# yifanlu0227/HEAL

Hardware: AMD Instinct MI355X
Metric: scenes/sec (5-agent OPV2V-H, PointPillars+PyramidFusion) (higher is better)
Workload: dtype f32

## Files before the change

### heal_amd/_capi.py

```python
import ctypes
import os
import re

HERE = os.path.dirname(os.path.abspath(__file__))
LIB_PATH = os.environ.get("HEAL_AMD_LIB") or os.path.join(HERE, "lib", "libheal_amd.so")
HEADER = os.path.join(os.path.dirname(HERE), "include", "heal_amd.h")
HEADER_EXPERIMENTAL = os.path.join(os.path.dirname(HERE), "include", "heal_amd_experimental.h")

_lib = None

c_void_p, c_int, c_float, c_size_t = ctypes.c_void_p, ctypes.c_int, ctypes.c_float, ctypes.c_size_t

_SIGNATURES = {
    "heal_abi_version": (c_int, []),
    "heal_last_error": (ctypes.c_char_p, []),
    "heal_fill_bytes": (c_int, [c_void_p, c_int, c_size_t, c_void_p]),
    "heal_next_launch_events": (c_int, [c_void_p, c_void_p]),
    "heal_voxelize_workspace": (c_size_t, [c_int, c_int, c_int, ctypes.c_longlong]),
    "heal_voxelize": (c_int, [c_void_p, c_int, c_void_p, c_void_p, c_int, c_int, c_int,
                              c_void_p, c_void_p, c_void_p, c_void_p, c_void_p, c_void_p, c_void_p, c_size_t, c_int, c_void_p]),
    "heal_voxelize_batch_workspace": (c_size_t, [c_int, c_int, c_int, c_int, ctypes.c_longlong]),
    "heal_voxelize_batch": (c_int, [c_void_p, c_void_p, c_int, c_void_p, c_void_p, c_int, c_int, c_void_p, c_void_p,
                                    c_void_p, c_void_p, c_void_p, c_size_t, c_int, c_void_p]),
    "heal_mask_points": (c_int, [c_void_p, c_int, c_void_p, c_int, c_void_p, c_void_p]),
    "heal_pfn_scatter_workspace": (c_size_t, [c_int] * 5),
    "heal_pfn_scatter": (c_int, [c_void_p, c_void_p, c_void_p, c_int, c_void_p, c_int,
                                 c_void_p, c_void_p, c_void_p, c_int,
                                 c_float, c_float, c_float, c_float, c_float, c_float,
                                 c_int, c_int, c_int, c_void_p, c_void_p, c_void_p, c_size_t, c_void_p]),
    "heal_pfn_pillars": (c_int, [c_void_p, c_void_p, c_void_p, c_int, c_void_p, c_int, c_void_p, c_void_p, c_void_p, c_int,
                                 c_float, c_float, c_float, c_float, c_float, c_float, c_int, c_int, c_int, c_void_p, c_void_p,
                                 c_void_p]),
    "heal_pillar_canvas": (c_int, [c_void_p, c_void_p, c_int, c_int, c_int, c_int, c_void_p, c_void_p]),
    "heal_pillar_stem_block": (c_int, [c_void_p, c_void_p, c_int, c_int, c_int, c_int] + [c_void_p] * 4 + [c_int] + [c_void_p] * 3),
    "heal_bev_pool_backward": (c_int, [c_void_p] * 5 + [c_int] * 6 + [c_void_p] * 6),
    "heal_warp_fuse": (c_int, [c_void_p, c_void_p, c_int, c_int, c_int, c_int, c_void_p, c_void_p, c_int, c_void_p,
                               c_void_p, c_void_p]),
    "heal_warp_fuse_levels": (c_int, [c_int, c_void_p, c_void_p, c_int, c_void_p, c_void_p, c_void_p, c_void_p, c_void_p, c_int,
                                      c_void_p, c_void_p, c_void_p]),
    "heal_warp_fuse_backward": (c_int, [c_void_p, c_void_p, c_int, c_int, c_int, c_int, c_void_p, c_void_p, c_int, c_void_p,
                                        c_void_p, c_void_p, c_void_p, c_void_p]),
    "heal_warp_agent": (c_int, [c_void_p, c_void_p, c_int, c_int, c_int, c_void_p, c_void_p, c_int, c_void_p,
                                c_void_p, c_void_p, c_void_p]),
    "heal_warp_agents_pm": (c_int, [c_void_p, c_int, c_int, c_int, c_int, c_void_p, c_void_p, c_int, c_void_p, c_void_p]),
    "heal_fuse_warped": (c_int, [c_void_p, c_void_p, c_int, c_int, c_int, c_int, c_void_p, c_void_p]),
    "heal_fuse_warped_rows": (c_int, [c_void_p, c_void_p, c_void_p, c_int, c_int, c_int, c_int, c_void_p, c_void_p]),
    "heal_decode_nms_workspace": (c_size_t, [c_int, c_int]),
    "heal_decode_nms": (c_int, [c_void_p, c_void_p, c_void_p, c_void_p, c_int, c_int, c_int, c_int,
                                c_float, c_float, c_float, c_int, c_void_p, c_void_p,
                                c_void_p, c_void_p, c_void_p, c_int, c_void_p, c_size_t, c_void_p]),
    "heal_quad_iou": (c_int, [c_void_p, c_int, c_void_p, c_int, c_void_p, c_void_p]),
    "heal_bev_pool_workspace": (c_size_t, [c_int] * 9),
    "heal_bev_pool": (c_int, [c_void_p, c_void_p, c_void_p, c_void_p, c_int, c_int, c_int, c_int, c_int, c_int,
                              c_void_p, c_void_p, c_void_p, c_void_p, c_void_p, c_size_t, c_void_p]),
    "heal_bev_pool_pm_workspace": (c_size_t, [c_int] * 5),
    "heal_bev_pool_pm": (c_int, [c_void_p, c_int, c_void_p, c_void_p] + [c_int] * 6 + [c_void_p] * 5 + [c_size_t, c_void_p]),
    "heal_bev_pool_scatter": (c_int, [c_void_p, c_int, c_void_p, c_void_p] + [c_int] * 6 + [c_void_p] * 4 + [c_size_t, c_void_p]),
    "heal_bev_pool_scatter_multi": (c_int, [c_int] + [c_void_p] * 16),
    "heal_bev_pool_emit": (c_int, [c_int, c_int, c_void_p, c_void_p, c_void_p, c_size_t, c_void_p]),
    "heal_bev_stem_block": (c_int, [c_int, c_int] + [c_void_p] * 8 + [c_size_t, c_void_p]),
    "heal_pfn_train_blocks": (c_int, [c_int]),
    "heal_pfn_features": (c_int, [c_void_p, c_void_p, c_void_p, c_int, c_int, c_void_p, c_void_p, c_void_p, c_float, c_float,
                                  c_float, c_float, c_float, c_float, c_void_p, c_void_p]),
    "heal_pfn_moments": (c_int, [c_void_p, c_void_p, c_void_p, c_int, c_int, c_float, c_float, c_float, c_float, c_float, c_float,
                                 c_void_p, c_void_p]),
    "heal_pfn_backward": (c_int, [c_void_p, c_void_p, c_void_p, c_int, c_int, c_void_p, c_void_p, c_void_p, c_void_p, c_void_p,
                                  c_float, c_float, c_float, c_float, c_float, c_float, c_void_p, c_void_p, c_void_p]),
    "heal_mean_vfe": (c_int, [c_void_p, c_void_p, c_int, c_int, c_int, c_void_p, c_void_p, c_void_p]),
    "heal_sp_sort_workspace": (c_size_t, [c_int]),
    "heal_sp_sort_sites": (c_int, [c_void_p, c_int, c_void_p, c_int, c_void_p, c_void_p, c_void_p, c_size_t, c_void_p,
                                   c_void_p]),
    "heal_sp_wgrad_chunks": (c_int, [c_int]),
    "heal_sp_wgrad": (c_int, [c_void_p, c_void_p, c_void_p, c_int, c_int, c_int, c_int, c_void_p, c_void_p, c_void_p]),
    "heal_sp_gather_rows": (c_int, [c_void_p, c_void_p, c_int, c_int, c_void_p, c_void_p, c_void_p]),
    "heal_sp_table_capacity": (c_size_t, [c_int]),
    "heal_sp_hash_build": (c_int, [c_void_p, c_int, c_void_p, c_int, c_void_p, c_void_p, c_size_t, c_void_p, c_void_p]),
    "heal_sp_neighbors": (c_int, [c_void_p, c_int, c_void_p, c_void_p, c_void_p, c_void_p, c_void_p, c_int,
                                  c_void_p, c_void_p, c_size_t, c_void_p, c_void_p, c_void_p]),
    "heal_sp_out_sites_workspace": (c_size_t, [c_int, c_int]),
    "heal_sp_out_sites": (c_int, [c_void_p, c_int, c_void_p, c_void_p, c_void_p, c_void_p, c_void_p, c_int,
                                  c_void_p, c_int, c_void_p, c_void_p, c_size_t, c_void_p, c_void_p]),
    "heal_conv_gemm": (c_int, [c_void_p, c_void_p, c_void_p, c_void_p] + [c_int] * 8 + [c_void_p, c_void_p]),
    "heal_ln_stats": (c_int, [c_void_p, c_int, c_int, c_float, c_void_p, c_void_p]),
    "heal_linear": (c_int, [c_void_p, c_int, c_int, ctypes.c_longlong, c_void_p, c_void_p, c_void_p, c_int, c_void_p, c_int,
                            c_int, c_void_p, c_int, c_void_p, c_int, c_int, c_int, c_int, c_int, c_int, c_int,
                            ctypes.c_longlong, c_int, c_void_p]),
    "heal_split_attn_workspace": (c_size_t, [c_int, c_int, c_int]),
    "heal_split_attn_weights": (c_int, [c_void_p, ctypes.c_longlong, c_int, c_int, c_int] + [c_void_p] * 5 + [c_float] +
                                [c_void_p] * 5),
    "heal_split_attn_colsum": (c_int, [c_void_p, ctypes.c_longlong, c_int, c_int, c_int, c_void_p, c_void_p]),
    "heal_split_attn_weights_from_colsum": (c_int, [c_void_p, c_int, c_int, c_int, c_int] + [c_void_p] * 5 + [c_float] +
                                            [c_void_p] * 4),
    "heal_sp_rank_bytes": (c_size_t, [c_void_p, c_int]),
    "heal_sp_out_sites_rank": (c_int, [c_void_p, c_int, c_void_p, c_void_p, c_void_p, c_void_p, c_void_p, c_int,
                                       c_void_p, c_int, c_void_p, c_void_p, c_size_t, c_void_p, c_void_p, c_void_p]),
    "heal_sp_neighbors_rank": (c_int, [c_void_p, c_int, c_void_p, c_void_p, c_void_p, c_void_p, c_void_p, c_int,
                                       c_void_p, c_size_t, c_int, c_void_p, c_void_p, c_void_p, c_void_p]),
    "heal_sp_neighbors_root": (c_int, [c_void_p, c_int, c_void_p, c_void_p, c_void_p, c_void_p, c_void_p, c_int,
                                       c_void_p, c_size_t, c_int, c_void_p, c_void_p, c_void_p, c_void_p]),
    "heal_sp_root_rank_bytes": (c_size_t, [c_void_p, c_int]),
    "heal_sp_pair_tiles_words": (c_size_t, [c_int, c_int]),
    "heal_sp_neighbor_tiles": (c_int, [c_void_p, c_int, c_void_p, c_void_p, c_void_p, c_void_p, c_void_p, c_int,
                                       c_void_p, c_size_t, c_int, c_int, c_void_p, c_int, c_void_p, c_void_p, c_void_p]),
    "heal_sp_tiles_to_neighbors": (c_int, [c_void_p, c_int, c_int, c_void_p, c_void_p, c_void_p]),
    "heal_sp_conv_tiles_supported": (c_int, [c_int, c_int]),
    "heal_sp_conv_tiles": (c_int, [c_void_p, c_void_p, c_int, c_int, c_int, c_int, c_void_p, c_void_p, c_void_p, c_int,
                                   c_void_p, c_void_p, c_void_p]),
    "heal_sp_root_rank": (c_int, [c_void_p, c_int, c_void_p, c_int, c_void_p, c_void_p, c_void_p, c_int, c_void_p, c_void_p,
                                  c_size_t, c_void_p, c_void_p]),
    "heal_gconv_conv3_supported": (c_int, [c_int] * 5),
    "heal_gconv_conv3": (c_int, [c_void_p] * 6 + [c_int] * 7 + [c_void_p, c_void_p]),
    "heal_sp_transpose_neighbors": (c_int, [c_void_p, c_int, c_int, c_int, c_void_p, c_void_p, c_void_p]),
    "heal_sp_weight_fragments": (c_int, [c_void_p, c_int, c_int, c_int, c_void_p, c_void_p]),
    "heal_sp_conv": (c_int, [c_void_p, c_void_p, c_int, c_int, c_int, c_int, c_void_p, c_void_p, c_void_p, c_void_p, c_int,
                             c_void_p, c_void_p, c_void_p]),
    "heal_sp_to_bev_workspace": (c_size_t, [c_int, c_int, c_int, c_int]),
    "heal_sp_to_bev": (c_int, [c_void_p, c_void_p, c_int, c_int, c_void_p, c_int, c_void_p, c_void_p, c_size_t,
                               c_void_p, c_void_p]),
    "heal_agent_attention": (c_int, [c_void_p, c_void_p, c_void_p, c_void_p, c_int, c_int, c_int, c_int, c_float,
                                     c_int, c_void_p, c_int, c_void_p]),
    "heal_agent_attention_backward": (c_int, [c_void_p] * 5 + [c_int, c_int, c_int, c_int, c_float, c_int] + [c_void_p] * 3 +
                                      [c_int, c_void_p]),
    "heal_grouped_conv3x3": (c_int, [c_void_p, c_void_p, c_void_p, c_int, c_int, c_int, c_int, c_int, c_int, c_int,
                                     c_void_p, c_void_p]),
    "heal_bias_act": (c_int, [c_void_p, c_void_p, c_void_p, c_int, c_int, c_int, c_int, c_void_p]),
    "heal_resnext_bottleneck": (c_int, [c_void_p] * 7 + [c_int, c_int, c_int, c_int, c_void_p, c_void_p]),
    "heal_upsample2x_bilinear": (c_int, [c_void_p, c_int, c_int, c_int, c_int, c_void_p, c_void_p]),
    "heal_depthwise_conv": (c_int, [c_void_p, c_void_p, c_void_p] + [c_int] * 11 + [c_void_p, c_void_p, c_void_p]),
    "heal_camera_matrices": (c_int, [c_void_p] * 5 + [c_int, c_void_p, c_void_p]),
    "heal_channel_dot": (c_int, [c_void_p] * 3 + [c_int] * 3 + [c_void_p, c_void_p]),
    "heal_layernorm_nchw": (c_int, [c_void_p] * 3 + [c_int] * 3 + [c_float, c_void_p, c_void_p]),
    "heal_se_gate": (c_int, [c_void_p] * 5 + [c_int] * 3 + [c_float, c_int, c_void_p, c_void_p]),
    "heal_conv1x1": (c_int, [c_void_p] * 5 + [c_int] * 8 + [c_void_p, c_void_p]),
    "heal_stem7x7": (c_int, [c_void_p, ctypes.c_longlong, c_int, c_int, c_int, c_int, c_void_p, c_void_p, c_int, c_void_p, c_void_p]),
    "heal_conv1x1_split_supported": (c_int, [c_int] * 4),
    "heal_conv1x1_split": (c_int, [c_void_p] * 4 + [c_int] * 7 + [c_void_p, c_void_p]),
    "heal_conv1x1_tiled_supported": (c_int, [c_int] * 5),
    "heal_conv1x1_tiled": (c_int, [c_void_p] * 4 + [c_int] * 9 + [c_void_p, c_void_p]),
    "heal_conv1x1_splitk_workspace": (c_size_t, [c_int] * 5),
    "heal_conv1x1_splitk": (c_int, [c_void_p] * 5 + [c_int] * 7 + [c_void_p, c_void_p, c_size_t, c_void_p]),
    "heal_conv1x1_d2s": (c_int, [c_void_p] * 3 + [c_int] * 9 + [c_void_p, c_void_p]),
    "heal_conv3x3": (c_int, [c_void_p] * 4 + [c_int] * 7 + [c_void_p, c_void_p]),
    "heal_conv3x3_same": (c_int, [c_void_p] * 3 + [c_int] * 11 + [c_void_p, c_void_p]),
    "heal_grouped16_conv3x3": (c_int, [c_void_p] * 3 + [c_int] * 5 + [c_void_p, c_void_p]),
    "heal_grouped_small_conv3x3": (c_int, [c_void_p] * 3 + [c_int] * 7 + [c_void_p, c_void_p]),
    "heal_conv3x3_winograd4": (c_int, [c_void_p] * 4 + [c_int] * 6 + [c_void_p, c_void_p]),
    "heal_conv3x3_winograd": (c_int, [c_void_p] * 4 + [c_int] * 7 + [c_void_p, c_void_p]),
    "heal_conv3x3_winograd_kc": (c_int, [c_void_p] * 4 + [c_int] * 8 + [c_void_p, c_void_p]),
    "heal_conv3x3_winograd_splitk_workspace": (c_size_t, [c_int] * 5),
    "heal_conv3x3_winograd_splitk": (c_int, [c_void_p] * 4 + [c_int] * 8 + [c_void_p, c_void_p, c_size_t, c_void_p]),
    "heal_nms_quads_workspace": (c_size_t, [c_int]),
    "heal_nms_quads": (c_int, [c_void_p, c_int, c_float, c_void_p, c_size_t, c_void_p, c_void_p, c_void_p]),
    "heal_window_attention": (c_int, [c_void_p, c_void_p, c_int, c_int, c_int, c_int, c_int, c_int, c_float, c_void_p,
                                      c_void_p]),
    "heal_window_attention_backward_workspace": (c_size_t, [c_int, c_int, c_int, c_int]),
    "heal_window_attention_backward": (c_int, [c_void_p] * 4 + [c_int] * 6 + [c_float, c_void_p, c_void_p, c_void_p, c_size_t,
                                                c_void_p]),
    "heal_agent_window_attention": (c_int, [c_void_p, c_void_p] + [c_int] * 8 + [c_float, c_void_p, c_void_p]),
    "heal_agent_mean": (c_int, [c_void_p, c_int, ctypes.c_longlong, c_void_p, c_void_p]),
    "heal_v2v_message_workspace": (c_size_t, [c_int] * 5),
    "heal_v2v_message": (c_int, [c_void_p, c_void_p, c_void_p, ctypes.c_longlong, c_void_p, c_void_p] + [c_int] * 9
                         + [c_void_p, c_void_p, c_size_t, c_void_p]),
    "heal_gru_zero_state": (c_int, [c_void_p, ctypes.c_longlong, c_void_p, ctypes.c_longlong] + [c_int] * 4 + [c_void_p, c_void_p]),
    "heal_label_assign_workspace": (c_size_t, [c_int]),
    "heal_label_assign": (c_int, [c_void_p, c_int, c_void_p, c_int, c_float, c_float, c_void_p, c_void_p, c_void_p,
                                  c_size_t, c_void_p]),
    "heal_boxes_bev_matrix": (c_int, [c_void_p, c_int, c_void_p, c_int, c_int, c_void_p, c_void_p]),
    "heal_nms_bev_workspace": (c_size_t, [c_int]),
    "heal_nms_bev": (c_int, [c_void_p, c_int, c_float, c_int, c_void_p, c_size_t, c_void_p, c_void_p, c_void_p]),
}


class HealAmdError(RuntimeError):
    pass


def declared_symbols(experimental=False):
    text = open(HEADER_EXPERIMENTAL if experimental else HEADER).read()
    text = re.sub(r"/\*.*?\*/", "", text, flags=re.S)
    return sorted(set(re.findall(r"\b(heal_[a-z0-9_]+)\s*\(", text)))


def abi_version_of_header():
    m = re.search(r"#define\s+HEAL_AMD_ABI_VERSION\s+(\d+)", open(HEADER).read())
    if not m:
        raise HealAmdError(f"{HEADER} does not define HEAL_AMD_ABI_VERSION")
    return int(m.group(1))


def lib():
    global _lib
    if _lib is None:
        if not os.path.exists(LIB_PATH):
            raise HealAmdError(
                f"{LIB_PATH} is missing: the HIP extension has not been built "
                "(run `python -m heal_amd.build`); heal_amd has no CPU fallback")
        import torch
        L = ctypes.CDLL(LIB_PATH)
        for name, (res, args) in _SIGNATURES.items():
            if not hasattr(L, name):
                continue
            f = getattr(L, name)
            f.restype = res
            f.argtypes = args
        want = abi_version_of_header()
        got = int(L.heal_abi_version()) if hasattr(L, "heal_abi_version") else -1
        if got != want:
            raise HealAmdError(f"{LIB_PATH} has C-ABI version {got}, include/heal_amd.h declares {want}: rebuild it "
                               "(python -m heal_amd.build --force)")
        _lib = L
    return _lib


_TRACE = int(os.environ.get("HEAL_TRACE_CALLS", "0") or 0)


def _trace_call(name, args):
    import sys
    import torch
    cap = torch.cuda.is_current_stream_capturing()
    extra = ""
    if _TRACE >= 2:
        extra = " " + " ".join(hex(a.value or 0) if isinstance(a, ctypes.c_void_p) else str(a) for a in args
                               if isinstance(a, (int, float, ctypes.c_void_p)))
    print(f"[heal pid {os.getpid()}] {'capture ' if cap else ''}{name}{extra}", file=sys.stderr, flush=True)


def _trace_done(name):
    import sys
    import torch
    if not torch.cuda.is_current_stream_capturing():
        torch.cuda.synchronize()
        print(f"[heal pid {os.getpid()}]   ok {name}", file=sys.stderr, flush=True)


_GUARD = os.environ.get("HEAL_GRAPH_GUARD", "0") == "1"
_guard_log = []


def _segments():
    import torch
    segs = []
    for seg in torch.cuda.memory_snapshot():
        blocks, addr = [], seg["address"]
        for b in seg["blocks"]:
            a = b.get("address", addr)
            blocks.append((a, a + b["size"], b["state"]))
            addr = a + b["size"]
        pool = tuple(seg.get("segment_pool_id", (0, 0)))
        segs.append((seg["address"], seg["address"] + seg["total_size"], pool != (0, 0), blocks))
    segs.sort()
    return segs


def _locate(segs, addr):
    import bisect
    i = bisect.bisect_right(segs, (addr, float("inf"), True, [])) - 1
    if i < 0 or not (segs[i][0] <= addr < segs[i][1]):
        return None
    for lo, hi, state in segs[i][3]:
        if lo <= addr < hi:
            return segs[i][2], state
    return segs[i][2], "unknown"


def guard_begin():
    global _guard_log
    _guard_log = []


def guard_take():
    global _guard_log
    log, _guard_log = _guard_log, []
    if not log:
        return []
    segs = _segments()
    seen, out = set(), []
    for name, addr in log:
        if addr not in seen and _locate(segs, addr) is not None:
            seen.add(addr)
            out.append((name, addr))
    return out


def guard_check(entries, what="captured graph"):
    if not entries:
        return
    segs = _segments()
    for name, addr in entries:
        where = _locate(segs, addr)
        if where is None:
            raise HealAmdError(f"{what}: {name} was captured with device address {addr:#x}, which is no longer mapped "
                               "(its tensor was freed and the memory returned to the driver)")
        private, state = where
        if not private and state != "active_allocated":
            raise HealAmdError(f"{what}: {name} was captured with device address {addr:#x}, whose block is now '{state}' "
                               "(its tensor was freed: a replay would read or overwrite somebody else's memory)")


def call(name, *args):
    L = lib()
    if not hasattr(L, name):
        raise HealAmdError(f"libheal_amd.so does not export {name}")
    if _TRACE:
        _trace_call(name, args)
    if _GUARD:
        import torch
        if torch.cuda.is_current_stream_capturing():
            _guard_log.extend((name, a.value) for a in args if isinstance(a, ctypes.c_void_p) and a.value)
    rc = getattr(L, name)(*args)
    if rc != 0:
        raise HealAmdError(f"{name} failed: {L.heal_last_error().decode(errors='replace')}")
    if _TRACE:
        _trace_done(name)


def query(name, *args):
    L = lib()
    if not hasattr(L, name):
        raise HealAmdError(f"libheal_amd.so does not export {name}")
    return int(getattr(L, name)(*args))
```

### heal_amd/csrc/common.h

```cpp
#pragma once
#include <hip/hip_runtime.h>
#include <hip/hip_ext.h>
#include <stdint.h>
#include <stddef.h>
#include <stdio.h>
#include <stdarg.h>

#define HEAL_WAVE 64

namespace heal {

char* err_buf();
int set_error(const char* fmt, ...);

inline size_t align_up(size_t x, size_t a = 256) { return (x + a - 1) / a * a; }
inline int ceil_div(int a, int b) { return (a + b - 1) / b; }
inline int64_t ceil_div64(int64_t a, int64_t b) { return (a + b - 1) / b; }

struct Arena {
    char* base; size_t cap; size_t off;
    Arena(void* p, size_t n) : base((char*)p), cap(n), off(0) {}
    template <typename T> T* take(size_t count) {
        size_t bytes = align_up(count * sizeof(T));
        T* r = (T*)(base + off);
        off += bytes;
        return r;
    }
    bool ok() const { return off <= cap && (base != nullptr || off == 0); }
};

#define HEAL_HIP(expr)                                                                      \
    do {                                                                                    \
        hipError_t e__ = (expr);                                                            \
        if (e__ != hipSuccess)                                                              \
            return heal::set_error("%s failed: %s (%s:%d)", #expr, hipGetErrorString(e__), \
                                   __FILE__, __LINE__);                                     \
    } while (0)

#define HEAL_REQUIRE(cond, ...)                       \
    do {                                              \
        if (!(cond)) return heal::set_error(__VA_ARGS__); \
    } while (0)

#define HEAL_LAUNCH_CHECK() HEAL_HIP(hipGetLastError())

int debug_env_once(const char* name);
#define HEAL_DEBUG_ENV(name) ([]() -> int { static const int v__ = heal::debug_env_once(name); return v__; }())

int fill_bytes(void* dst, int byte, size_t bytes, hipStream_t s);
int copy_word(int* dst, const int* src, hipStream_t s);
#define HEAL_FILL(dst, byte, bytes, s)                      \
    do {                                                    \
        if (heal::fill_bytes((dst), (byte), (bytes), (s))) return 1; \
    } while (0)

struct LaunchEvents { hipEvent_t start, stop; };
LaunchEvents take_launch_events();
#define HEAL_LAUNCH_EV(kernel, grid, block, lds, stream, ...)                                                        \
    do {                                                                                                             \
        const heal::LaunchEvents ev__ = heal::take_launch_events();                                                  \
        if (ev__.start && ev__.stop)                                                                                 \
            hipExtLaunchKernelGGL(kernel, grid, block, (std::uint32_t)(lds), stream, ev__.start, ev__.stop, 0, __VA_ARGS__); \
        else                                                                                                         \
            hipLaunchKernelGGL(kernel, grid, block, (std::uint32_t)(lds), stream, __VA_ARGS__);                      \
    } while (0)

#define HEAL_LAUNCH_EV2(kernel, grid, block, lds, stream, ev_start, ev_stop, ...)                                    \
    do {                                                                                                             \
        if ((ev_start) || (ev_stop))                                                                                 \
            hipExtLaunchKernelGGL(kernel, grid, block, (std::uint32_t)(lds), stream, ev_start, ev_stop, 0, __VA_ARGS__); \
        else                                                                                                         \
            hipLaunchKernelGGL(kernel, grid, block, (std::uint32_t)(lds), stream, __VA_ARGS__);                      \
    } while (0)

__device__ __forceinline__ int lane_id() { return threadIdx.x & 63; }

__device__ __forceinline__ unsigned long long lanemask_lt() {
    return (1ull << (threadIdx.x & 63)) - 1ull;
}

__device__ __forceinline__ float wave_sum(float v) {
#pragma unroll
    for (int o = 32; o > 0; o >>= 1) v += __shfl_xor(v, o, 64);
    return v;
}
__device__ __forceinline__ int wave_sum_i(int v) {
#pragma unroll
    for (int o = 32; o > 0; o >>= 1) v += __shfl_xor(v, o, 64);
    return v;
}
__device__ __forceinline__ int wave_incl_scan(int v) {
    const int l = threadIdx.x & 63;
#pragma unroll
    for (int o = 1; o < 64; o <<= 1) {
        int t = __shfl_up(v, o, 64);
        if (l >= o) v += t;
    }
    return v;
}


__device__ __forceinline__ void lds_barrier() { asm volatile("s_waitcnt lgkmcnt(0)\n\ts_barrier" ::: "memory"); }

struct Block3 { unsigned x, y, z; };
__device__ inline Block3 xcd_block() {
    const unsigned gx = gridDim.x, gy = gridDim.y, nb = gx * gy * gridDim.z;
    unsigned b = blockIdx.x + gx * (blockIdx.y + gy * blockIdx.z);
    const unsigned q = nb >> 3, r = nb & 7u, xcd = b & 7u;
    b = (xcd < r ? xcd * (q + 1) : r * (q + 1) + (xcd - r) * q) + (b >> 3);
    Block3 o;
    o.x = b % gx;
    b /= gx;
    o.y = b % gy;
    o.z = b / gy;
    return o;
}

}
```

### heal_amd/csrc/conv1x1.hip

```cpp
#include <stdlib.h>
#include "common.h"
#include "../../include/heal_amd.h"

namespace heal {

using f32x4 = __attribute__((ext_vector_type(4))) float;

template <int BM, int BN, int KC, int STRIDE>
__global__ __launch_bounds__(256) void k_conv1x1(const float* __restrict__ x, const float* __restrict__ wfrag,
                                                const float* __restrict__ bias, const float* __restrict__ res,
                                                const float* __restrict__ in_scale, int Cin, int Kpad, int Cout,
                                                int HW, int Wo, int in_W, int in_HW, int act, int out_pm,
                                                int d2s_k, int d2s_ctot, int d2s_coff, int n_img, int ksplit,
                                                float* __restrict__ y) {
    constexpr int MT = BM / 64;
    constexpr int NT = BN / 16;
    constexpr int LD = BN + 16;
    constexpr int KS = KC / 4;
    constexpr int TPR = BN / 4;
    constexpr int RPP = 256 / TPR;
    constexpr int NPASS = KC / RPP;
    static_assert(NPASS >= 1 && KC % RPP == 0, "bad staging shape");
    __shared__ __attribute__((aligned(16))) float sB[2][KC][LD];
    const Block3 bk = xcd_block();
    const int m0 = bk.x * BM, p0 = bk.y * BN, n = bk.z % n_img, kpart = bk.z / n_img;
    const int wave = threadIdx.x >> 6, l = threadIdx.x & 63;
    const int lk = l >> 4, ln = l & 15;
    const float* __restrict__ xin = x + (size_t)n * Cin * in_HW;
    const int ksteps = Kpad / 4;
    const int nchunks_all = Kpad / KC, cps = (nchunks_all + ksplit - 1) / ksplit;
    const int cbeg = kpart * cps, nchunks = min(cbeg + cps, nchunks_all);
    const float* __restrict__ scl = in_scale ? in_scale + (size_t)n * Cin : nullptr;
    const int sp = (threadIdx.x % TPR) * 4, sc = threadIdx.x / TPR;
    const bool pix_ok = p0 + sp < HW;

    f32x4 acc[MT][NT];
#pragma unroll
    for (int mt = 0; mt < MT; ++mt)
#pragma unroll
        for (int nt = 0; nt < NT; ++nt) acc[mt][nt] = f32x4{0.f, 0.f, 0.f, 0.f};

    float4 stage[NPASS];
    auto load_chunk = [&](int c) {
#pragma unroll
        for (int i = 0; i < NPASS; ++i) {
            const int ch = c * KC + sc + RPP * i;
            if (pix_ok && ch < Cin) {
                float4 v;
                if constexpr (STRIDE == 1) {
                    v = *reinterpret_cast<const float4*>(xin + (size_t)ch * HW + p0 + sp);
                } else {
                    const int p = p0 + sp, oy = p / Wo, ox = p - oy * Wo;
                    const float* src = xin + (size_t)ch * in_HW + (size_t)(oy * STRIDE) * in_W + ox * STRIDE;
                    v = make_float4(src[0], src[STRIDE], src[2 * STRIDE], src[3 * STRIDE]);
                }
                if (scl) { const float g = scl[ch]; v.x *= g; v.y *= g; v.z *= g; v.w *= g; }
                stage[i] = v;
            } else {
                stage[i] = make_float4(0.f, 0.f, 0.f, 0.f);
            }
        }
    };
    auto store_chunk = [&](int buf) {
#pragma unroll
        for (int i = 0; i < NPASS; ++i) *reinterpret_cast<float4*>(&sB[buf][sc + RPP * i][sp]) = stage[i];
    };

    float a_cur[MT][KS], a_nxt[MT][KS];
    auto load_a = [&](int c, float (&a)[MT][KS]) {
#pragma unroll
        for (int mt = 0; mt < MT; ++mt) {
            const int mtg = (m0 >> 4) + wave * MT + mt;
#pragma unroll
            for (int q = 0; q < KS / 4; ++q) {
                const float4 v = *reinterpret_cast<const float4*>(wfrag + (((size_t)mtg * (ksteps / 4) + (c * KS) / 4 + q) * 64 + l) * 4);
                a[mt][4 * q] = v.x; a[mt][4 * q + 1] = v.y; a[mt][4 * q + 2] = v.z; a[mt][4 * q + 3] = v.w;
            }
        }
    };

    load_a(cbeg, a_cur);
    load_chunk(cbeg);
    store_chunk(0);
    __syncthreads();
    for (int c = cbeg; c < nchunks; ++c) {
        const int buf = (c - cbeg) & 1;
        if (c + 1 < nchunks) {
            load_a(c + 1, a_nxt);
            load_chunk(c + 1);
        }
        float bfr[2][NT];
        auto read_b = [&](int ks, float (&dst)[NT]) {
#pragma unroll
            for (int gq = 0; gq < NT / 4; ++gq) {
                const float4 v = *reinterpret_cast<const float4*>(&sB[buf][ks * 4 + lk][gq * 64 + 4 * ln]);
                dst[4 * gq] = v.x; dst[4 * gq + 1] = v.y; dst[4 * gq + 2] = v.z; dst[4 * gq + 3] = v.w;
            }
        };
        read_b(0, bfr[0]);
#pragma unroll
        for (int ks = 0; ks < KS; ++ks) {
            if (ks + 1 < KS) read_b(ks + 1, bfr[(ks + 1) & 1]);
            __builtin_amdgcn_sched_barrier(0);
#pragma unroll
            for (int nt = 0; nt < NT; ++nt)
#pragma unroll
                for (int mt = 0; mt < MT; ++mt)
                    acc[mt][nt] = __builtin_amdgcn_mfma_f32_16x16x4f32(a_cur[mt][ks], bfr[ks & 1][nt], acc[mt][nt], 0, 0, 0);
        }
        if (c + 1 < nchunks) store_chunk(buf ^ 1);
        __syncthreads();
#pragma unroll
        for (int mt = 0; mt < MT; ++mt)
#pragma unroll
            for (int ks = 0; ks < KS; ++ks) a_cur[mt][ks] = a_nxt[mt][ks];
    }

    if (out_pm == 1) {
        float* __restrict__ yout = y + (size_t)n * HW * Cout;
#pragma unroll
        for (int mt = 0; mt < MT; ++mt) {
            const int co = m0 + (wave * MT + mt) * 16 + lk * 4;
            if (co >= Cout) continue;
            float4 bv = make_float4(0.f, 0.f, 0.f, 0.f);
            if (bias) bv = *reinterpret_cast<const float4*>(bias + co);
#pragma unroll
            for (int nt = 0; nt < NT; ++nt) {
                const int p = p0 + (nt / 4) * 64 + 4 * ln + (nt & 3);
                if (p >= HW) continue;
                float4 v = make_float4(acc[mt][nt][0] + bv.x, acc[mt][nt][1] + bv.y, acc[mt][nt][2] + bv.z,
                                       acc[mt][nt][3] + bv.w);
                if (act == 1) {
                    v.x = fmaxf(v.x, 0.f); v.y = fmaxf(v.y, 0.f); v.z = fmaxf(v.z, 0.f); v.w = fmaxf(v.w, 0.f);
                } else if (act == 2) {
                    v.x = v.x / (1.f + expf(-v.x)); v.y = v.y / (1.f + expf(-v.y));
                    v.z = v.z / (1.f + expf(-v.z)); v.w = v.w / (1.f + expf(-v.w));
                }
                *reinterpret_cast<float4*>(yout + (size_t)p * Cout + co) = v;
            }
        }
        return;
    }
    float* __restrict__ yout = y + ((size_t)kpart * n_img + n) * Cout * HW;
    const float* __restrict__ rin = res ? res + (size_t)n * Cout * HW : nullptr;
    constexpr int NG = NT / 4;
#pragma unroll
    for (int mt = 0; mt < MT; ++mt) {
        float4 rq[4][NG];
        if (rin) {
#pragma unroll
            for (int r = 0; r < 4; ++r)
#pragma unroll
                for (int gq = 0; gq < NG; ++gq) {
                    const int co = min(m0 + (wave * MT + mt) * 16 + lk * 4 + r, Cout - 1), p = min(p0 + gq * 64 + 4 * ln, HW - 4);
                    rq[r][gq] = *reinterpret_cast<const float4*>(rin + (size_t)co * HW + p);
                }
        }
#pragma unroll
        for (int r = 0; r < 4; ++r) {
            const int co = m0 + (wave * MT + mt) * 16 + lk * 4 + r;
            if (co >= Cout) continue;
            const float bv = bias ? bias[co] : 0.f;
#pragma unroll
            for (int gq = 0; gq < NG; ++gq) {
                const int p = p0 + gq * 64 + 4 * ln;
                if (p >= HW) continue;
                float4 v = make_float4(acc[mt][4 * gq][r] + bv, acc[mt][4 * gq + 1][r] + bv, acc[mt][4 * gq + 2][r] + bv,
                                       acc[mt][4 * gq + 3][r] + bv);
                const size_t o = (size_t)co * HW + p;
                if (rin) { const float4 q = rq[r][gq]; v.x += q.x; v.y += q.y; v.z += q.z; v.w += q.w; }
                if (act == 1) {
                    v.x = fmaxf(v.x, 0.f); v.y = fmaxf(v.y, 0.f); v.z = fmaxf(v.z, 0.f); v.w = fmaxf(v.w, 0.f);
                } else if (act == 2) {
                    v.x = v.x / (1.f + expf(-v.x)); v.y = v.y / (1.f + expf(-v.y));
                    v.z = v.z / (1.f + expf(-v.z)); v.w = v.w / (1.f + expf(-v.w));
                } else if (act == 3) {
                    v.x = 0.5f * v.x * (1.f + erff(v.x * 0.70710678118654752f));
                    v.y = 0.5f * v.y * (1.f + erff(v.y * 0.70710678118654752f));
                    v.z = 0.5f * v.z * (1.f + erff(v.z * 0.70710678118654752f));
                    v.w = 0.5f * v.w * (1.f + erff(v.w * 0.70710678118654752f));
                }
                if (out_pm != 2) {
                    *reinterpret_cast<float4*>(yout + o) = v;
                } else {
                    const int kk = d2s_k * d2s_k, Ho = HW / Wo;
                    const int c = co / kk, rr = co - c * kk, dy = rr / d2s_k, dx = rr - dy * d2s_k;
                    const int hh = p / Wo, ww = p - hh * Wo;
                    float* dst = y + (((size_t)n * d2s_ctot + d2s_coff + c) * ((size_t)Ho * d2s_k) + (size_t)hh * d2s_k + dy) *
                                         ((size_t)Wo * d2s_k) + (size_t)ww * d2s_k + dx;
                    if (d2s_k == 1) {
                        *reinterpret_cast<float4*>(dst) = v;
                    } else {
                        dst[0] = v.x; dst[d2s_k] = v.y; dst[2 * d2s_k] = v.z; dst[3 * d2s_k] = v.w;
                    }
                }
            }
        }
    }
}


__global__ __launch_bounds__(256) void k_conv1x1_splitk_reduce(const float4* __restrict__ part, const float* __restrict__ bias,
                                                              const float4* __restrict__ res, int ksplit, int Cout, int HW4,
                                                              size_t total4, int act, float4* __restrict__ y) {
    const size_t i = (size_t)blockIdx.x * 256 + threadIdx.x;
    if (i >= total4) return;
    float4 v = part[i];
    for (int k = 1; k < ksplit; ++k) {
        const float4 q = part[(size_t)k * total4 + i];
        v.x += q.x; v.y += q.y; v.z += q.z; v.w += q.w;
    }
    const float bv = bias ? bias[(i / HW4) % Cout] : 0.f;
    v.x += bv; v.y += bv; v.z += bv; v.w += bv;
    if (res) { const float4 q = res[i]; v.x += q.x; v.y += q.y; v.z += q.z; v.w += q.w; }
    if (act == 1) {
        v.x = fmaxf(v.x, 0.f); v.y = fmaxf(v.y, 0.f); v.z = fmaxf(v.z, 0.f); v.w = fmaxf(v.w, 0.f);
    } else if (act == 2) {
        v.x = v.x / (1.f + expf(-v.x)); v.y = v.y / (1.f + expf(-v.y)); v.z = v.z / (1.f + expf(-v.z)); v.w = v.w / (1.f + expf(-v.w));
    } else if (act == 3) {
        v.x = 0.5f * v.x * (1.f + erff(v.x * 0.70710678118654752f)); v.y = 0.5f * v.y * (1.f + erff(v.y * 0.70710678118654752f));
        v.z = 0.5f * v.z * (1.f + erff(v.z * 0.70710678118654752f)); v.w = 0.5f * v.w * (1.f + erff(v.w * 0.70710678118654752f));
    }
    y[i] = v;
}

}

using namespace heal;

namespace heal {
int splitk_reduce_launch(const float* partials, const float* bias, const float* residual, int ksplit, int n, int cout, int HW,
                         int act, float* y, hipStream_t s, hipEvent_t ev_stop) {
    const size_t total4 = (size_t)n * cout * HW / 4;
    HEAL_LAUNCH_EV2(k_conv1x1_splitk_reduce, dim3((unsigned)((total4 + 255) / 256)), dim3(256), 0, s, (hipEvent_t) nullptr, ev_stop,
                    reinterpret_cast<const float4*>(partials), bias, reinterpret_cast<const float4*>(residual), ksplit, cout,
                    HW / 4, total4, act, reinterpret_cast<float4*>(y));
    HEAL_LAUNCH_CHECK();
    return 0;
}
}

static int conv1x1_launch(const float* x, const float* weight_frag, const float* bias, const float* residual,
                          const float* in_scale, int n, int cin, int cout, int H, int W, int stride, int act,
                          int out_pixel_major, int d2s_k, int d2s_ctot, int d2s_coff, float* y, void* stream,
                          int ksplit = 1, float* partials = nullptr) {
    HEAL_REQUIRE(n >= 1 && H >= 1 && W >= 1 && cin >= 1 && cout >= 1, "conv1x1: bad shape");
    HEAL_REQUIRE(stride == 1 || stride == 2, "conv1x1: stride must be 1 or 2 (got %d)", stride);
    const int kpad = (cin + 31) / 32 * 32, mpad = (cout + 63) / 64 * 64;
    const int Ho = (H - 1) / stride + 1, Wo = (W - 1) / stride + 1, HW = Ho * Wo;
    if (stride == 1) HEAL_REQUIRE(HW % 4 == 0, "conv1x1: H*W must be a multiple of 4 (got %d)", HW);
    else HEAL_REQUIRE(Wo % 4 == 0, "conv1x1: output width must be a multiple of 4 for stride 2 (got %d)", Wo);
    HEAL_REQUIRE(act >= 0 && act <= 3, "conv1x1: act must be 0 (none), 1 (ReLU), 2 (SiLU) or 3 (GELU)");
    HEAL_REQUIRE(x && weight_frag && y, "conv1x1: null pointer");
    if (out_pixel_major == 1) {
        HEAL_REQUIRE(residual == nullptr && act != 3, "conv1x1: pixel-major output takes no residual / GELU");
        HEAL_REQUIRE(cout % 4 == 0 && ((uintptr_t)bias & 15) == 0, "conv1x1: pixel-major output needs Cout %% 4 == 0 and a 16-B aligned bias");
    }
    hipStream_t s = (hipStream_t)stream;
    int bm = 64, bn = 64, kc = 32;
    if (const char* e = getenv("HEAL_C1_CFG")) {
        int a_ = 0, b_ = 0, c_ = 0;
        if (stride == 1 && sscanf(e, "%d,%d,%d", &a_, &b_, &c_) == 3) { bm = a_; bn = b_; kc = c_; }
    }
    HEAL_REQUIRE(mpad % bm == 0, "conv1x1: padded Cout %d not a multiple of the tile height %d", mpad, bm);
#define HEAL_C1(BM_, BN_, KC_, ST_)                                                                              \
    if (bm == BM_ && bn == BN_ && kc == KC_ && stride == ST_) {                                                  \
        if (ksplit > 1)                                                                                          \
            HEAL_LAUNCH_EV2((k_conv1x1<BM_, BN_, KC_, ST_>), dim3(mpad / BM_, ceil_div(HW, BN_), n * ksplit), dim3(256), 0, s, \
                            ev.start, (hipEvent_t) nullptr,                                                      \
                            x, weight_frag, (const float*)nullptr, (const float*)nullptr, in_scale, cin, kpad, cout, HW, Wo, W, \
                            H * W, 0, 0, 1, 0, 0, n, ksplit, partials);                                          \
        else                                                                                                     \
            HEAL_LAUNCH_EV2((k_conv1x1<BM_, BN_, KC_, ST_>), dim3(mpad / BM_, ceil_div(HW, BN_), n), dim3(256), 0, s, \
                            ev.start, ev.stop,                                                                   \
                            x, weight_frag, bias, residual, in_scale, cin, kpad, cout, HW, Wo, W, H * W, act, out_pixel_major, \
                            d2s_k, d2s_ctot, d2s_coff, n, 1, y);                                                 \
        launched = true;                                                                                         \
    }
    bool launched = false;
    const LaunchEvents ev = take_launch_events();
    HEAL_C1(64, 64, 32, 1) HEAL_C1(64, 64, 32, 2)
    HEAL_C1(128, 128, 32, 1) HEAL_C1(64, 128, 32, 1) HEAL_C1(128, 64, 32, 1)
#undef HEAL_C1
    HEAL_REQUIRE(launched, "conv1x1: no kernel for tile (%d,%d,%d) stride %d", bm, bn, kc, stride);
    if (ksplit > 1) {
        const size_t total4 = (size_t)n * cout * HW / 4;
        HEAL_LAUNCH_EV2(k_conv1x1_splitk_reduce, dim3((unsigned)((total4 + 255) / 256)), dim3(256), 0, s, (hipEvent_t) nullptr, ev.stop,
                        reinterpret_cast<const float4*>(partials), bias, reinterpret_cast<const float4*>(residual), ksplit, cout,
                        HW / 4, total4, act, reinterpret_cast<float4*>(y));
    }
    HEAL_LAUNCH_CHECK();
    return 0;
}

extern "C" int heal_conv1x1(const float* x, const float* weight_frag, const float* bias, const float* residual,
                            const float* in_scale, int n, int cin, int cout, int H, int W, int stride, int act,
                            int out_pixel_major, float* y, void* stream) {
    HEAL_REQUIRE(out_pixel_major == 0 || out_pixel_major == 1, "conv1x1: out_pixel_major must be 0 or 1");
    return conv1x1_launch(x, weight_frag, bias, residual, in_scale, n, cin, cout, H, W, stride, act, out_pixel_major, 1, 0, 0,
                          y, stream);
}

extern "C" int heal_conv1x1_d2s(const float* x, const float* weight_frag, const float* bias, int n, int cin, int cout, int H,
                                int W, int act, int k, int dst_channels, int dst_channel_offset, float* y, void* stream) {
    HEAL_REQUIRE(k >= 1 && k <= 8 && cout % (k * k) == 0, "conv1x1_d2s: Cout must be a multiple of k^2 (k = %d)", k);
    HEAL_REQUIRE(W % 4 == 0, "conv1x1_d2s: W must be a multiple of 4 (got %d)", W);
    HEAL_REQUIRE(dst_channel_offset >= 0 && dst_channel_offset + cout / (k * k) <= dst_channels,
                 "conv1x1_d2s: channel slice [%d, %d) outside the %d destination channels", dst_channel_offset,
                 dst_channel_offset + cout / (k * k), dst_channels);
    HEAL_REQUIRE(((uintptr_t)y & 15) == 0, "conv1x1_d2s: destination must be 16-B aligned");
    return conv1x1_launch(x, weight_frag, bias, nullptr, nullptr, n, cin, cout, H, W, 1, act, 2, k, dst_channels,
                          dst_channel_offset, y, stream);
}

extern "C" size_t heal_conv1x1_splitk_workspace(int n, int cout, int H, int W, int ksplit) {
    return ksplit > 1 ? (size_t)ksplit * n * cout * H * W * sizeof(float) : 0;
}

extern "C" int heal_conv1x1_splitk(const float* x, const float* weight_frag, const float* bias, const float* residual,
                                   const float* in_scale, int n, int cin, int cout, int H, int W, int act, int ksplit, float* y,
                                   void* ws, size_t ws_bytes, void* stream) {
    const int nchunks = (cin + 31) / 32;
    HEAL_REQUIRE(ksplit >= 2 && ksplit <= nchunks, "conv1x1_splitk: ksplit must be in [2, %d] (got %d)", nchunks, ksplit);
    HEAL_REQUIRE((ksplit - 1) * ceil_div(nchunks, ksplit) < nchunks,
                 "conv1x1_splitk: %d splits of %d chunks leave an empty split (use ceil(chunks / ceil(chunks / ksplit)))", ksplit,
                 nchunks);
    HEAL_REQUIRE((H * W) % 4 == 0, "conv1x1_splitk: H*W must be a multiple of 4");
    HEAL_REQUIRE((long long)n * ksplit <= 65535, "conv1x1_splitk: n * ksplit exceeds the grid limit");
    HEAL_REQUIRE(ws && ws_bytes >= heal_conv1x1_splitk_workspace(n, cout, H, W, ksplit) && ((uintptr_t)ws & 15) == 0,
                 "conv1x1_splitk: workspace too small or misaligned");
    HEAL_REQUIRE(act >= 0 && act <= 3, "conv1x1_splitk: act must be 0..3");
    return conv1x1_launch(x, weight_frag, bias, residual, in_scale, n, cin, cout, H, W, 1, act, 0, 1, 0, 0, y, stream, ksplit,
                          (float*)ws);
}
```

### heal_amd/csrc/gconv_small.hip

```cpp
#include <stdlib.h>
#include "common.h"
#include "../../include/heal_amd.h"

namespace heal {

using f32x4 = __attribute__((ext_vector_type(4))) float;

template <int CG, int TH, int STRIDE>
__global__ __launch_bounds__(256) __attribute__((amdgpu_waves_per_eu(3, 4))) void k_gconv_small(
    const float* __restrict__ x, const float* __restrict__ wq, const float* __restrict__ bias, int C, int H, int W, int Ho,
    int Wo, int tiles_x, int relu, float* __restrict__ y) {
    static_assert(CG == 4 || CG == 8 || CG == 16, "4, 8 or 16 channels per group");
    static_assert(TH == 8 || TH == 16, "tile height");
    static_assert(STRIDE == 1 || STRIDE == 2, "stride");
    constexpr int TW = STRIDE == 1 ? 32 : 16, NSEG = TW / 16, RW = TH / 4;
    constexpr int PR = STRIDE * TH + 3 - STRIDE, PC = STRIDE * TW + 3 - STRIDE;
    constexpr int NSIDE = 3 - STRIDE;
    constexpr int NSTEP = 9 * CG;
    constexpr int KH = CG == 16 ? 2 : 1;
    constexpr int CGH = CG / KH;
    constexpr int NB = CG / 4, NBH = CGH / 4;
    __shared__ float4 sP[PR * PC * 4];
    __shared__ float4 sW[NSTEP * 16 / 4];
    const Block3 bk = xcd_block();
    const int sg = bk.y, n = bk.z;
    const int ty = bk.x / tiles_x, tx = bk.x - ty * tiles_x;
    const int oy0 = ty * TH, ox0 = tx * TW;
    const int gy0 = oy0 * STRIDE - 1, gx0 = ox0 * STRIDE;
    const int t = threadIdx.x, wave = t >> 6, l = t & 63;
    const size_t HW = (size_t)H * W, HWo = (size_t)Ho * Wo;
    const float* __restrict__ xin = x + ((size_t)n * C + (size_t)sg * 16) * HW;

    constexpr int N_IN = PR * 8 * 4, IT_IN = (N_IN + 255) / 256;
    constexpr int N_HA = PR * NSIDE * 4;
    static_assert(N_HA <= 256 && STRIDE * TW == 32, "staging shape");
    float4 vin[IT_IN][4];
    unsigned ok_bits = 0;
#pragma unroll
    for (int it = 0; it < IT_IN; ++it) {
        const int u = min(t + 256 * it, N_IN - 1);
        const int gq = u & 3, quad = (u >> 2) & 7, row = u >> 5;
        const int gy = gy0 + row, gx = gx0 + quad * 4;
        const bool ok = gy >= 0 && gy < H && gx < W;
        ok_bits |= ok ? (1u << it) : 0u;
        const float* src = xin + (size_t)(gq * 4) * HW + (ok ? (size_t)gy * W + gx : 0);
        vin[it][0] = *reinterpret_cast<const float4*>(src);
        vin[it][1] = *reinterpret_cast<const float4*>(src + HW);
        vin[it][2] = *reinterpret_cast<const float4*>(src + 2 * HW);
        vin[it][3] = *reinterpret_cast<const float4*>(src + 3 * HW);
    }
    float4 vha;
    {
        const int u = min(t, N_HA - 1);
        const int gq = u & 3, side = NSIDE == 2 ? (u >> 2) & 1 : 0, row = u / (4 * NSIDE);
        const int gy = gy0 + row, gx = side ? gx0 + 32 : gx0 - 1;
        const bool ok = gy >= 0 && gy < H && gx >= 0 && gx < W;
        ok_bits |= ok ? 256u : 0u;
        const float* src = xin + (size_t)(gq * 4) * HW + (ok ? (size_t)gy * W + gx : 0);
        vha = make_float4(src[0], src[HW], src[2 * HW], src[3 * HW]);
    }
    constexpr int N_W4 = NSTEP * 16 / 4, IT_W = (N_W4 + 255) / 256;
#pragma unroll
    for (int it = 0; it < IT_W; ++it) {
        const int i = min(t + 256 * it, N_W4 - 1);
        sW[i] = reinterpret_cast<const float4*>(wq + (size_t)sg * NSTEP * 16)[i];
    }
#pragma unroll
    for (int it = 0; it < IT_IN; ++it) {
        const int u = min(t + 256 * it, N_IN - 1);
        const int gq = u & 3, quad = (u >> 2) & 7, row = u >> 5;
        const bool ok = (ok_bits >> it) & 1u;
        float4* d = sP + (row * PC + 1 + quad * 4) * 4 + gq;
        const float4 a = vin[it][0], b = vin[it][1], c = vin[it][2], e = vin[it][3];
        d[0] = make_float4(ok ? a.x : 0.f, ok ? b.x : 0.f, ok ? c.x : 0.f, ok ? e.x : 0.f);
        d[4] = make_float4(ok ? a.y : 0.f, ok ? b.y : 0.f, ok ? c.y : 0.f, ok ? e.y : 0.f);
        d[8] = make_float4(ok ? a.z : 0.f, ok ? b.z : 0.f, ok ? c.z : 0.f, ok ? e.z : 0.f);
        d[12] = make_float4(ok ? a.w : 0.f, ok ? b.w : 0.f, ok ? c.w : 0.f, ok ? e.w : 0.f);
    }
    {
        const int u = min(t, N_HA - 1);
        const int gq = u & 3, side = NSIDE == 2 ? (u >> 2) & 1 : 0, row = u / (4 * NSIDE);
        const bool okh = ok_bits & 256u;
        sP[(row * PC + (side ? PC - 1 : 0)) * 4 + gq] =
            make_float4(okh ? vha.x : 0.f, okh ? vha.y : 0.f, okh ? vha.z : 0.f, okh ? vha.w : 0.f);
    }
    __syncthreads();
    const float bv0 = bias ? bias[sg * 16 + (l & 15)] : 0.f;
    const int p = (l >> 4) * 4 + (l & 3);
    const int unit0 = (((l >> 2) & 3) * 4 / CG) * NB;
    const float4* __restrict__ abase = sP + ((wave * RW * STRIDE) * PC + p * STRIDE) * 4 + unit0;

    f32x4 acc[RW][NSEG];
#pragma unroll
    for (int o = 0; o < RW; ++o)
#pragma unroll
        for (int s = 0; s < NSEG; ++s) acc[o][s] = f32x4{0.f, 0.f, 0.f, 0.f};
#pragma unroll
    for (int half = 0; half < KH; ++half) {
        float wreg[9 * CGH];
#pragma unroll
        for (int tap = 0; tap < 9; ++tap)
#pragma unroll
            for (int ci = 0; ci < CGH; ++ci)
                wreg[tap * CGH + ci] = reinterpret_cast<const float*>(sW)[(tap * CG + half * CGH + ci) * 16 + (l & 15)];
#pragma unroll
        for (int ry = 0; ry < STRIDE * (RW - 1) + 3; ++ry) {
#pragma unroll
            for (int dx = 0; dx < 3; ++dx) {
                float4 av[NSEG][NBH];
#pragma unroll
                for (int s = 0; s < NSEG; ++s)
#pragma unroll
                    for (int h = 0; h < NBH; ++h) av[s][h] = abase[(ry * PC + s * 16 * STRIDE + dx) * 4 + half * NBH + h];
#pragma unroll
                for (int ci = 0; ci < CGH; ++ci) {
#pragma unroll
                    for (int o = 0; o < RW; ++o) {
                        const int dy = ry - STRIDE * o;
                        if (dy < 0 || dy > 2) continue;
#pragma unroll
                        for (int s = 0; s < NSEG; ++s) {
                            const float4 q = av[s][ci >> 2];
                            const float a = (ci & 3) == 0 ? q.x : (ci & 3) == 1 ? q.y : (ci & 3) == 2 ? q.z : q.w;
                            acc[o][s] = __builtin_amdgcn_mfma_f32_4x4x1f32(a, wreg[(dy * 3 + dx) * CGH + ci], acc[o][s], 0, 0, 0);
                        }
                    }
                }
            }
        }
    }
    float* __restrict__ yout = y + ((size_t)n * C + (size_t)sg * 16 + (l & 15)) * HWo;
#pragma unroll
    for (int o = 0; o < RW; ++o) {
        const int oy = oy0 + wave * RW + o;
#pragma unroll
        for (int s = 0; s < NSEG; ++s) {
            const int ox = ox0 + s * 16 + (l >> 4) * 4;
            if (oy >= Ho || ox >= Wo) continue;
            float4 v = make_float4(acc[o][s][0] + bv0, acc[o][s][1] + bv0, acc[o][s][2] + bv0, acc[o][s][3] + bv0);
            if (relu) { v.x = fmaxf(v.x, 0.f); v.y = fmaxf(v.y, 0.f); v.z = fmaxf(v.z, 0.f); v.w = fmaxf(v.w, 0.f); }
            *reinterpret_cast<float4*>(yout + (size_t)oy * Wo + ox) = v;
        }
    }
}

}

using namespace heal;

extern "C" int heal_grouped_small_conv3x3(const float* x, const float* weight_q, const float* bias, int n, int channels,
                                          int group_channels, int H, int W, int stride, int relu, float* y, void* stream) {
    HEAL_REQUIRE(group_channels == 4 || group_channels == 8 || group_channels == 16,
                 "grouped_small_conv3x3: 4, 8 or 16 channels per group (got %d)", group_channels);
    HEAL_REQUIRE(stride == 1 || stride == 2, "grouped_small_conv3x3: stride must be 1 or 2 (got %d)", stride);
    const int Ho = (H - 1) / stride + 1, Wo = (W - 1) / stride + 1;
    HEAL_REQUIRE(n >= 1 && channels >= 16 && channels % 16 == 0 && H >= 1 && W >= 4 && W % 4 == 0 && Wo % 4 == 0,
                 "grouped_small_conv3x3: needs channels %% 16 == 0, W %% 4 == 0 and an output width %% 4 == 0 (got C=%d W=%d)",
                 channels, W);
    HEAL_REQUIRE(x && weight_q && y && ((uintptr_t)x & 15) == 0 && ((uintptr_t)y & 15) == 0,
                 "grouped_small_conv3x3: bad pointer (x, y must be 16-B aligned)");
    int th = (group_channels == 4 && stride == 1) ? 16 : 8;
    if (const char* e = getenv("HEAL_GS_TH")) th = atoi(e) == 8 ? 8 : atoi(e) == 16 ? 16 : th;
    if (stride == 2 || group_channels == 16) th = 8;
    const int tw = stride == 1 ? 32 : 16;
    const int tiles_x = ceil_div(Wo, tw), tiles_y = ceil_div(Ho, th);
    HEAL_REQUIRE(channels / 16 <= 65535 && n <= 65535, "grouped_small_conv3x3: grid limit");
    const dim3 grid(tiles_x * tiles_y, channels / 16, n);
    hipStream_t s_ = (hipStream_t)stream;
#define HEAL_GS(CG_, TH_, ST_)                                                                                        \
    if (group_channels == CG_ && th == TH_ && stride == ST_)                                                          \
        HEAL_LAUNCH_EV((k_gconv_small<CG_, TH_, ST_>), grid, dim3(256), 0, s_, x, weight_q, bias, channels, H, W, Ho, Wo, tiles_x, relu, y);
    HEAL_GS(4, 16, 1) HEAL_GS(4, 8, 1) HEAL_GS(8, 16, 1) HEAL_GS(8, 8, 1)
    HEAL_GS(4, 8, 2) HEAL_GS(8, 8, 2) HEAL_GS(16, 8, 1) HEAL_GS(16, 8, 2)
#undef HEAL_GS
    HEAL_LAUNCH_CHECK();
    return 0;
}
```

### heal_amd/opencood/models/fuse_modules/pyramid_fuse.py

```python
import torch
import torch.nn as nn

from heal_amd import derived, ops
from heal_amd.opencood.models.sub_modules.bev_blocks import (Bottleneck, ResNetBEVBackbone, ResNetModified)


def crop_window(H, W, ratio_h, ratio_w):
    crop_H = H / ratio_h - 4
    crop_W = W / ratio_w - 4
    return (int(H // 2 - crop_H // 2), int(H // 2 + crop_H // 2),
            int(W // 2 - crop_W // 2), int(W // 2 + crop_W // 2))


def weighted_fuse_autograd(x, occ, record_len, affine_matrix, crops=None):
    import torch.nn.functional as F
    score = torch.sigmoid(occ) + 1e-4
    if crops is not None:
        keep = torch.ones_like(score)
        for a, c in enumerate(crops):
            if c is not None:
                keep[a] = 0
                keep[a, :, c[0]:c[1], c[2]:c[3]] = 1
        score = score * keep
    out, start = [], 0
    for b, n in enumerate(record_len):
        M = torch.as_tensor(affine_matrix[b][0, :n], dtype=x.dtype, device=x.device)
        xs, ss = x[start:start + n], score[start:start + n]
        grid = F.affine_grid(M, list(xs.shape), align_corners=False)
        feat = F.grid_sample(xs, grid, align_corners=False)
        sc = F.grid_sample(ss, F.affine_grid(M, list(ss.shape), align_corners=False), align_corners=False)
        sc = sc.masked_fill(sc == 0, float("-inf")).softmax(dim=0)
        sc = torch.where(torch.isnan(sc), torch.zeros_like(sc), sc)
        out.append((feat * sc).sum(0))
        start += n
    return torch.stack(out)


class _WarpFuse(torch.autograd.Function):

    @staticmethod
    def forward(ctx, x, occ, rows, grid_f64, crop):
        x, occ = x.contiguous(), occ.contiguous()
        ctx.save_for_backward(x, occ)
        ctx.args = (rows, grid_f64, crop)
        return ops.warp_fuse(x, occ, rows, grid_f64, crop)

    @staticmethod
    def backward(ctx, grad_out):
        x, occ = ctx.saved_tensors
        rows, grid_f64, crop = ctx.args
        g_x, g_occ = ops.warp_fuse_backward(x, occ, rows, grad_out.contiguous(), grid_f64, crop)
        return g_x, g_occ, None, None, None


def weighted_fuse(x, occ, record_len, affine_matrix, grid_f64=True, crops=None):
    import os
    grad = torch.is_grad_enabled() and (x.requires_grad or occ.requires_grad)
    if grad and not (x.is_cuda and os.environ.get("HEAL_K5_BACKWARD", "1") == "1"):
        return weighted_fuse_autograd(x, occ, record_len, affine_matrix, crops)
    out = []
    start = 0
    for b, n in enumerate(record_len):
        rows = affine_matrix[b][0, :n]
        crop = None
        if crops is not None:
            crop = [crops[start + a] if crops[start + a] is not None else (0, 0, 0, 0) for a in range(n)]
        if grad:
            out.append(_WarpFuse.apply(x[start:start + n], occ[start:start + n], rows, grid_f64, crop))
        else:
            out.append(ops.warp_fuse(x[start:start + n], occ[start:start + n], rows, grid_f64, crop))
        start += n
    return out[0].unsqueeze(0) if len(out) == 1 else torch.stack(out)


def _stage_influence(lo, hi, layer, size_in):
    size = size_in
    for blk in layer:
        s_ = blk.stride
        size = (size - 1) // s_ + 1
        lo = max(0, -((1 - lo) // s_))
        hi = min(size, hi // s_ + 1)
    return lo, hi, size


def _stage_needs(olo, ohi, layer, size_in):
    for blk in reversed(list(layer)):
        s_ = blk.stride
        olo, ohi = s_ * olo - 1, s_ * (ohi - 1) + 2
    return max(0, olo), min(size_in, ohi)


class PyramidFusion(ResNetBEVBackbone):
    def __init__(self, model_cfg, input_channels=64):
        super().__init__(model_cfg, input_channels)
        if model_cfg["resnext"]:
            self.resnet = ResNetModified(Bottleneck, model_cfg["layer_nums"], model_cfg["layer_strides"],
                                         model_cfg["num_filters"], inplanes=model_cfg.get("inplanes", 64),
                                         groups=32, width_per_group=4, expansion=1)
        self.align_corners = model_cfg.get("align_corners", False)
        if self.align_corners:
            raise NotImplementedError("align_corners=True fusion is not used by any HEAL config")
        for i in range(self.num_levels):
            setattr(self, f"single_head_{i}", nn.Conv2d(model_cfg["num_filters"][i], 1, kernel_size=1))

    def occupancy_head(self, i, feature):
        head = getattr(self, f"single_head_{i}")
        if not torch.is_grad_enabled() and ops.channel_dot_supported(feature):
            return ops.channel_dot(feature, head.weight, head.bias)
        return head(feature)

    def forward_single(self, spatial_features):
        feature_list = self.get_multiscale_feature(spatial_features)
        occ_map_list = [self.occupancy_head(i, feature_list[i]) for i in range(self.num_levels)]
        return self.decode_multiscale_feature(feature_list), occ_map_list

    def _zero_response_slot(self, like):
        return "pyramid_zero_response", [*self.resnet.parameters(), *self.resnet.buffers()], (tuple(like.shape[1:]), str(like.device))

    def _zero_response(self, like):
        def build():
            z = torch.zeros((1,) + tuple(like.shape[1:]), dtype=like.dtype, device=like.device)
            return [f.clone() for f in self.resnet(z)]
        tag, sources, extra = self._zero_response_slot(like)
        return derived.derived(tag, sources, build, extra)

    def _camcrop_plan(self, x, cam_slice, box):
        H, W = int(x.shape[2]), int(x.shape[3])
        ly, hy, lx, hx = box
        plan = []
        for i in range(self.layernum_):
            layer = getattr(self.resnet, f"layer{i}")
            s_tot = 1
            for blk in layer:
                s_tot *= blk.stride
            oly, ohy, Ho = _stage_influence(ly, hy, layer, H)
            olx, ohx, Wo = _stage_influence(lx, hx, layer, W)
            iy0, iy1 = _stage_needs(oly, ohy, layer, H)
            ix0, ix1 = _stage_needs(olx, ohx, layer, W)
            a = 8 * s_tot
            cy0, cy1, cx0, cx1 = iy0 // a * a, min(H, -(-iy1 // a) * a), ix0 // a * a, min(W, -(-ix1 // a) * a)
            if (cy1 - cy0) * (cx1 - cx0) > 0.7 * H * W:
                plan.append(None)
            else:
                plan.append(((cy0, cy1, cx0, cx1), (oly, ohy, olx, ohx),
                             (oly - cy0 // s_tot, ohy - cy0 // s_tot, olx - cx0 // s_tot, ohx - cx0 // s_tot)))
            ly, hy, lx, hx, H, W = oly, ohy, olx, ohx, Ho, Wo
        return plan

    def get_multiscale_feature_camcrop(self, x, cam_slice, box):
        n = int(x.shape[0])
        c0, c1 = cam_slice
        other = (0, c0) if c0 > 0 else (c1, n)
        bg = self._zero_response(x)
        plan = self._camcrop_plan(x, cam_slice, box)
        feats = []
        for i in range(self.layernum_):
            layer = getattr(self.resnet, f"layer{i}")
            if plan[i] is None:
                x = self.resnet.run_stage(layer, x)
                feats.append(x)
                continue
            (cy0, cy1, cx0, cx1), (gy0, gy1, gx0, gx1), (py0, py1, px0, px1) = plan[i]
            full = torch.empty((n,) + tuple(bg[i].shape[1:]), dtype=x.dtype, device=x.device)
            if other[1] > other[0]:
                xa = x[other[0]:other[1]]
                for j, blk in enumerate(layer):
                    xa = blk(xa, out=full[other[0]:other[1]]) if j == len(layer) - 1 else blk(xa)
            yc = layer(x[c0:c1, :, cy0:cy1, cx0:cx1].contiguous())
            full[c0:c1] = bg[i]
            full[c0:c1, :, gy0:gy1, gx0:gx1] = yc[:, :, py0:py1, px0:px1]
            x = full
            feats.append(x)
        return feats

    @property
    def layernum_(self):
        return self.resnet.layernum

    def _camcrop_args(self, spatial_features, agent_modality_list, cam_boxes):
        import os
        if (not cam_boxes or agent_modality_list is None or torch.is_grad_enabled() or not spatial_features.is_cuda
                or os.environ.get("HEAL_PYRAMID_CAMCROP", "1") != "1"):
            return None
        cams = [k for k, m in enumerate(agent_modality_list) if m in cam_boxes]
        n = len(agent_modality_list)
        if not cams or cams != list(range(cams[0], cams[-1] + 1)) or (cams[0] != 0 and cams[-1] != n - 1):
            return None
        from heal_amd.opencood.models.sub_modules.bev_blocks import Bottleneck
        if not all(isinstance(b, Bottleneck) and b.conv2.kernel_size == (3, 3) and b.conv2.padding == (1, 1)
                   for i in range(self.layernum_) for b in getattr(self.resnet, f"layer{i}")):
            return None
        boxes = [cam_boxes[agent_modality_list[k]] for k in cams]
        box = (min(b[0] for b in boxes), max(b[1] for b in boxes), min(b[2] for b in boxes), max(b[3] for b in boxes))
        H, W = int(spatial_features.shape[2]), int(spatial_features.shape[3])
        if H % 32 or W % 32 or not (0 <= box[0] < box[1] <= H and 0 <= box[2] < box[3] <= W):
            return None
        if derived.capturing() and not derived.ready(*self._zero_response_slot(spatial_features)):
            return None
        return (cams[0], cams[-1] + 1), box

    def multiscale(self, spatial_features, agent_modality_list=None, cam_boxes=None):
        cc = self._camcrop_args(spatial_features, agent_modality_list, cam_boxes)
        if cc is not None:
            return self.get_multiscale_feature_camcrop(spatial_features, *cc)
        return self.get_multiscale_feature(spatial_features)

    def forward_collab(self, spatial_features, record_len, affine_matrix, agent_modality_list=None,
                       cam_crop_info=None, grid_f64=True, cam_boxes=None):
        feature_list = self.multiscale(spatial_features, agent_modality_list, cam_boxes if len(record_len) == 1 else None)
        use_crop = bool(cam_crop_info) and not self.training
        fused_feature_list, occ_map_list = [], []
        import os
        if (len(record_len) == 1 and not torch.is_grad_enabled() and feature_list[0].is_cuda and 1 <= self.num_levels <= 4
                and int(record_len[0]) <= 8 and os.environ.get("HEAL_K5_LEVELS", "1") == "1"):
            n = int(record_len[0])
            crops_all = []
            for i in range(self.num_levels):
                occ_map_list.append(self.occupancy_head(i, feature_list[i]))
                crops = None
                if use_crop:
                    _, _, H, W = occ_map_list[i].shape
                    crops = [crop_window(H, W, cam_crop_info[mod][f"crop_ratio_H_{mod}"], cam_crop_info[mod][f"crop_ratio_W_{mod}"])
                             if mod in cam_crop_info else None for mod in agent_modality_list]
                crops_all.append(crops)
            fused = ops.warp_fuse_levels([f[:n] for f in feature_list], [o[:n] for o in occ_map_list], affine_matrix[0][0, :n],
                                         grid_f64, crops_all if use_crop else None)
            return self.decode_multiscale_feature([f.unsqueeze(0) for f in fused]), occ_map_list
        for i in range(self.num_levels):
            occ_map = self.occupancy_head(i, feature_list[i])
            occ_map_list.append(occ_map)
            crops = None
            if use_crop:
                _, _, H, W = occ_map.shape
                crops = []
                for mod in agent_modality_list:
                    if mod in cam_crop_info:
                        crops.append(crop_window(H, W, cam_crop_info[mod][f"crop_ratio_H_{mod}"],
                                                 cam_crop_info[mod][f"crop_ratio_W_{mod}"]))
                    else:
                        crops.append(None)
            fused_feature_list.append(weighted_fuse(feature_list[i], occ_map, record_len, affine_matrix,
                                                    grid_f64, crops))
        return self.decode_multiscale_feature(fused_feature_list), occ_map_list
```

### heal_amd/opencood/models/sub_modules/bev_blocks.py

```python
import numpy as np
import torch
import torch.nn as nn
import torch.nn.functional as F

from heal_amd.derived import derived


def fold_bn(conv, bn, transposed=False):
    def build():
        scale = bn.weight / torch.sqrt(bn.running_var + bn.eps)
        shift = bn.bias - bn.running_mean * scale
        if transposed:
            w = conv.weight * scale.view(1, -1, 1, 1)
        else:
            w = conv.weight * scale.view(-1, 1, 1, 1)
        b = shift if conv.bias is None else shift + conv.bias * scale
        return w.contiguous(), b.contiguous()
    return derived("fold_bn", (conv.weight, conv.bias, bn.weight, bn.bias, bn.running_mean, bn.running_var), build, (transposed,))


import os
_CONV1X1 = os.environ.get("HEAL_CONV1X1", "1") == "1"
_CONV3X3 = os.environ.get("HEAL_CONV3X3", "1") == "1"


def conv_bias_act(x, w, b, stride, padding, dilation=1, groups=1, relu=True, residual=None, out=None):
    from heal_amd import ops
    if torch.is_grad_enabled() and (x.requires_grad or w.requires_grad or (b is not None and b.requires_grad)):
        y = F.conv2d(x, w, b, stride, padding, dilation, groups)
        if residual is not None:
            y = y + residual
        return F.relu(y) if relu else y
    st = stride if isinstance(stride, int) else stride[0]
    pd = padding if isinstance(padding, int) else padding[0]
    dl = dilation if isinstance(dilation, int) else dilation[0]
    if (groups > 1 and w.shape[2:] == (3, 3) and pd == 1 and dl == 1 and st in (1, 2) and residual is None
            and w.shape[1] in (4, 8, 16) and w.shape[0] == x.shape[1]):
        return ops.grouped_conv3x3(x, w, b, groups, st, relu)
    if _CONV1X1 and groups == 1 and w.shape[2:] == (1, 1) and st in (1, 2) and pd == 0:
        Ho, Wo = (int(x.shape[2]) - 1) // st + 1, (int(x.shape[3]) - 1) // st + 1
        if ops.conv1x1_supported(int(w.shape[1]), int(w.shape[0]), Ho * Wo, st, Wo):
            return ops.conv1x1(x, w, b, residual, 1 if relu else 0, stride=st, out=out)
    if (_CONV3X3 and x.is_cuda and groups == 1 and tuple(w.shape[2:]) == (3, 3) and pd == 1 and dl == 1 and st in (1, 2)
            and (padding if isinstance(padding, int) else padding[1]) == 1
            and (stride if isinstance(stride, int) else stride[1]) == st):
        return ops.conv3x3(x, w, b, residual, relu, st)
    if (x.is_cuda and groups == 1 and tuple(w.shape[2:]) == (7, 7) and st == 2 and pd == 3 and dl == 1 and residual is None
            and ops.conv7x7_s2_supported(int(w.shape[1]), int(w.shape[0]), int(x.shape[3]))):
        return ops.conv7x7_s2(x, w, b, relu)
    _library_fallthrough(x, w, stride, padding, dilation, groups)
    y = F.conv2d(x, w, None, stride, padding, dilation, groups)
    if b is None and residual is None and not relu:
        return y
    return ops.bias_act_(y, b, residual, relu)


LIBRARY_CONV_SHAPES = {}


def _library_fallthrough(x, w, stride, padding, dilation, groups):
    key = (int(w.shape[1]) * groups, int(w.shape[0]), tuple(int(v) for v in w.shape[2:]), stride, padding, dilation, groups,
           int(x.shape[2]), int(x.shape[3]))
    n = LIBRARY_CONV_SHAPES.get(key, 0)
    LIBRARY_CONV_SHAPES[key] = n + 1
    if n == 0 and x.is_cuda:
        import warnings
        warnings.warn(f"heal_amd: convolution Cin={key[0]} Cout={key[1]} k={key[2]} stride={stride} pad={padding} dil={dilation} "
                      f"groups={groups} on a {key[7]}x{key[8]} map is not covered by a hand-written kernel: library (MIOpen) path",
                      RuntimeWarning, stacklevel=3)


def grad_path(x, *modules):
    if not torch.is_grad_enabled():
        return False
    if torch.is_tensor(x) and x.requires_grad:
        return True
    for m in modules:
        if m is not None and (m.training or any(p.requires_grad for p in m.parameters())):
            return True
    return False


def _require_eval(module):
    if module.training and torch.is_grad_enabled():
        raise NotImplementedError(
            f"{type(module).__name__}: no gradient path (the sparse-convolution encoder is inference-only in this build). "
            "Call model.eval() and run under torch.no_grad(), or freeze this module (eval mode, input without gradient).")


class ConvBN(nn.Module):

    @staticmethod
    def run(x, conv, bn, relu, residual=None, out=None):
        if out is not None and not grad_path(x, bn, conv):
            w, b = fold_bn(conv, bn)
            y = conv_bias_act(x, w, b, conv.stride, conv.padding, conv.dilation, conv.groups, relu, residual, out=out)
            if y.data_ptr() != out.data_ptr():
                out.copy_(y)
            return out
        if out is not None:
            return out.copy_(ConvBN.run(x, conv, bn, relu, residual))
        if grad_path(x, bn, conv):
            y = bn(conv(x))
            if residual is not None:
                y = y + residual
            return F.relu(y) if relu else y
        w, b = fold_bn(conv, bn)
        return conv_bias_act(x, w, b, conv.stride, conv.padding, conv.dilation, conv.groups, relu, residual)


def conv3x3(in_planes, out_planes, stride=1, groups=1, dilation=1):
    return nn.Conv2d(in_planes, out_planes, kernel_size=3, stride=stride, padding=dilation, groups=groups,
                     bias=False, dilation=dilation)


def conv1x1(in_planes, out_planes, stride=1):
    return nn.Conv2d(in_planes, out_planes, kernel_size=1, stride=stride, bias=False)


class BasicBlock(nn.Module):
    expansion = 1

    def __init__(self, inplanes, planes, stride=1, downsample=None, groups=1, base_width=64, dilation=1,
                 norm_layer=None):
        super().__init__()
        norm_layer = norm_layer or nn.BatchNorm2d
        if groups != 1 or base_width != 64:
            raise ValueError("BasicBlock only supports groups=1 and base_width=64")
        self.conv1 = conv3x3(inplanes, planes, stride)
        self.bn1 = norm_layer(planes)
        self.relu = nn.ReLU(inplace=True)
        self.conv2 = conv3x3(planes, planes)
        self.bn2 = norm_layer(planes)
        self.downsample = downsample
        self.stride = stride

    def takes_pooled(self):
        d = self.downsample
        return (d is not None and isinstance(d[0], nn.Conv2d) and d[0].kernel_size == (1, 1) and d[0].stride == (2, 2)
                and d[0].padding == (0, 0) and d[0].out_channels == 64 and d[0].bias is None
                and self.conv1.stride == (2, 2) and self.conv1.out_channels == 64 and self.conv1.in_channels % 32 == 0
                and isinstance(self.bn1, nn.BatchNorm2d) and isinstance(d[1], nn.BatchNorm2d))

    def _stem_params(self, x):
        from heal_amd import ops
        w1, b1 = fold_bn(self.conv1, self.bn1)
        wd, bd = fold_bn(self.downsample[0], self.downsample[1])
        frag = getattr(x, "fragments", ops.stem_fragments)
        return derived("stem_block", (w1, b1, wd, bd), lambda: frag(w1, wd) + (b1, bd), (getattr(x, "weight_layout", "tiles"),))

    def forward(self, x):
        from heal_amd import ops
        if isinstance(x, (ops.PooledBEV, ops.PillarBEV)):
            if (not grad_path(None, self) and self.takes_pooled() and x.channels == self.conv1.in_channels
                    and x.stem_supported(self.conv1.out_channels, self.downsample[0].out_channels)):
                wm, wd, b1, bd = self._stem_params(x)
                out, identity = x.stem_block(wm, b1, wd, bd)
                return ConvBN.run(out, self.conv2, self.bn2, relu=True, residual=identity)
            x = x.dense()
        identity = x
        if self.downsample is not None:
            identity = ConvBN.run(x, self.downsample[0], self.downsample[1], relu=False)
        out = ConvBN.run(x, self.conv1, self.bn1, relu=True)
        return ConvBN.run(out, self.conv2, self.bn2, relu=True, residual=identity)


class Bottleneck(nn.Module):
    expansion = 4

    def __init__(self, inplanes, planes, stride=1, downsample=None, groups=1, base_width=64, dilation=1,
                 norm_layer=None, expansion=None):
        super().__init__()
        norm_layer = norm_layer or nn.BatchNorm2d
        exp = self.expansion if expansion is None else expansion
        width = int(planes * (base_width / 64.0)) * groups
        self.conv1 = conv1x1(inplanes, width)
        self.bn1 = norm_layer(width)
        self.conv2 = conv3x3(width, width, stride, groups, dilation)
        self.bn2 = norm_layer(width)
        self.conv3 = conv1x1(width, planes * exp)
        self.bn3 = norm_layer(planes * exp)
        self.relu = nn.ReLU(inplace=True)
        self.downsample = downsample
        self.stride = stride

    def _fused_params(self):
        from heal_amd import ops
        w1, b1 = fold_bn(self.conv1, self.bn1)
        w2, b2 = fold_bn(self.conv2, self.bn2)
        w3, b3 = fold_bn(self.conv3, self.bn3)
        return derived("resnext_bottleneck", (w1, b1, w2, b2, w3, b3), lambda: (
            ops.mfma_a_fragments(w1.reshape(w1.shape[0], w1.shape[1])), b1, w2, b2,
            ops.mfma_a_fragments(w3.reshape(w3.shape[0], w3.shape[1])), b3))

    def _fusable(self, x):
        import os
        if os.environ.get("HEAL_FUSED_BOTTLENECK", "0") != "1":
            return False
        from heal_amd import ops
        if not ops.experimental_build():
            return False
        c = self.conv1.in_channels
        return (x.is_cuda and self.downsample is None and self.stride == 1 and self.conv2.groups == 32
                and self.conv3.out_channels == c and self.conv1.out_channels == 2 * c and c in (64, 128, 256)
                and self.conv2.dilation == (1, 1))

    def out_shape(self, x):
        s = self.stride
        return (int(x.shape[0]), self.conv3.out_channels, (int(x.shape[2]) - 1) // s + 1, (int(x.shape[3]) - 1) // s + 1)

    def forward(self, x, out=None):
        if not grad_path(x, self) and self._fusable(x):
            from heal_amd import ops
            y = ops.resnext_bottleneck(x.contiguous(), *self._fused_params())
            return y if out is None else out.copy_(y)
        identity = x
        if self.downsample is not None:
            identity = ConvBN.run(x, self.downsample[0], self.downsample[1], relu=False)
        y = ConvBN.run(x, self.conv1, self.bn1, relu=True)
        y = ConvBN.run(y, self.conv2, self.bn2, relu=True)
        return ConvBN.run(y, self.conv3, self.bn3, relu=True, residual=identity, out=out)


class ResNetModified(nn.Module):

    def __init__(self, block, layers, layer_strides, num_filters, groups=1, width_per_group=64, inplanes=64,
                 expansion=None):
        super().__init__()
        self.inplanes = inplanes
        self.groups = groups
        self.base_width = width_per_group
        self.layernum = len(num_filters)
        self._exp = block.expansion if expansion is None else expansion
        for i in range(self.layernum):
            setattr(self, f"layer{i}", self._make_layer(block, num_filters[i], layers[i], layer_strides[i]))
        for m in self.modules():
            if isinstance(m, nn.Conv2d):
                nn.init.kaiming_normal_(m.weight, mode="fan_out", nonlinearity="relu")

    def _make_layer(self, block, planes, blocks, stride):
        exp = self._exp
        kw = {"expansion": exp} if block is Bottleneck else {}
        downsample = None
        if stride != 1 or self.inplanes != planes * exp:
            downsample = nn.Sequential(conv1x1(self.inplanes, planes * exp, stride), nn.BatchNorm2d(planes * exp))
        layers = [block(self.inplanes, planes, stride, downsample, self.groups, self.base_width, 1, None, **kw)]
        self.inplanes = planes * exp
        for _ in range(1, blocks):
            layers.append(block(self.inplanes, planes, groups=self.groups, base_width=self.base_width, **kw))
        return nn.Sequential(*layers)

    @staticmethod
    def stage_chunk(layer, x):
        mb = float(os.environ.get("HEAL_STAGE_CHUNK_MB", "0"))
        if mb <= 0 or not x.is_cuda or torch.is_grad_enabled() or not all(isinstance(b, Bottleneck) for b in layer):
            return 0
        n = int(x.shape[0])
        blk = layer[-1]
        co, s0 = blk.conv3.out_channels, layer[0].stride
        ho, wo = (int(x.shape[2]) - 1) // s0 + 1, (int(x.shape[3]) - 1) // s0 + 1
        per_agent = 4.0 * ho * wo * (2 * co + 2 * blk.conv1.out_channels) / 2 ** 20
        chunk = max(1, int(mb // per_agent))
        return chunk if chunk < n else 0

    def run_stage(self, layer, x):
        chunk = self.stage_chunk(layer, x)
        if not chunk:
            return layer(x)
        n = int(x.shape[0])
        shape = list(x.shape)
        for blk in layer:
            shape = list(blk.out_shape(torch.empty(shape, device="meta")))
        y = torch.empty(shape, dtype=x.dtype, device=x.device)
        for a in range(0, n, chunk):
            xa = x[a:a + chunk]
            for j, blk in enumerate(layer):
                xa = blk(xa, out=y[a:a + chunk]) if j == len(layer) - 1 else blk(xa)
        return y

    def forward(self, x):
        feats = []
        for i in range(self.layernum):
            x = self.run_stage(getattr(self, f"layer{i}"), x)
            feats.append(x)
        return feats


class _Deblock(nn.Sequential):

    def __init__(self, conv, bn):
        super().__init__(conv, bn, nn.ReLU())

    def out_shape(self, x):
        conv = self[0]
        if isinstance(conv, nn.ConvTranspose2d):
            return conv.out_channels, int(x.shape[2]) * conv.stride[0], int(x.shape[3]) * conv.stride[1]
        s0, s1 = conv.stride
        return conv.out_channels, (int(x.shape[2]) - conv.kernel_size[0]) // s0 + 1, (int(x.shape[3]) - conv.kernel_size[1]) // s1 + 1

    def forward(self, x, into=None):
        y = self._forward(x, into)
        if into is not None and y.data_ptr() != into[0][:, into[1]:].data_ptr():
            dst = into[0][:, into[1]:into[1] + y.shape[1]]
            dst.copy_(y)
            return dst
        return y

    def _forward(self, x, into=None):
        if grad_path(x, self):
            return super().forward(x)
        conv, bn = self[0], self[1]
        from heal_amd import ops
        if isinstance(conv, nn.ConvTranspose2d):
            w, b = fold_bn(conv, bn, transposed=True)
            k = conv.kernel_size[0]
            if (_CONV1X1 and x.is_cuda and conv.kernel_size == conv.stride and conv.kernel_size[0] == conv.kernel_size[1]
                    and conv.padding == (0, 0) and conv.output_padding == (0, 0) and conv.groups == 1
                    and ops.conv1x1_supported(int(w.shape[0]), int(w.shape[1]) * k * k, int(x.shape[2] * x.shape[3]))):
                cin, cout = int(w.shape[0]), int(w.shape[1])
                wp, bp = derived("deblock_pointwise", (w, b), lambda: (
                    w.permute(1, 2, 3, 0).reshape(cout * k * k, cin, 1, 1).contiguous(), b.repeat_interleave(k * k).contiguous()))
                if into is not None and int(x.shape[3]) % 4 == 0 and into[0].is_contiguous():
                    return ops.conv1x1_d2s(x, wp, bp, 1, k, into[0], into[1])
                y = ops.conv1x1(x, wp, bp, None, 1)
                return y if k == 1 else F.pixel_shuffle(y, k)
            y = F.conv_transpose2d(x, w, None, conv.stride, conv.padding, conv.output_padding, conv.groups)
            return ops.bias_act_(y, b, None, True)
        w, b = fold_bn(conv, bn)
        return conv_bias_act(x, w, b, conv.stride, conv.padding, 1, 1, True)


class ResNetBEVBackbone(nn.Module):

    def __init__(self, model_cfg, input_channels=64):
        super().__init__()
        self.model_cfg = model_cfg
        if "layer_nums" in model_cfg:
            layer_nums = model_cfg["layer_nums"]
            layer_strides = model_cfg["layer_strides"]
            num_filters = model_cfg["num_filters"]
            assert len(layer_nums) == len(layer_strides) == len(num_filters)
        else:
            layer_nums = layer_strides = num_filters = []
        if "upsample_strides" in model_cfg:
            assert len(model_cfg["upsample_strides"]) == len(model_cfg["num_upsample_filter"])
            num_upsample_filters = model_cfg["num_upsample_filter"]
            upsample_strides = model_cfg["upsample_strides"]
        else:
            upsample_strides = num_upsample_filters = []
        self.resnet = ResNetModified(BasicBlock, layer_nums, layer_strides, num_filters,
                                     inplanes=model_cfg.get("inplanes", 64))
        self.num_levels = len(layer_nums)
        self.deblocks = nn.ModuleList()
        for idx in range(self.num_levels):
            if len(upsample_strides) > 0:
                stride = upsample_strides[idx]
                if stride >= 1:
                    conv = nn.ConvTranspose2d(num_filters[idx], num_upsample_filters[idx], stride, stride=stride,
                                              bias=False)
                else:
                    stride = int(np.round(1 / stride))
                    conv = nn.Conv2d(num_filters[idx], num_upsample_filters[idx], stride, stride=stride, bias=False)
                self.deblocks.append(_Deblock(conv, nn.BatchNorm2d(num_upsample_filters[idx], eps=1e-3, momentum=0.01)))
        c_in = sum(num_upsample_filters)
        if len(upsample_strides) > self.num_levels:
            self.deblocks.append(_Deblock(
                nn.ConvTranspose2d(c_in, c_in, upsample_strides[-1], stride=upsample_strides[-1], bias=False),
                nn.BatchNorm2d(c_in, eps=1e-3, momentum=0.01)))
        self.num_bev_features = c_in

    def takes_pooled(self):
        first = getattr(self.resnet, "layer0", None)
        return first is not None and len(first) > 0 and isinstance(first[0], BasicBlock) and first[0].takes_pooled()

    def get_multiscale_feature(self, spatial_features):
        return self.resnet(spatial_features)

    def decode_multiscale_feature(self, x):
        ups = []
        if (len(self.deblocks) >= self.num_levels > 1 and x[0].is_cuda and not grad_path(x[0], self)
                and len({self.deblocks[i].out_shape(x[i])[1:] for i in range(self.num_levels)}) == 1):
            shapes = [self.deblocks[i].out_shape(x[i]) for i in range(self.num_levels)]
            cat = torch.empty((int(x[0].shape[0]), sum(s[0] for s in shapes), shapes[0][1], shapes[0][2]),
                              dtype=x[0].dtype, device=x[0].device)
            off = 0
            for i in range(self.num_levels):
                self.deblocks[i](x[i], into=(cat, off))
                off += shapes[i][0]
            ups = [cat]
        else:
            for i in range(self.num_levels):
                ups.append(self.deblocks[i](x[i]) if len(self.deblocks) > 0 else x[i])
        x = torch.cat(ups, dim=1) if len(ups) > 1 else ups[0]
        if len(self.deblocks) > self.num_levels:
            x = self.deblocks[-1](x)
        return x

    def get_layer_i_feature(self, spatial_features, layer_i):
        return getattr(self.resnet, f"layer{layer_i}")(spatial_features)

    def forward(self, data_dict):
        x = self.resnet(data_dict["spatial_features"])
        data_dict["spatial_features_2d"] = self.decode_multiscale_feature(x)
        return data_dict


class DoubleConv(nn.Module):

    def __init__(self, in_channels, out_channels, kernel_size, stride, padding):
        super().__init__()
        self.double_conv = nn.Sequential(
            nn.Conv2d(in_channels, out_channels, kernel_size=kernel_size, stride=stride, padding=padding),
            nn.ReLU(inplace=True),
            nn.Conv2d(out_channels, out_channels, kernel_size=3, padding=1),
            nn.ReLU(inplace=True))

    def forward(self, x):
        if grad_path(x, self):
            return self.double_conv(x)
        c0, c1 = self.double_conv[0], self.double_conv[2]
        x = conv_bias_act(x, c0.weight, c0.bias, c0.stride, c0.padding, 1, 1, True)
        return conv_bias_act(x, c1.weight, c1.bias, c1.stride, c1.padding, 1, 1, True)


class DownsampleConv(nn.Module):

    def __init__(self, config):
        super().__init__()
        self.layers = nn.ModuleList([])
        input_dim = config["input_dim"]
        for ksize, dim, stride, padding in zip(config["kernal_size"], config["dim"], config["stride"],
                                               config["padding"]):
            self.layers.append(DoubleConv(input_dim, dim, kernel_size=ksize, stride=stride, padding=padding))
            input_dim = dim

    def forward(self, x):
        for layer in self.layers:
            x = layer(x)
        return x


class LayerNorm(nn.Module):

    def __init__(self, normalized_shape, eps=1e-6, data_format="channels_last"):
        super().__init__()
        self.weight = nn.Parameter(torch.ones(normalized_shape))
        self.bias = nn.Parameter(torch.zeros(normalized_shape))
        self.eps = eps
        self.data_format = data_format
        if data_format not in ("channels_last", "channels_first"):
            raise NotImplementedError
        self.normalized_shape = (normalized_shape,)

    def forward(self, x):
        if self.data_format == "channels_last":
            return F.layer_norm(x, self.normalized_shape, self.weight, self.bias, self.eps)
        u = x.mean(1, keepdim=True)
        s = (x - u).pow(2).mean(1, keepdim=True)
        x = (x - u) / torch.sqrt(s + self.eps)
        return self.weight[:, None, None] * x + self.bias[:, None, None]


class ConvNeXtBlock(nn.Module):

    def __init__(self, dim, layer_scale_init_value=1e-6, kernel_size=7):
        super().__init__()
        self.dwconv = nn.Conv2d(dim, dim, kernel_size=kernel_size, padding=kernel_size // 2, groups=dim)
        self.norm = LayerNorm(dim, eps=1e-6)
        self.pwconv1 = nn.Linear(dim, 4 * dim)
        self.act = nn.GELU()
        self.pwconv2 = nn.Linear(4 * dim, dim)
        self.gamma = nn.Parameter(layer_scale_init_value * torch.ones((dim)), requires_grad=True) \
            if layer_scale_init_value > 0 else None

    def _folded_pw2(self):
        def build():
            w, b = self.pwconv2.weight, self.pwconv2.bias
            if self.gamma is not None:
                w, b = w * self.gamma[:, None], b * self.gamma
            return w.contiguous()[:, :, None, None], b.contiguous()
        return derived("convnext_pw2", (self.pwconv2.weight, self.pwconv2.bias, self.gamma), build)

    def forward(self, x):
        from heal_amd import ops
        inp = x
        k = self.dwconv.kernel_size[0]
        fused = x.is_cuda and not grad_path(x, self)
        if fused and k == 7 and int(x.shape[0] * x.shape[1]) <= 65535:
            x = ops.depthwise_conv(x, self.dwconv.weight, self.dwconv.bias, 1, (3, 3, 3, 3), "none")
        else:
            x = self.dwconv(x)
        if fused and ops.conv1x1_supported(x.shape[1], 4 * x.shape[1], int(x.shape[2] * x.shape[3])):
            xn = ops.layernorm_nchw(x, self.norm.weight, self.norm.bias, self.norm.eps)
            h = ops.conv1x1(xn, self.pwconv1.weight[:, :, None, None], self.pwconv1.bias, None, 3)
            w2, b2 = self._folded_pw2()
            return ops.conv1x1(h, w2, b2, inp, 0)
        x = x.permute(0, 2, 3, 1)
        x = self.pwconv2(self.act(self.pwconv1(self.norm(x))))
        if self.gamma is not None:
            x = self.gamma * x
        return inp + x.permute(0, 3, 1, 2)


class ConvNeXt(nn.Module):

    def __init__(self, args):
        super().__init__()
        if args.get("deform", False):
            raise NotImplementedError("deformable ConvNeXt aligner is out of scope (needs mmcv)")
        self.model = nn.Sequential(*[ConvNeXtBlock(args["dim"], kernel_size=args.get("kernel_size", 7))
                                     for _ in range(args["num_of_blocks"])])

    def forward(self, x):
        return self.model(x)


class AlignNet(nn.Module):

    def __init__(self, args):
        super().__init__()
        name = args["core_method"]
        if name == "identity":
            self.channel_align = nn.Identity()
        elif name == "convnext":
# ... 32 lines not shown
```

### heal_amd/ops.py

```python
import ctypes
import os

import numpy as np
import torch

from . import _capi, derived
from .derived import derived as _derived

_WS = {}

TIMING = None
SP_TRACE = None
LAST_CALLS = None


def _remember(name, fn):
    if LAST_CALLS is not None:
        LAST_CALLS[name] = fn


def graph_period_ms(fn, reps=20, iters=10):
    global TIMING, LAST_CALLS
    saved = (TIMING, LAST_CALLS)
    TIMING, LAST_CALLS = None, None
# ... 1222 lines not shown
                and self.n < (1 << 24) and bool(_capi.query("heal_sp_conv_tiles_supported", int(cin), int(cout))))

    def out_sites(self, ksize, stride, padding):
        return self.out_sites_ex(ksize, stride, padding)[:3]

    def out_sites_ex(self, ksize, stride, padding):
        out_shape = [(self.spatial_shape[d] + 2 * padding[d] - ksize[d]) // stride[d] + 1 for d in range(3)]
        K = int(ksize[0] * ksize[1] * ksize[2])
        dev = self.indices.device
        cells = self.batch_size * out_shape[0] * out_shape[1] * out_shape[2]
        worst = max(1, min(self.n * min(K, 8), cells))
        out_cap = worst if self.n_dev is None else max(1, min(worst, 2 * self._root_cap))
        out_idx = torch.empty((out_cap, 4), dtype=torch.int32, device=dev)
        n_out = torch.zeros((1,), dtype=torch.int32, device=dev)
        rank = None
        if os.environ.get("HEAL_SP_RULEBOOK", "rank") != "hash":
            nbytes = _capi.query("heal_sp_rank_bytes", _i3(out_shape), self.batch_size)
            rank = torch.empty((nbytes,), dtype=torch.uint8, device=dev)
            with _Timed("sp_rulebook"):
                _capi.call("heal_sp_out_sites_rank", _ptr(self.indices), self.n, _i3(ksize), _i3(stride), _i3(padding),
                           _i3(self.spatial_shape), _i3(out_shape), self.batch_size, _ptr(out_idx), out_cap, _ptr(n_out),
                           _ptr(rank), nbytes, _optr(self.n_dev), _ptr(sparse_overflow_flag(dev)), _stream())
        else:
            ws = _workspace("sp_out_sites", _capi.query("heal_sp_out_sites_workspace", self.n, K), dev)
            with _Timed("sp_rulebook"):
                _capi.call("heal_sp_out_sites", _ptr(self.indices), self.n, _i3(ksize), _i3(stride), _i3(padding),
                           _i3(self.spatial_shape), _i3(out_shape), self.batch_size, _ptr(out_idx), out_cap, _ptr(n_out),
                           _ptr(ws), ws.numel(), _optr(self.n_dev), _stream())
        if self.n_dev is None:
            return out_idx[:int(n_out.item())], out_shape, None, rank
        self._checks.append((n_out, out_cap))
        _SPARSE_CHECKS.append((n_out, out_cap))
        if len(_SPARSE_CHECKS) > 4096:
            del _SPARSE_CHECKS[:2048]
        return out_idx, out_shape, n_out, rank

    def conv(self, nbr, weight, bn_scale, bn_shift, relu=True, n_out_dev=None):
        weight = _need(weight, torch.float32, "weight")
        K, cin, cout = (int(v) for v in weight.shape)
        features = _need_rows(self.features, cin, "features", "SparseTensor.conv")
        if not isinstance(nbr, PairTiles):
            nbr = _need_nbr(nbr, K, "SparseTensor.conv")
        bn_scale = _need_channels(bn_scale, cout, "bn_scale", "SparseTensor.conv")
        bn_shift = _need_channels(bn_shift, cout, "bn_shift", "SparseTensor.conv")
        frag = sp_weight_fragments(weight)
        n_out = int(nbr.shape[0])
        out = torch.empty((n_out, cout), dtype=torch.float32, device=nbr.device)
        with _Timed(f"sp_conv_{cin}_{cout}") as tm:
            if isinstance(nbr, PairTiles):
                if K != 27 or not _capi.query("heal_sp_conv_tiles_supported", cin, cout):
                    raise ValueError(f"SparseTensor.conv: pair tiles do not serve a {K}-tap {cin} -> {cout} layer "
                                     "(SparseTensor.rulebook decides per layer)")
                _capi.call("heal_sp_conv_tiles", _ptr(features), _ptr(nbr.buf), n_out, nbr.slot_sites, cin, cout, _ptr(frag),
                           _ptr(bn_scale), _ptr(bn_shift), int(bool(relu)), _ptr(out), _optr(n_out_dev), _stream())
            else:
                _capi.call("heal_sp_conv", _ptr(features), _ptr(nbr), n_out, K, cin, cout, _ptr(weight), _optr(frag),
                           _ptr(bn_scale), _ptr(bn_shift), int(bool(relu)), _ptr(out), _optr(n_out_dev), _stream())
        if SP_TRACE is not None and TIMING is not None:
            SP_TRACE.append({"cin": cin, "cout": cout, "K": K, "n_in": self.n_dev if self.n_dev is not None else self.n,
                             "n_out": n_out_dev if n_out_dev is not None else n_out, "nbr": nbr, "events": (tm.e0, tm.e1)})
        return out

    def dense(self):
        C = int(self.features.shape[1])
        D, H, W = self.spatial_shape
        dev = self.indices.device
        out = torch.empty((self.batch_size, C * D, H, W), dtype=torch.float32, device=dev)
        ws = _workspace("sp_to_bev", _capi.query("heal_sp_to_bev_workspace", self.batch_size, D, H, W), dev)
        with _Timed("sp_to_bev"):
            _capi.call("heal_sp_to_bev", _ptr(self.features), _ptr(self.indices), self.n, C, _i3(self.spatial_shape),
                       self.batch_size, _ptr(out), _ptr(ws), ws.numel(), _optr(self.n_dev), _stream())
        return out


_SP_IDENT = {}


def sp_conv_raw(features, nbr, weight):
    features = _need(features, torch.float32, "features")
    weight = _need(weight, torch.float32, "weight")
    K, cin, cout = (int(v) for v in weight.shape)
    features = _need_rows(features, cin, "features", "sp_conv_raw")
    nbr = _need_nbr(nbr, K, "sp_conv_raw")
    key = (cout, str(features.device))
    ident = _SP_IDENT.get(key)
    if ident is None:
        ident = _SP_IDENT[key] = (torch.ones(cout, device=features.device), torch.zeros(cout, device=features.device))
    n_out = int(nbr.shape[0])
    out = torch.empty((n_out, cout), dtype=torch.float32, device=features.device)
    if n_out:
        _capi.call("heal_sp_conv", _ptr(features), _ptr(nbr), n_out, K, cin, cout, _ptr(weight), _optr(sp_weight_fragments(weight)),
                   _ptr(ident[0]), _ptr(ident[1]), 0, _ptr(out), None, _stream())
    return out


def sp_wgrad_supported(cin, cout):
    return 1 <= cin <= 64 and cout in (16, 32, 48, 64)


def sp_wgrad(features, grad_out, nbr):
    features = _need(features, torch.float32, "features")
    grad_out = _need(grad_out, torch.float32, "grad_out")
    nbr = _need(nbr, torch.int32, "nbr")
    if nbr.dim() != 2 or features.dim() != 2 or grad_out.dim() != 2:
        raise _capi.HealAmdError(f"sp_wgrad: features {tuple(features.shape)}, grad_out {tuple(grad_out.shape)} and nbr "
                                 f"{tuple(nbr.shape)} must be matrices")
    n_out, K = (int(v) for v in nbr.shape)
    cin, cout = int(features.shape[1]), int(grad_out.shape[1])
    if int(grad_out.shape[0]) != n_out:
        raise _capi.HealAmdError(f"sp_wgrad: grad_out has {int(grad_out.shape[0])} rows for the {n_out} output rows of nbr")
    if n_out == 0:
        return torch.zeros((K, cin, cout), dtype=torch.float32, device=features.device)
    chunks = _capi.query("heal_sp_wgrad_chunks", n_out)
    part = torch.empty((chunks, K, cin, cout), dtype=torch.float32, device=features.device)
    _capi.call("heal_sp_wgrad", _ptr(features), _ptr(grad_out), _ptr(nbr), n_out, K, cin, cout, None, _ptr(part), _stream())
    return part.sum(0)


def sp_transpose_neighbors(nbr, n_in):
    nbr = _need(nbr, torch.int32, "nbr")
    n_out, K = (int(v) for v in nbr.shape)
    nbr_t = torch.empty((int(n_in), K), dtype=torch.int32, device=nbr.device)
    _capi.call("heal_sp_transpose_neighbors", _ptr(nbr), n_out, K, int(n_in), _ptr(nbr_t), None, _stream())
    return nbr_t


def agent_attention(q, k, v, heads, scale, key_mask=None, out_rows=None, agent_major=False):
    q = _need(q, torch.float32, "q"); k = _need(k, torch.float32, "k"); v = _need(v, torch.float32, "v")
    if agent_major:
        L, n_pix, C = (int(x) for x in q.shape)
    else:
        n_pix, L, C = (int(x) for x in q.shape)
    rows = L if out_rows is None else int(out_rows)
    out = torch.empty((rows, n_pix, C) if agent_major else (n_pix, rows, C), dtype=torch.float32, device=q.device)
    if key_mask is not None:
        key_mask = _need(key_mask, torch.int32, "key_mask")
    with _Timed(f"agent_attention_h{heads}"):
        _capi.call("heal_agent_attention", _ptr(q), _ptr(k), _ptr(v), _optr(key_mask), n_pix, L, C, int(heads),
                   float(scale), rows, _ptr(out), int(bool(agent_major)), _stream())
    return out


def agent_attention_backward(q, k, v, grad_out, heads, scale, key_mask=None, agent_major=False):
    q = _need(q, torch.float32, "q"); k = _need(k, torch.float32, "k"); v = _need(v, torch.float32, "v")
    grad_out = _need(grad_out, torch.float32, "grad_out")
    if agent_major:
        L, n_pix, C = (int(x) for x in q.shape)
        rows = int(grad_out.shape[0])
    else:
        n_pix, L, C = (int(x) for x in q.shape)
        rows = int(grad_out.shape[1])
    if key_mask is not None:
        key_mask = _need(key_mask, torch.int32, "key_mask")
    gq, gk, gv = torch.empty_like(q), torch.empty_like(q), torch.empty_like(q)
    with _Timed(f"agent_attention_bwd_h{heads}"):
        _capi.call("heal_agent_attention_backward", _ptr(q), _ptr(k), _ptr(v), _optr(key_mask), _ptr(grad_out), n_pix, L, C,
                   int(heads), float(scale), rows, _ptr(gq), _ptr(gk), _ptr(gv), int(bool(agent_major)), _stream())
    return gq, gk, gv


class AgentAttention(torch.autograd.Function):

    @staticmethod
    def forward(ctx, q, k, v, heads, scale, out_rows, agent_major):
        q, k, v = q.contiguous(), k.contiguous(), v.contiguous()
        ctx.save_for_backward(q, k, v)
        ctx.cfg = (int(heads), float(scale), bool(agent_major))
        return agent_attention(q, k, v, heads, scale, out_rows=out_rows, agent_major=agent_major)

    @staticmethod
    def backward(ctx, grad_out):
        q, k, v = ctx.saved_tensors
        heads, scale, am = ctx.cfg
        gq, gk, gv = agent_attention_backward(q, k, v, grad_out.contiguous(), heads, scale, agent_major=am)
        return gq, gk, gv, None, None, None, None


def agent_attention_train_supported(q, heads):
    return bool(q.is_cuda and q.dtype == torch.float32 and q.shape[-1] == 256 and heads in (1, 4, 8, 16))


def ln_stats(x, eps):
    x = _need(x, torch.float32, "x")
    C = int(x.shape[-1])
    T = x.numel() // C
    stats = torch.empty((T, 2), dtype=torch.float32, device=x.device)
    _capi.call("heal_ln_stats", _ptr(x), T, C, float(eps), _ptr(stats), _stream())
    return stats


def linear_supported(n_tokens, n_in, n_out):
    return n_out % 128 == 0 and n_in % 32 == 0 and n_in >= 32 and n_tokens > 0


_ACT = {None: 0, "none": 0, "gelu": 1, "relu": 2}


def linear(x, weight, bias=None, stats=None, act=None, residual=None, out=None, row_map=None, parts=1, colscale=None,
           colscale_part=0, group_rows=0, bias_per_group=False, x_parts=1):
    x = _need(x, torch.float32, "x")
    weight = _need(weight, torch.float32, "weight")
    xk = int(x.shape[-1])
    K = xk * int(x_parts)
    T = x.numel() // K
    N = int(weight.shape[0])
    if int(weight.shape[1]) != K or not linear_supported(T, K, N) or N % parts or (N // parts) % 4:
        raise _capi.HealAmdError(f"linear: unsupported shape T={T} K={K} N={N} parts={parts}")
    pc = N // parts
    if out is None:
        out = torch.empty((parts, T, pc) if parts > 1 else (T, N), dtype=torch.float32, device=x.device)
    inner, outer = (int(row_map[0]), int(row_map[1])) if row_map is not None else (0, 0)
    if residual is not None:
        residual = _need(residual, torch.float32, "residual")
    with _Timed(f"linear_{K}_{N}", flops=2.0 * T * K * N, kernel_events=True):
        _capi.call("heal_linear", _ptr(x), xk, xk if x_parts > 1 else 0, T * xk, _optr(stats), _ptr(weight), _optr(bias),
                   int(bool(bias_per_group)),
                   _optr(colscale), int(colscale_part), int(group_rows), _optr(residual), N if residual is not None else 0,
                   _ptr(out), pc, T, N, K, inner, outer, pc, T * pc, _ACT[act], _stream())
    return out


def split_attn_weights(branches, groups, rows_per_group, w_out, b_out, fc1, ln_g, ln_b, eps, fc2):
    branches = _need(branches, torch.float32, "branches")
    C = int(branches.shape[-1])
    dev = branches.device
    ws = _workspace("split_attn", _capi.query("heal_split_attn_workspace", groups, rows_per_group, C), dev)
    scale = torch.empty((groups, 3, C), dtype=torch.float32, device=dev)
    bias = torch.empty((groups, C), dtype=torch.float32, device=dev)
    _capi.call("heal_split_attn_weights", _ptr(branches), int(branches.stride(0)), groups, rows_per_group, C, _ptr(w_out),
               _ptr(b_out), _ptr(fc1), _ptr(ln_g), _ptr(ln_b), float(eps), _ptr(fc2), _ptr(ws), _ptr(scale), _ptr(bias),
               _stream())
    return scale, bias


def split_attn_colsum(branches, groups, rows_per_group):
    branches = _need(branches, torch.float32, "branches")
    C = int(branches.shape[-1])
    out = torch.empty((groups, 3, (rows_per_group + 511) // 512, C), dtype=torch.float32, device=branches.device)
    _capi.call("heal_split_attn_colsum", _ptr(branches), int(branches.stride(0)), groups, rows_per_group, C, _ptr(out), _stream())
    return out


def split_attn_weights_from_colsum(colsum, rows_per_part, w_out, b_out, fc1, ln_g, ln_b, eps, fc2):
    colsum = _need(colsum, torch.float32, "colsum")
    n_parts, groups, _three, chunks, C = (int(v) for v in colsum.shape)
    if chunks != (rows_per_part + 511) // 512:
        raise ValueError(f"split_attn_weights_from_colsum: {chunks} chunks do not match {rows_per_part} rows per part")
    dev = colsum.device
    scale = torch.empty((groups, 3, C), dtype=torch.float32, device=dev)
    bias = torch.empty((groups, C), dtype=torch.float32, device=dev)
    _capi.call("heal_split_attn_weights_from_colsum", _ptr(colsum), n_parts, groups, int(rows_per_part), C, _ptr(w_out),
               _ptr(b_out), _ptr(fc1), _ptr(ln_g), _ptr(ln_b), float(eps), _ptr(fc2), _ptr(scale), _ptr(bias), _stream())
    return scale, bias


def grouped16_fragments(weight, cg):
    def build():
        C = int(weight.shape[0])
        w = weight.detach().reshape(C // 16, 16, cg, 9)
        if cg == 16:
            full = w
        else:
            full = torch.zeros((C // 16, 16, 16, 9), dtype=w.dtype, device=w.device)
            full[:, :8, :8] = w[:, :8]
            full[:, 8:, 8:] = w[:, 8:]
        return full.reshape(C // 16, 16, 4, 4, 9).permute(0, 4, 2, 3, 1).contiguous()
    return _derived("grouped16_fragments", (weight,), build)


def grouped_small_fragments(weight, cg):
    C = int(weight.shape[0])
    return _derived("grouped_small_fragments", (weight,),
                    lambda: weight.detach().reshape(C // 16, 16, cg, 9).permute(0, 3, 2, 1).contiguous())


def grouped_conv3x3(x, weight, bias, groups, stride=1, relu=True):
    import os
    x = _need(x, torch.float32, "x")
    weight = _need(weight, torch.float32, "weight")
    n, C, H, W = (int(v) for v in x.shape)
    bias = _need_bias(bias, C, "grouped_conv3x3")
    Ho, Wo = (H + 2 - 3) // stride + 1, (W + 2 - 3) // stride + 1
    y = torch.empty((n, C, Ho, Wo), dtype=torch.float32, device=x.device)
    cg = C // groups
    mode = os.environ.get("HEAL_GCONV_MFMA", "1")
    if C % 16 == 0 and W % 4 == 0 and Wo % 4 == 0 and mode in ("1", "s") and cg in (4, 8, 16):
        frag = grouped_small_fragments(weight, cg)
        with _Timed(f"grouped_conv3x3_c{C}" + ("_s2" if stride == 2 else ""), 2.0 * 9 * n * C * cg * Ho * Wo,
                    4.0 * n * C * (H * W + Ho * Wo), kernel_events=True):
            _capi.call("heal_grouped_small_conv3x3", _ptr(x), _ptr(frag), _ptr(bias), n, C, cg, H, W, int(stride),
                       int(bool(relu)), _ptr(y), _stream())
        return y
    if stride == 1 and C % 16 == 0 and W % 4 == 0 and ((cg == 16 and mode != "0") or (cg == 8 and mode == "8")):
        frag = grouped16_fragments(weight, cg)
        with _Timed(f"grouped_conv3x3_c{C}", 2.0 * 9 * n * C * cg * Ho * Wo, 4.0 * n * C * (H * W + Ho * Wo)):
            _capi.call("heal_grouped16_conv3x3", _ptr(x), _ptr(frag), _ptr(bias), n, C, H, W, int(bool(relu)), _ptr(y),
                       _stream())
        return y
    with _Timed(f"grouped_conv3x3_c{C}" + ("_s2" if stride == 2 else ""), 2.0 * 9 * n * C * (C // groups) * Ho * Wo,
                4.0 * n * C * (H * W + Ho * Wo)):
        _capi.call("heal_grouped_conv3x3", _ptr(x), _ptr(weight), _ptr(bias), n, C, int(groups), H, W, int(stride),
                   int(bool(relu)), _ptr(y), _stream())
    return y


def gconv_conv3_supported(width, cg, cout, H, W):
    return bool(_capi.query("heal_gconv_conv3_supported", int(width), int(cg), int(cout), int(H), int(W)))


def gconv_conv3(x, w2, b2, groups, w3, b3, residual=None, relu=True):
    x = _need(x, torch.float32, "x")
    n, width, H, W = (int(v) for v in x.shape)
    cg = width // groups
    cout = int(w3.shape[0])
    frag2 = grouped_small_fragments(_need(w2, torch.float32, "w2"), cg)
    frag3 = _derived("gconv_conv3_fragments", (w3,), lambda: mfma_a_fragments(w3.detach().reshape(cout, width)))
    y = torch.empty((n, cout, H, W), dtype=torch.float32, device=x.device)
    flops = 2.0 * n * H * W * (9 * width * cg + width * cout)
    nbytes = 4.0 * n * H * W * (width + cout * (2 if residual is not None else 1))
    with _Timed(f"gconv_conv3_{width}_{cout}", flops, nbytes, kernel_events=True):
        _capi.call("heal_gconv_conv3", _ptr(x), _ptr(frag2), _ptr(_need(b2, torch.float32, "b2")), _ptr(frag3),
                   _ptr(_need(b3, torch.float32, "b3")), _optr(residual), n, width, cg, cout, H, W, int(bool(relu)), _ptr(y), _stream())
    return y


def bias_act_(x, bias=None, residual=None, relu=True):
    x = _need(x, torch.float32, "x")
    n, C = int(x.shape[0]), int(x.shape[1])
    HW = int(x.shape[2] * x.shape[3])
    if residual is not None:
        residual = _need(residual, torch.float32, "residual")
    _capi.call("heal_bias_act", _ptr(x), _ptr(bias), _ptr(residual), n, C, HW, int(bool(relu)), _stream())
    return x


def mfma_a_fragments(wm):
    M, K = wm.shape
    return wm.reshape(M // 16, 16, K // 4, 4).permute(0, 2, 3, 1).reshape(M // 16, K // 4, 64).contiguous()


def conv1x1_fragments(w):
    def build():
        cout, cin = int(w.shape[0]), int(w.shape[1])
        mpad, kpad = (cout + 63) // 64 * 64, (cin + 31) // 32 * 32
        wm = w.detach().reshape(cout, cin)
        if (mpad, kpad) != (cout, cin):
            wm = torch.nn.functional.pad(wm, (0, kpad - cin, 0, mpad - cout))
        fr = mfma_a_fragments(wm)
        return fr.reshape(mpad // 16, kpad // 16, 4, 64).permute(0, 1, 3, 2).contiguous()
    return _derived("conv1x1_fragments", (w,), build)


def conv1x1_supported(cin, cout, hw, stride=1, out_w=None):
    if stride == 1:
        return hw % 4 == 0 and hw >= 64
    return stride == 2 and out_w is not None and out_w % 4 == 0 and hw >= 64


def conv1x1_ksplit(n, cin, cout, hw):
    chunks = (cin + 31) // 32
    blocks = -(-cout // 64) * -(-hw // 64) * n
    env = os.environ.get("HEAL_C1_KSPLIT")
    want = int(env) if env is not None else (min(chunks // 2, max(2, 256 // blocks)) if blocks < 128 and chunks >= 8 else 1)
    if want < 2 or chunks < 2 or hw % 4:
        return 1
    want = min(want, chunks, 65535 // n)
    return -(-chunks // -(-chunks // want))


def stem7x7_fragments(w):
    cout, cin = int(w.shape[0]), int(w.shape[1])
    if cout != 64 or tuple(w.shape[2:]) != (7, 7) or not 1 <= cin <= 4:
        raise _capi.HealAmdError(f"stem7x7: weight must be [64, 1..4, 7, 7], got {tuple(w.shape)}")

    def build():
        K = cin * 49
        ks = (K + 3) // 4
        wk = torch.nn.functional.pad(w.detach().to(torch.float32).reshape(64, K), (0, 4 * ks - K))
        return wk.reshape(4, 16, ks, 4).permute(0, 2, 3, 1).contiguous()
    return _derived("stem7x7_fragments", (w,), build)


def stem7x7(x, w, bias, pool=True):
    x = _need(x, torch.float32, "x")
    n, cx, H, W = (int(v) for v in x.shape)
    cin = int(w.shape[1])
    if cx < cin:
        raise _capi.HealAmdError(f"stem7x7: input has {cx} channels, the weight wants {cin}")
    frag = stem7x7_fragments(w)
    Hc, Wc = (H - 1) // 2 + 1, (W - 1) // 2 + 1
    Ho, Wo = ((Hc - 1) // 2 + 1, (Wc - 1) // 2 + 1) if pool else (Hc, Wc)
    y = torch.empty((n, 64, Ho, Wo), dtype=torch.float32, device=x.device)
    with _Timed(f"stem7x7_{cin}" + ("_pool" if pool else ""), 2.0 * n * 64 * cin * 49 * Hc * Wc, kernel_events=True):
        _capi.call("heal_stem7x7", _ptr(x), cx * H * W, n, cin, H, W, _ptr(frag),
                   _ptr(_need_bias(bias, 64, "stem7x7")), int(bool(pool)), _ptr(y), _stream())
    return y


def conv1x1_tiled_ok(n, cin, cout, hw):
    mode = os.environ.get("HEAL_C1_TILED", "0")
    if mode == "0" or not experimental_build() or cin % 32 or cout % 64 or hw % 4 or hw < 128:
        return False
    bm = 128 if cout % 128 == 0 else 64
    blocks = (cout // bm) * -(-hw // 128) * n
    if mode == "force":
        return True
    return blocks >= 256 and cin >= 128


def arith_products():
    a = os.environ.get("HEAL_ARITH", "")
    return {"bf16x6": 6, "bf16x9": 9}.get(a, 0)


def conv1x1_split_fragments(w):
    def build():
        cout, cin = int(w.shape[0]), int(w.shape[1])
        wm = w.detach().reshape(cout, cin).to(torch.float32)
        h = wm.to(torch.bfloat16)
        r1 = wm - h.float()
        m = r1.to(torch.bfloat16)
        lo = (r1 - m.float()).to(torch.bfloat16)
        planes = torch.stack([h, m, lo], 0)
        f = planes.reshape(3, cout // 128, 4, 32, cin // 32, 2, 2, 8)
        return f.permute(1, 4, 5, 2, 0, 6, 3, 7).contiguous()
    return _derived("conv1x1_split_fragments", (w,), build)


def _w_rowmajor(w):
    w2 = w.detach().reshape(int(w.shape[0]), int(w.shape[1]))
    return w2 if w2.is_contiguous() else w2.contiguous()


def _out_or_empty(out, shape, device, who):
    if out is None:
        return torch.empty(shape, dtype=torch.float32, device=device)
    if (tuple(out.shape) != tuple(shape) or out.dtype != torch.float32 or not out.is_cuda or not out.is_contiguous()):
        raise _capi.HealAmdError(f"{who}: `out` must be a contiguous f32 cuda tensor of shape {tuple(shape)}")
    return out


def conv1x1(x, w, bias=None, residual=None, act=0, in_scale=None, stride=1, pixel_major=False, out=None):
    x = _need(x, torch.float32, "x")
    n, cin, H, W = (int(v) for v in x.shape)
    cout = int(w.shape[0])
    bias = _need_bias(bias, cout, "conv1x1")
    Ho, Wo = (H - 1) // stride + 1, (W - 1) // stride + 1
    hard_ok = stride in (1, 2) and ((Ho * Wo) % 4 == 0 if stride == 1 else Wo % 4 == 0)
    if int(w.shape[1]) != cin or not hard_ok:
        raise _capi.HealAmdError(f"conv1x1: unsupported shape Cin={cin} Cout={cout} HxW={H}x{W} stride={stride}")
    if out is not None and pixel_major:
        raise _capi.HealAmdError("conv1x1: `out` is for the NCHW result")
    nprod = arith_products()
    if (nprod and stride == 1 and not pixel_major and in_scale is None and w.dtype == torch.float32
            and _capi.query("heal_conv1x1_split_supported", cin, cout, H, W)):
        y = _out_or_empty(out, (n, cout, H, W), x.device, "conv1x1")
        if residual is not None:
            residual = _need(residual, torch.float32, "residual")
            if tuple(residual.shape) != tuple(y.shape):
                raise _capi.HealAmdError("conv1x1: residual shape mismatch")
        frag = conv1x1_split_fragments(w)
        with _Timed(f"conv1x1_{cin}_{cout}", 2.0 * n * cin * cout * H * W,
                    4.0 * n * (cin * H * W + cout * H * W * (2 if residual is not None else 1)), kernel_events=True):
            _capi.call("heal_conv1x1_split", _ptr(x), _ptr(frag), _ptr(bias) if bias is not None else None,
                       _ptr(residual) if residual is not None else None, n, cin, cout, H, W, int(act), nprod, _ptr(y), _stream())
        return y
    if (stride == 1 and not pixel_major and in_scale is None and conv1x1_tiled_ok(n, cin, cout, H * W)
            and w.dtype == torch.float32):
        y = _out_or_empty(out, (n, cout, H, W), x.device, "conv1x1")
        if residual is not None:
            residual = _need(residual, torch.float32, "residual")
            if tuple(residual.shape) != tuple(y.shape):
                raise _capi.HealAmdError("conv1x1: residual shape mismatch")
        wr = _w_rowmajor(w)
        with _Timed(f"conv1x1_{cin}_{cout}", 2.0 * n * cin * cout * H * W,
                    4.0 * n * (cin * H * W + cout * H * W * (2 if residual is not None else 1))):
            _capi.call("heal_conv1x1_tiled", _ptr(x), _ptr(wr), _ptr(bias) if bias is not None else None,
                       _ptr(residual) if residual is not None else None, n, cin, cout, H, W, int(act), 0, 0, 0, _ptr(y), _stream())
        return y
    frag = conv1x1_fragments(w)
    if pixel_major:
        if residual is not None or cout % 4 != 0:
            raise _capi.HealAmdError("conv1x1: pixel-major output needs Cout % 4 == 0 and takes no residual")
        y = torch.empty((n, Ho * Wo, cout), dtype=torch.float32, device=x.device)
    else:
        y = _out_or_empty(out, (n, cout, Ho, Wo), x.device, "conv1x1")
    if residual is not None:
        residual = _need(residual, torch.float32, "residual")
        if tuple(residual.shape) != tuple(y.shape):
            raise _capi.HealAmdError("conv1x1: residual shape mismatch")
    if in_scale is not None:
        in_scale = _need(in_scale.reshape(n, cin), torch.float32, "in_scale")
    ksplit = conv1x1_ksplit(n, cin, cout, H * W) if (stride == 1 and not pixel_major) else 1
    if ksplit > 1:
        nbytes = _capi.query("heal_conv1x1_splitk_workspace", n, cout, H, W, ksplit)
        ws = _workspace("conv1x1_splitk", nbytes, x.device)
        with _Timed(f"conv1x1_{cin}_{cout}", 2.0 * n * cin * cout * H * W,
                    4.0 * n * (cin * H * W + cout * H * W * (2 if residual is not None else 1)), kernel_events=True):
            _capi.call("heal_conv1x1_splitk", _ptr(x), _ptr(frag), _ptr(bias) if bias is not None else None,
                       _ptr(residual) if residual is not None else None, _ptr(in_scale) if in_scale is not None else None,
                       n, cin, cout, H, W, int(act), ksplit, _ptr(y), _ptr(ws), ws.numel(), _stream())
        return y
    with _Timed(f"conv1x1_{cin}_{cout}" + ("_s2" if stride == 2 else ""), 2.0 * n * cin * cout * Ho * Wo,
                4.0 * n * (cin * Ho * Wo + cout * Ho * Wo * (2 if residual is not None else 1)), kernel_events=True):
        _capi.call("heal_conv1x1", _ptr(x), _ptr(frag), _ptr(bias) if bias is not None else None,
                   _ptr(residual) if residual is not None else None, _ptr(in_scale) if in_scale is not None else None,
                   n, cin, cout, H, W, int(stride), int(act), int(bool(pixel_major)), _ptr(y), _stream())
    return y


def conv1x1_d2s(x, w, bias, act, k, dst, channel_offset):
    x = _need(x, torch.float32, "x")
    dst = _need(dst, torch.float32, "dst")
    n, cin, H, W = (int(v) for v in x.shape)
    cout = int(w.shape[0])
    if (not dst.is_contiguous() or int(dst.shape[0]) != n or int(dst.shape[2]) != H * k or int(dst.shape[3]) != W * k
            or cout % (k * k) or W % 4):
        raise _capi.HealAmdError(f"conv1x1_d2s: destination {tuple(dst.shape)} does not fit x {tuple(x.shape)} at k={k}")
    bias = _need_bias(bias, cout, "conv1x1_d2s")
    if conv1x1_tiled_ok(n, cin, cout, H * W) and w.dtype == torch.float32:
        wr = _w_rowmajor(w)
        with _Timed(f"conv1x1_{cin}_{cout}", 2.0 * n * cin * cout * H * W, 4.0 * n * H * W * (cin + cout)):
            _capi.call("heal_conv1x1_tiled", _ptr(x), _ptr(wr), _ptr(bias) if bias is not None else None, None, n, cin, cout, H, W,
                       int(act), int(k), int(dst.shape[1]), int(channel_offset), _ptr(dst), _stream())
        return dst[:, channel_offset:channel_offset + cout // (k * k)]
    frag = conv1x1_fragments(w)
    with _Timed(f"conv1x1_{cin}_{cout}", 2.0 * n * cin * cout * H * W, 4.0 * n * H * W * (cin + cout), kernel_events=True):
        _capi.call("heal_conv1x1_d2s", _ptr(x), _ptr(frag), _ptr(bias) if bias is not None else None, n, cin, cout, H, W,
                   int(act), int(k), int(dst.shape[1]), int(channel_offset), _ptr(dst), _stream())
    return dst[:, channel_offset:channel_offset + cout // (k * k)]


def conv3x3_fragments(w):
    def build():
        cout, cin = int(w.shape[0]), int(w.shape[1])
        mpad, kpad = (cout + 63) // 64 * 64, (cin + 7) // 8 * 8
        wm = w.detach().reshape(cout, cin, 9)
        if (mpad, kpad) != (cout, cin):
            wm = torch.nn.functional.pad(wm, (0, 0, 0, kpad - cin, 0, mpad - cout))
        return wm.reshape(mpad // 64, 4, 16, kpad // 8, 2, 4, 9).permute(0, 3, 6, 4, 1, 5, 2).contiguous()
    return _derived("conv3x3_fragments", (w,), build)


def conv3x3_same(x, w, bias, stride, pad, act="none"):
    x = _need(x, torch.float32, "x")
    n, cin, H, W = (int(v) for v in x.shape)
    cout = int(w.shape[0])
    pl, pr, pt, pb = (int(v) for v in pad)
    Ho, Wo = (H + pt + pb - 3) // stride + 1, (W + pl + pr - 3) // stride + 1
    if pl not in (0, 1) or pt not in (0, 1) or pr > 1 or pb > 1 or tuple(w.shape[1:]) != (cin, 3, 3):
        raise _capi.HealAmdError(f"conv3x3_same: unsupported padding {pad} / weight {tuple(w.shape)}")
    frag = conv3x3_fragments(w)
    y = torch.empty((n, cout, Ho, Wo), dtype=torch.float32, device=x.device)
    with _Timed(f"conv3x3_{cin}_{cout}_s{stride}same", 2.0 * 9 * n * cin * cout * Ho * Wo, 4.0 * n * (cin * H * W + cout * Ho * Wo),
                kernel_events=True):
        _capi.call("heal_conv3x3_same", _ptr(x), _ptr(frag), _ptr(_need_bias(bias, cout, "conv3x3_same")),
                   n, cin, cout, H, W, int(stride), pt, pl, Ho, Wo, {"none": 0, "relu": 1, "silu": 2}[act], _ptr(y), _stream())
    return y


def conv3x3_winograd_waves(n=1, cout=64, H=256, W=256):
    import os
    e = os.environ.get("HEAL_WG_WAVES", "")
    if e in ("4", "8"):
        return int(e)
    blocks8 = n * ((cout + 63) // 64) * ((H + 15) // 16) * ((W + 15) // 16)
    return 8 if blocks8 >= 512 else 4


def conv3x3_winograd_kc(cin, waves, H=1, W=1):
    import os
    want = os.environ.get("HEAL_WG_KC", _WG_KC_DEFAULT)
    ok16 = (want == "16" and waves == 8 and cin % 16 == 0 and 16 * H * W * 4 < 2 ** 31 and experimental_build())
    return 16 if ok16 else 8


def experimental_build():
    return hasattr(_capi.lib(), "heal_gconv_conv3")


_WG_KC_DEFAULT = "8"


def conv3x3_winograd_fragments(w, waves=8, kc=8):
    def build():
        cout, cin = int(w.shape[0]), int(w.shape[1])
        mpad, kpad = (cout + 63) // 64 * 64, (cin + kc - 1) // kc * kc
        G = torch.tensor([[1.0, 0.0, 0.0], [0.5, 0.5, 0.5], [0.5, -0.5, 0.5], [0.0, 0.0, 1.0]], dtype=torch.float64,
                         device=w.device)
        U = (G @ w.detach().double() @ G.t()).float().reshape(cout, cin, 16)
        if (mpad, kpad) != (cout, cin):
            U = torch.nn.functional.pad(U, (0, 0, 0, kpad - cin, 0, mpad - cout))
        return U.reshape(mpad // 64, 4, 16, kpad // kc, kc // 4, 4, waves, 16 // waves).permute(0, 3, 6, 5, 2, 7, 4, 1).contiguous()
    return _derived("conv3x3_winograd_fragments", (w,), build, (waves, kc))


def conv3x3_winograd4_fragments(w):
    def build():
        cout, cin = int(w.shape[0]), int(w.shape[1])
        mpad, kpad = (cout + 31) // 32 * 32, (cin + 15) // 16 * 16
        G = torch.tensor([[1 / 4, 0, 0], [-1 / 6, -1 / 6, -1 / 6], [-1 / 6, 1 / 6, -1 / 6], [1 / 24, 1 / 12, 1 / 6],
                          [1 / 24, -1 / 12, 1 / 6], [0, 0, 1]], dtype=torch.float64, device=w.device)
        U = (G @ w.detach().double() @ G.t()).float().reshape(cout, cin, 36)
        if (mpad, kpad) != (cout, cin):
            U = torch.nn.functional.pad(U, (0, 0, 0, kpad - cin, 0, mpad - cout))
        return U.reshape(mpad // 32, 2, 16, kpad // 16, 4, 4, 4, 9).permute(0, 3, 1, 6, 5, 2, 7, 4).contiguous()
# ... 204 lines not shown
```

### include/heal_amd.h

```cpp
#ifndef HEAL_AMD_H
#define HEAL_AMD_H

#include <stddef.h>
#include <stdint.h>

#ifdef __cplusplus
extern "C" {
#endif

#define HEAL_AMD_ABI_VERSION 9

int heal_abi_version(void);
const char* heal_last_error(void);

int heal_fill_bytes(void* dst, int byte, size_t bytes, void* stream);
int heal_next_launch_events(void* start_event, void* stop_event);

size_t heal_voxelize_workspace(int n_points, int max_points, int max_voxels, long long agents_x_cells);
int heal_voxelize(const float* points, int n_points,
                  const float* range_host, const float* voxel_size_host,
                  int max_points, int max_voxels, int batch_idx,
                  float* voxels, int32_t* coords, int32_t* num_points, int32_t* n_voxels,
                  const int32_t* row_offset, int32_t* row_offset_next,
                  void* ws, size_t ws_bytes, int tables_clean, void* stream);

size_t heal_voxelize_batch_workspace(int n_points_total, int n_agents, int max_points, int max_voxels, long long agents_x_cells);
int heal_voxelize_batch(const float* points, const int32_t* point_offsets_host, int n_agents,
                        const float* range_host, const float* voxel_size_host, int max_points, int max_voxels,
                        float* voxels, int32_t* coords, int32_t* num_points, int32_t* row_offsets,
                        void* ws, size_t ws_bytes, int tables_clean, void* stream);

int heal_mask_points(const float* points, int n_points, const float* range_host, int mask_ego, float* out,
                     void* stream);

size_t heal_pfn_scatter_workspace(int n_voxels, int n_agents, int ny, int nx, int channels);
int heal_pfn_scatter(const float* voxels, const int32_t* coords, const int32_t* num_points,
                     int n_voxels, const int32_t* n_voxels_dev, int max_points,
                     const float* weight, const float* bn_scale, const float* bn_shift, int channels,
                     float vx, float vy, float vz, float x_offset, float y_offset, float z_offset,
                     int n_agents, int ny, int nx,
                     float* canvas, float* pillar_feat,
                     void* ws, size_t ws_bytes, void* stream);

int heal_pfn_pillars(const float* voxels, const int32_t* coords, const int32_t* num_points, int n_voxels,
                     const int32_t* n_voxels_dev, int max_points, const float* weight, const float* bn_scale,
                     const float* bn_shift, int channels, float vx, float vy, float vz, float x_offset, float y_offset,
                     float z_offset, int n_agents, int ny, int nx, float* pillar_feat, int32_t* cell_map, void* stream);
int heal_pillar_canvas(const int32_t* cell_map, const float* pillar_feat, int n_agents, int channels, int ny, int nx,
                       float* canvas, void* stream);
int heal_pillar_stem_block(const float* pillar_feat, const int32_t* cell_map, int n_agents, int channels, int ny, int nx,
                           const float* w_main, const float* b_main, const float* w_down, const float* b_down,
                           int weight_layout, float* out_main, float* out_identity, void* stream);

int heal_warp_fuse(const float* feats, const float* occ, int n_agents, int channels, int H, int W,
                   const double* affine_host, const double* affine_dev, int grid_f64,
                   const int32_t* crop_host, float* out, void* stream);

int heal_warp_fuse_levels(int n_levels, const float* const* feats_host, const float* const* occ_host, int n_agents,
                          const int32_t* channels_host, const int32_t* h_host, const int32_t* w_host,
                          const double* affine_host, const double* affine_dev, int grid_f64, const int32_t* crop_host,
                          float* const* out_host, void* stream);

int heal_warp_fuse_backward(const float* feats, const float* occ, int n_agents, int channels, int H, int W,
                            const double* affine_host, const double* affine_dev, int grid_f64, const int32_t* crop_host,
                            const float* grad_out, float* grad_feats, float* grad_occ, void* stream);

int heal_warp_agent(const float* feat, const float* occ, int channels, int H, int W,
                    const double* affine_host, const double* affine_dev, int grid_f64,
                    const int32_t* crop_host, float* feat_ego, float* score_ego, void* stream);
int heal_warp_agents_pm(const float* feats, int n_agents, int channels, int H, int W, const double* affine_host,
                        const double* affine_dev, int grid_f64, float* out, void* stream);
int heal_fuse_warped(const float* feats_ego, const float* scores_ego, int n_agents, int channels,
                     int H, int W, float* out, void* stream);
int heal_fuse_warped_rows(const float* base, const int64_t* feat_offsets_host, const int64_t* score_offsets_host,
                          int n_agents, int channels, int H, int W, float* out, void* stream);

size_t heal_decode_nms_workspace(int anchors_total, int nms_top);
int heal_decode_nms(const float* cls, const float* reg, const float* dir, const float* anchors,
                    int H, int W, int anchor_num, int num_bins,
                    float score_thr, float dir_offset, float nms_thr, int nms_top,
                    const float* tfm_host, const float* gt_range_host,
                    float* out_corners, float* out_scores, int32_t* out_count, int max_out,
                    void* ws, size_t ws_bytes, void* stream);

int heal_quad_iou(const float* a, int n, const float* b, int m, float* iou, void* stream);

int heal_camera_matrices(const float* rots, const float* trans, const float* intrins, const float* post_rots,
                         const float* post_trans, int n_cameras, float* cam_mats, void* stream);
size_t heal_bev_pool_workspace(int n_agents, int n_cams, int D, int fH, int fW, int channels,
                               int nx, int ny, int nz);
int heal_bev_pool(const float* depth_logit, const float* feat, const float* frustum,
                  const float* cam_mats, int n_agents, int n_cams, int D, int fH, int fW, int channels,
                  const float* dx_host, const float* bx_host, const int32_t* nx_host,
                  float* out, void* ws, size_t ws_bytes, void* stream);
size_t heal_bev_pool_pm_workspace(int n_agents, int channels, int nx, int ny, int nz);
int heal_bev_pool_scatter(const float* head, int head_stride, const float* frustum, const float* cam_mats, int n_agents,
                          int n_cams, int D, int fH, int fW, int channels, const float* dx_host, const float* bx_host,
                          const int32_t* nx_host, void* ws, size_t ws_bytes, void* stream);

int heal_bev_pool_emit(int n_agents, int channels, const int32_t* nx_host, float* out, void* ws, size_t ws_bytes,
                       void* stream);
int heal_bev_stem_block(int n_agents, int channels, const int32_t* nx_host, const float* w_main, const float* b_main,
                        const float* w_down, const float* b_down, float* out_main, float* out_identity, void* ws,
                        size_t ws_bytes, void* stream);
int heal_bev_pool_pm(const float* head, int head_stride, const float* frustum, const float* cam_mats, int n_agents,
                     int n_cams, int D, int fH, int fW, int channels, const float* dx_host, const float* bx_host,
                     const int32_t* nx_host, float* out, void* ws, size_t ws_bytes, void* stream);

int heal_pfn_train_blocks(int n_voxels);
int heal_pfn_features(const float* voxels, const int32_t* coords, const int32_t* num_points, int n_voxels, int max_points,
                      const float* weight, const float* bn_scale, const float* bn_shift, float vx, float vy, float vz,
                      float x_offset, float y_offset, float z_offset, float* pillar_feat, void* stream);
int heal_pfn_moments(const float* voxels, const int32_t* coords, const int32_t* num_points, int n_voxels, int max_points,
                     float vx, float vy, float vz, float x_offset, float y_offset, float z_offset, float* partials, void* stream);
int heal_pfn_backward(const float* voxels, const int32_t* coords, const int32_t* num_points, int n_voxels, int max_points,
                      const float* weight, const float* bn_scale, const float* bn_shift, const float* mean, const float* rstd,
                      float vx, float vy, float vz, float x_offset, float y_offset, float z_offset, const float* grad_pillar,
                      float* partials, void* stream);

int heal_mean_vfe(const float* voxels, const int32_t* num_points, int n_voxels, int max_points, int n_feat,
                  float* out, const int32_t* n_dev, void* stream);
size_t heal_sp_sort_workspace(int n);
int heal_sp_sort_sites(const int32_t* indices, int n, const int32_t* shape_host, int batch,
                       int32_t* sorted_indices, int32_t* perm, void* ws, size_t ws_bytes, const int32_t* n_dev,
                       void* stream);
int heal_sp_gather_rows(const float* features, const int32_t* perm, int n, int channels, const int32_t* n_dev, float* out,
                        void* stream);
size_t heal_sp_table_capacity(int n);
int heal_sp_hash_build(const int32_t* indices, int n, const int32_t* shape_host, int batch,
                       uint32_t* table_keys, int32_t* table_vals, size_t table_cap, const int32_t* n_dev,
                       void* stream);
int heal_sp_neighbors(const int32_t* out_indices, int n_out, const int32_t* ksize_host,
                      const int32_t* stride_host, const int32_t* padding_host, const int32_t* in_shape_host,
                      const int32_t* out_shape_host, int batch, const uint32_t* table_keys,
                      const int32_t* table_vals, size_t table_cap, int32_t* nbr, const int32_t* n_out_dev,
                      void* stream);
size_t heal_sp_out_sites_workspace(int n_in, int kernel_volume);
int heal_sp_out_sites(const int32_t* in_indices, int n_in, const int32_t* ksize_host,
                      const int32_t* stride_host, const int32_t* padding_host, const int32_t* in_shape_host,
                      const int32_t* out_shape_host, int batch, int32_t* out_indices, int out_cap,
                      int32_t* n_out, void* ws, size_t ws_bytes, const int32_t* n_in_dev, void* stream);
size_t heal_sp_rank_bytes(const int32_t* shape_host, int batch);
int heal_sp_out_sites_rank(const int32_t* in_indices, int n_in, const int32_t* ksize_host,
                           const int32_t* stride_host, const int32_t* padding_host, const int32_t* in_shape_host,
                           const int32_t* out_shape_host, int batch, int32_t* out_indices, int out_cap,
                           int32_t* n_out, void* rank, size_t rank_bytes, const int32_t* n_in_dev,
                           int32_t* overflow , void* stream);
int heal_sp_neighbors_rank(const int32_t* out_indices, int n_out, const int32_t* ksize_host,
                           const int32_t* stride_host, const int32_t* padding_host, const int32_t* in_shape_host,
                           const int32_t* out_shape_host, int batch, const void* rank, size_t rank_bytes,
                           int n_in, const int32_t* n_in_dev, int32_t* nbr, const int32_t* n_out_dev, void* stream);
size_t heal_sp_root_rank_bytes(const int32_t* shape_host, int batch);
int heal_sp_root_rank(const int32_t* indices, int n, const int32_t* shape_host, int batch, int32_t* sorted_indices,
                      int32_t* perm, const float* features , int channels,
                      float* sorted_features , void* rank,
                      size_t rank_bytes, const int32_t* n_dev, void* stream);
int heal_sp_neighbors_root(const int32_t* out_indices, int n_out, const int32_t* ksize_host,
                           const int32_t* stride_host, const int32_t* padding_host, const int32_t* in_shape_host,
                           const int32_t* out_shape_host, int batch, const void* rank, size_t rank_bytes,
                           int n_in, const int32_t* n_in_dev, int32_t* nbr, const int32_t* n_out_dev, void* stream);
size_t heal_sp_pair_tiles_words(int n_out, int slot_sites);
int heal_sp_neighbor_tiles(const int32_t* out_indices, int n_out, const int32_t* ksize_host, const int32_t* stride_host,
                           const int32_t* padding_host, const int32_t* in_shape_host, const int32_t* out_shape_host,
                           int batch, const void* rank, size_t rank_bytes, int root, int n_in, const int32_t* n_in_dev,
                           int slot_sites, uint32_t* tiles, const int32_t* n_out_dev, void* stream);
int heal_sp_tiles_to_neighbors(const uint32_t* tiles, int n_out, int slot_sites, const int32_t* n_out_dev, int32_t* nbr,
                               void* stream);
int heal_sp_conv_tiles_supported(int c_in, int c_out);
int heal_sp_conv_tiles(const float* feat_in, const uint32_t* tiles, int n_out, int slot_sites, int c_in, int c_out,
                       const float* weight_frag, const float* bn_scale, const float* bn_shift, int relu, float* feat_out,
                       const int32_t* n_out_dev, void* stream);
int heal_sp_transpose_neighbors(const int32_t* nbr, int n_out, int kernel_volume, int n_in, int32_t* nbr_t,
                                const int32_t* n_out_dev, void* stream);
int heal_sp_wgrad_chunks(int n_out);
int heal_sp_wgrad(const float* feat_in, const float* grad_out, const int32_t* nbr, int n_out, int kernel_volume, int c_in,
                  int c_out, const int32_t* n_out_dev, float* partials, void* stream);
int heal_sp_weight_fragments(const float* weight, int kernel_volume, int c_in, int c_out, float* out, void* stream);
int heal_sp_conv(const float* feat_in, const int32_t* nbr, int n_out, int kernel_volume, int c_in, int c_out,
                 const float* weight, const float* weight_frag, const float* bn_scale, const float* bn_shift,
                 int relu, float* feat_out, const int32_t* n_out_dev, void* stream);
size_t heal_sp_to_bev_workspace(int batch, int D, int H, int W);
int heal_sp_to_bev(const float* features, const int32_t* indices, int n, int channels,
                   const int32_t* shape_host, int batch, float* out, void* ws, size_t ws_bytes,
                   const int32_t* n_dev, void* stream);

int heal_bev_pool_backward(const float* grad_cells, const float* depth_logit, const float* feat, const float* frustum,
                           const float* cam_mats, int n_agents, int n_cams, int D, int fH, int fW, int channels,
                           const float* dx_host, const float* bx_host, const int32_t* nx_host, float* grad_logit,
                           float* grad_feat, void* stream);

int heal_agent_attention(const float* q, const float* k, const float* v, const int32_t* key_mask, int n_pix,
                         int n_agents, int channels, int heads, float scale, int out_rows, float* out,
                         int agent_major ,
                         void* stream);
int heal_agent_attention_backward(const float* q, const float* k, const float* v, const int32_t* key_mask,
                                  const float* grad_out, int n_pix, int n_agents, int channels, int heads, float scale,
                                  int out_rows, float* grad_q, float* grad_k, float* grad_v, int agent_major, void* stream);

int heal_grouped_conv3x3(const float* x, const float* weight, const float* bias, int n, int channels, int groups,
                         int H, int W, int stride, int relu, float* y, void* stream);
int heal_bias_act(float* x, const float* bias, const float* residual, int n, int channels, int HW, int relu,
                  void* stream);

int heal_upsample2x_bilinear(const float* x, int n, int channels, int H, int W, float* y, void* stream);

int heal_depthwise_conv(const float* x, const float* weight, const float* bias, int n, int channels, int H, int W,
                        int ksize, int stride, int pad_t, int pad_l, int Ho, int Wo, int act, float* y,
                        float* channel_sums, void* stream);

int heal_layernorm_nchw(const float* x, const float* gamma, const float* beta, int n, int channels, int HW, float eps,
                        float* y, void* stream);

int heal_channel_dot(const float* x, const float* weight, const float* bias, int n, int channels, int HW, float* y,
                     void* stream);

int heal_se_gate(const float* mean, const float* w_reduce, const float* b_reduce, const float* w_expand_t,
                 const float* b_expand, int n, int channels, int squeezed, float scale, int tiles, float* gate,
                 void* stream);

int heal_conv1x1(const float* x, const float* weight_frag, const float* bias, const float* residual,
                 const float* in_scale, int n, int cin, int cout, int H, int W, int stride, int act,
                 int out_pixel_major, float* y, void* stream);

int heal_conv3x3_same(const float* x, const float* weight_frag, const float* bias, int n, int cin, int cout, int H, int W,
                      int stride, int pad_t, int pad_l, int Ho, int Wo, int act, float* y, void* stream);

int heal_stem7x7(const float* x, long long image_stride, int n, int cin, int H, int W, const float* weight_frag,
                 const float* bias, int pool, float* y, void* stream);
int heal_conv1x1_split_supported(int cin, int cout, int H, int W);
int heal_conv1x1_split(const float* x, const void* weight_frag, const float* bias, const float* residual, int n, int cin, int cout,
                       int H, int W, int act, int n_products, float* y, void* stream);
size_t heal_conv1x1_splitk_workspace(int n, int cout, int H, int W, int ksplit);
int heal_conv1x1_splitk(const float* x, const float* weight_frag, const float* bias, const float* residual,
                        const float* in_scale, int n, int cin, int cout, int H, int W, int act, int ksplit, float* y, void* ws,
                        size_t ws_bytes, void* stream);

int heal_conv1x1_d2s(const float* x, const float* weight_frag, const float* bias, int n, int cin, int cout, int H, int W,
                     int act, int k, int dst_channels, int dst_channel_offset, float* y, void* stream);

int heal_conv3x3(const float* x, const float* weight_frag, const float* bias, const float* residual, int n, int cin,
                 int cout, int H, int W, int stride, int relu, float* y, void* stream);

int heal_conv_gemm(const float* x, const float* weight_tap_major, const float* bias, const float* residual, int n, int cin,
                   int cout, int H, int W, int ksize, int stride, int relu, float* y, void* stream);

int heal_grouped16_conv3x3(const float* x, const float* weight_frag, const float* bias, int n, int channels, int H, int W,
                           int relu, float* y, void* stream);

int heal_grouped_small_conv3x3(const float* x, const float* weight_q, const float* bias, int n, int channels,
                               int group_channels, int H, int W, int stride, int relu, float* y, void* stream);

int heal_conv3x3_winograd(const float* x, const float* u_frag, const float* bias, const float* residual, int n, int cin,
                          int cout, int H, int W, int relu, int waves, float* y, void* stream);
int heal_conv3x3_winograd_kc(const float* x, const float* u_frag, const float* bias, const float* residual, int n, int cin,
                             int cout, int H, int W, int relu, int waves, int kc, float* y, void* stream);
size_t heal_conv3x3_winograd_splitk_workspace(int n, int cout, int H, int W, int ksplit);
int heal_conv3x3_winograd_splitk(const float* x, const float* u_frag, const float* bias, const float* residual, int n, int cin,
                                 int cout, int H, int W, int relu, int waves, int ksplit, float* y, void* ws, size_t ws_bytes,
                                 void* stream);

int heal_boxes_bev_matrix(const float* boxes_a, int n, const float* boxes_b, int m, int mode, float* out,
                          void* stream);
size_t heal_nms_bev_workspace(int n);
int heal_nms_bev(const float* boxes_sorted, int n, float thresh, int rotated, void* workspace,
                 size_t workspace_bytes, long long* keep, int* num_keep, void* stream);

size_t heal_nms_quads_workspace(int n);
int heal_nms_quads(const float* quads_sorted, int n, float thresh, void* workspace, size_t workspace_bytes,
                   long long* keep, int* num_keep, void* stream);

int heal_window_attention(const float* qkv, const float* pos_bias, int n_agents, int H, int W, int heads,
                          int dim_head, int window, float scale, float* out, void* stream);
size_t heal_window_attention_backward_workspace(int n_agents, int H, int W, int heads);
int heal_window_attention_backward(const float* qkv, const float* pos_bias, const float* out, const float* grad_out, int n_agents,
                                   int H, int W, int heads, int dim_head, int window, float scale, float* grad_qkv,
                                   float* grad_bias, void* ws, size_t ws_bytes, void* stream);

int heal_agent_window_attention(const float* qkv, const float* bias, int n_agents, int n_valid, int H, int W, int heads,
                                int dim_head, int window, int mode, float scale, float* out, void* stream);
int heal_agent_mean(const float* x, int n_agents, long long n_elems, float* out, void* stream);

size_t heal_v2v_message_workspace(int n_ego, int cout, int H, int W, int nsplit);
int heal_v2v_message(const float* xs, const float* mask, const float* e, long long e_stride, const float* w_frag,
                     const float* residual, int n_ego, int n_agents, int cin, int cout, int H, int W, int mode, int nsplit,
                     int tile_h, float* out, void* ws, size_t ws_bytes, void* stream);
int heal_gru_zero_state(const float* gates, long long gates_stride, const float* add, long long add_stride, int n, int channels,
                        int H, int W, float* h, void* stream);

int heal_ln_stats(const float* x, int n_tokens, int channels, float eps, float* stats, void* stream);
int heal_linear(const float* x, int lda, int x_part_cols, long long x_part_stride, const float* ln_stats,
                const float* weight, const float* bias,
                int bias_per_group, const float* colscale, int colscale_part, int group_rows, const float* residual,
                int ldr, float* out, int ldo, int n_tokens, int n_out, int n_in, int map_inner, int map_outer,
                int part_cols, long long part_stride, int act, void* stream);
size_t heal_split_attn_workspace(int groups, int rows_per_group, int channels);
int heal_split_attn_weights(const float* branches, long long part_stride, int groups, int rows_per_group, int channels,
                            const float* w_out, const float* b_out, const float* fc1, const float* ln_gamma,
                            const float* ln_beta, float eps, const float* fc2, float* colsum_ws, float* scale,
                            float* bias, void* stream);
int heal_split_attn_colsum(const float* branches, long long part_stride, int groups, int rows_per_group, int channels,
                           float* colsum, void* stream);
int heal_split_attn_weights_from_colsum(const float* colsum, int n_parts, int groups, int rows_per_part, int channels,
                                        const float* w_out, const float* b_out, const float* fc1, const float* ln_gamma,
                                        const float* ln_beta, float eps, const float* fc2, float* scale, float* bias,
                                        void* stream);

size_t heal_label_assign_workspace(int n_gt);
int heal_label_assign(const float* anchor_boxes, int n_anchors, const float* gt_boxes, int n_gt,
                      float pos_threshold, float neg_threshold, int32_t* assigned, uint8_t* neg, void* ws,
                      size_t ws_bytes, void* stream);

#ifdef __cplusplus
}
#endif
#endif
```

Baseline: 162.6.

## Add multi-image batched conv1x1 and grouped conv3x3 kernels over strided regions

Adds 'images' variants of the conv1x1 and small-group grouped conv3x3 kernels. One launch walks a table of up to eight image regions, each with its own offsets, pitches and store window, and a tile-to-image lookup. The ResNeXt bottleneck now runs its convolutions through these variants, so differently sized or cropped feature maps are processed in one launch without compaction copies, and the final conv can write straight into a window of the destination. The cost is extra per-thread index arithmetic, non-contiguous loads, and partial-window scalar stores.

```diff
diff --git a/heal_amd/_capi.py b/heal_amd/_capi.py
--- a/heal_amd/_capi.py
+++ b/heal_amd/_capi.py
@@ -132,6 +132,10 @@
     "heal_layernorm_nchw": (c_int, [c_void_p] * 3 + [c_int] * 3 + [c_float, c_void_p, c_void_p]),
     "heal_se_gate": (c_int, [c_void_p] * 5 + [c_int] * 3 + [c_float, c_int, c_void_p, c_void_p]),
     "heal_conv1x1": (c_int, [c_void_p] * 5 + [c_int] * 8 + [c_void_p, c_void_p]),
+    "heal_conv1x1_images": (c_int, [c_void_p] * 5 + [c_int] * 5 + [c_void_p, c_void_p]),
+    "heal_grouped_small_conv3x3_images": (c_int, [c_void_p] * 4 + [c_int] * 5 + [c_void_p, c_void_p]),
+    "heal_images_plan": (c_int, [c_void_p] + [c_int] * 4 + [c_void_p]),
+    "heal_images_locate": (c_int, [c_void_p, c_int, c_int]),
     "heal_stem7x7": (c_int, [c_void_p, ctypes.c_longlong, c_int, c_int, c_int, c_int, c_void_p, c_void_p, c_int, c_void_p, c_void_p]),
     "heal_conv1x1_split_supported": (c_int, [c_int] * 4),
     "heal_conv1x1_split": (c_int, [c_void_p] * 4 + [c_int] * 7 + [c_void_p, c_void_p]),
@@ -175,6 +179,14 @@
     pass
 
 
+IMAGES_MAX = 8
+
+
+class ImageDesc(ctypes.Structure):
+    _fields_ = ([(k, ctypes.c_longlong) for k in ("x_off", "y_off", "r_off")]
+                + [(k, c_int) for k in ("x_row", "x_chan", "y_row", "y_chan", "r_row", "r_chan", "H", "W", "wy0", "wy1", "wx0", "wx1")])
+
+
 def declared_symbols(experimental=False):
     text = open(HEADER_EXPERIMENTAL if experimental else HEADER).read()
     text = re.sub(r"/\*.*?\*/", "", text, flags=re.S)
diff --git a/heal_amd/csrc/common.h b/heal_amd/csrc/common.h
--- a/heal_amd/csrc/common.h
+++ b/heal_amd/csrc/common.h
@@ -116,4 +116,14 @@
     return o;
 }
 
+#define HEAL_MAX_IMAGES 8
+template <typename D>
+__host__ __device__ inline int images_locate(const D* d, int n, int tile) {
+    int img = 0;
+#pragma unroll
+    for (int i = 1; i < HEAL_MAX_IMAGES; ++i)
+        if (i < n && tile >= d[i].tile0) img = i;
+    return img;
 }
+
+}
diff --git a/heal_amd/csrc/conv1x1.hip b/heal_amd/csrc/conv1x1.hip
--- a/heal_amd/csrc/conv1x1.hip
+++ b/heal_amd/csrc/conv1x1.hip
@@ -6,13 +6,22 @@
 
 using f32x4 = __attribute__((ext_vector_type(4))) float;
 
-template <int BM, int BN, int KC, int STRIDE>
-__global__ __launch_bounds__(256) void k_conv1x1(const float* __restrict__ x, const float* __restrict__ wfrag,
-                                                const float* __restrict__ bias, const float* __restrict__ res,
-                                                const float* __restrict__ in_scale, int Cin, int Kpad, int Cout,
-                                                int HW, int Wo, int in_W, int in_HW, int act, int out_pm,
-                                                int d2s_k, int d2s_ctot, int d2s_coff, int n_img, int ksplit,
-                                                float* __restrict__ y) {
+struct C1Image {
+    long long x_off, y_off, r_off;
+    int x_row, x_chan, y_row, y_chan, r_row, r_chan;
+    int Ho, Wo;
+    int wy0, wy1, wx0, wx1;
+    int tile0;
+};
+struct C1Images { C1Image d[HEAL_MAX_IMAGES]; int n; };
+
+template <int BM, int BN, int KC, int STRIDE, bool IMG>
+__device__ __forceinline__ void conv1x1_body(const float* __restrict__ x, const float* __restrict__ wfrag,
+                                             const float* __restrict__ bias, const float* __restrict__ res,
+                                             const float* __restrict__ in_scale, int Cin, int Kpad, int Cout,
+                                             int HW, int Wo, int in_W, int in_HW, int act, int out_pm,
+                                             int d2s_k, int d2s_ctot, int d2s_coff, int n_img, int ksplit,
+                                             float* __restrict__ y, const C1Images* __restrict__ tab) {
     constexpr int MT = BM / 64;
     constexpr int NT = BN / 16;
     constexpr int LD = BN + 16;
@@ -23,16 +32,28 @@
     static_assert(NPASS >= 1 && KC % RPP == 0, "bad staging shape");
     __shared__ __attribute__((aligned(16))) float sB[2][KC][LD];
     const Block3 bk = xcd_block();
-    const int m0 = bk.x * BM, p0 = bk.y * BN, n = bk.z % n_img, kpart = bk.z / n_img;
+    const int m0 = bk.x * BM, n = bk.z % n_img, kpart = bk.z / n_img;
+    int p0 = bk.y * BN;
     const int wave = threadIdx.x >> 6, l = threadIdx.x & 63;
     const int lk = l >> 4, ln = l & 15;
-    const float* __restrict__ xin = x + (size_t)n * Cin * in_HW;
+    const C1Image* __restrict__ D = nullptr;
+    if constexpr (IMG) {
+        D = tab->d + images_locate(tab->d, tab->n, (int)bk.y);
+        p0 = ((int)bk.y - D->tile0) * BN;
+        HW = D->Ho * D->Wo; Wo = D->Wo;
+    }
+    const float* __restrict__ xin = IMG ? x + D->x_off : x + (size_t)n * Cin * in_HW;
     const int ksteps = Kpad / 4;
     const int nchunks_all = Kpad / KC, cps = (nchunks_all + ksplit - 1) / ksplit;
     const int cbeg = kpart * cps, nchunks = min(cbeg + cps, nchunks_all);
     const float* __restrict__ scl = in_scale ? in_scale + (size_t)n * Cin : nullptr;
     const int sp = (threadIdx.x % TPR) * 4, sc = threadIdx.x / TPR;
     const bool pix_ok = p0 + sp < HW;
+    size_t img_src = 0;
+    if constexpr (IMG) {
+        const int p = pix_ok ? p0 + sp : 0, oy = p / Wo, ox = p - oy * Wo;
+        img_src = (size_t)(oy * STRIDE) * D->x_row + ox * STRIDE;
+    }
 
     f32x4 acc[MT][NT];
 #pragma unroll
@@ -47,7 +68,11 @@
             const int ch = c * KC + sc + RPP * i;
             if (pix_ok && ch < Cin) {
                 float4 v;
-                if constexpr (STRIDE == 1) {
+                if constexpr (IMG) {
+                    const float* src = xin + (size_t)ch * D->x_chan + img_src;
+                    if constexpr (STRIDE == 1) v = *reinterpret_cast<const float4*>(src);
+                    else v = make_float4(src[0], src[STRIDE], src[2 * STRIDE], src[3 * STRIDE]);
+                } else if constexpr (STRIDE == 1) {
                     v = *reinterpret_cast<const float4*>(xin + (size_t)ch * HW + p0 + sp);
                 } else {
                     const int p = p0 + sp, oy = p / Wo, ox = p - oy * Wo;
@@ -116,7 +141,7 @@
             for (int ks = 0; ks < KS; ++ks) a_cur[mt][ks] = a_nxt[mt][ks];
     }
 
-    if (out_pm == 1) {
+    if (!IMG && out_pm == 1) {
         float* __restrict__ yout = y + (size_t)n * HW * Cout;
 #pragma unroll
         for (int mt = 0; mt < MT; ++mt) {
@@ -141,9 +166,22 @@
         }
         return;
     }
-    float* __restrict__ yout = y + ((size_t)kpart * n_img + n) * Cout * HW;
-    const float* __restrict__ rin = res ? res + (size_t)n * Cout * HW : nullptr;
+    float* __restrict__ yout = IMG ? y + D->y_off : y + ((size_t)kpart * n_img + n) * Cout * HW;
+    const float* __restrict__ rin = res ? (IMG ? res + D->r_off : res + (size_t)n * Cout * HW) : nullptr;
     constexpr int NG = NT / 4;
+    size_t img_dst[NG], img_res[NG];
+    int img_mode[NG], img_ox[NG];
+    if constexpr (IMG) {
+#pragma unroll
+        for (int gq = 0; gq < NG; ++gq) {
+            const int p = p0 + gq * 64 + 4 * ln, pc = p < HW ? p : 0, oy = pc / Wo, ox = pc - oy * Wo;
+            img_dst[gq] = (size_t)oy * D->y_row + ox;
+            img_res[gq] = (size_t)oy * D->r_row + ox;
+            img_ox[gq] = ox;
+            img_mode[gq] = (p >= HW || oy < D->wy0 || oy >= D->wy1 || ox + 4 <= D->wx0 || ox >= D->wx1) ? 0
+                           : (ox >= D->wx0 && ox + 4 <= D->wx1) ? 1 : 2;
+        }
+    }
 #pragma unroll
     for (int mt = 0; mt < MT; ++mt) {
         float4 rq[4][NG];
@@ -153,7 +191,8 @@
 #pragma unroll
                 for (int gq = 0; gq < NG; ++gq) {
                     const int co = min(m0 + (wave * MT + mt) * 16 + lk * 4 + r, Cout - 1), p = min(p0 + gq * 64 + 4 * ln, HW - 4);
-                    rq[r][gq] = *reinterpret_cast<const float4*>(rin + (size_t)co * HW + p);
+                    if constexpr (IMG) rq[r][gq] = *reinterpret_cast<const float4*>(rin + (size_t)co * D->r_chan + img_res[gq]);
+                    else rq[r][gq] = *reinterpret_cast<const float4*>(rin + (size_t)co * HW + p);
                 }
         }
 #pragma unroll
@@ -180,7 +219,18 @@
                     v.z = 0.5f * v.z * (1.f + erff(v.z * 0.70710678118654752f));
                     v.w = 0.5f * v.w * (1.f + erff(v.w * 0.70710678118654752f));
                 }
-                if (out_pm != 2) {
+                if constexpr (IMG) {
+                    float* dst = yout + (size_t)co * D->y_chan + img_dst[gq];
+                    if (img_mode[gq] == 1) {
+                        *reinterpret_cast<float4*>(dst) = v;
+                    } else if (img_mode[gq] == 2) {
+                        const int ox = img_ox[gq];
+                        if (ox >= D->wx0 && ox < D->wx1) dst[0] = v.x;
+                        if (ox + 1 >= D->wx0 && ox + 1 < D->wx1) dst[1] = v.y;
+                        if (ox + 2 >= D->wx0 && ox + 2 < D->wx1) dst[2] = v.z;
+                        if (ox + 3 >= D->wx0 && ox + 3 < D->wx1) dst[3] = v.w;
+                    }
+                } else if (out_pm != 2) {
                     *reinterpret_cast<float4*>(yout + o) = v;
                 } else {
                     const int kk = d2s_k * d2s_k, Ho = HW / Wo;
@@ -199,6 +249,23 @@
     }
 }
 
+template <int BM, int BN, int KC, int STRIDE>
+__global__ __launch_bounds__(256) void k_conv1x1(const float* __restrict__ x, const float* __restrict__ wfrag,
+                                                const float* __restrict__ bias, const float* __restrict__ res,
+                                                const float* __restrict__ in_scale, int Cin, int Kpad, int Cout,
+                                                int HW, int Wo, int in_W, int in_HW, int act, int out_pm,
+                                                int d2s_k, int d2s_ctot, int d2s_coff, int n_img, int ksplit,
+                                                float* __restrict__ y) {
+    conv1x1_body<BM, BN, KC, STRIDE, false>(x, wfrag, bias, res, in_scale, Cin, Kpad, Cout, HW, Wo, in_W, in_HW, act, out_pm, d2s_k,
+                                            d2s_ctot, d2s_coff, n_img, ksplit, y, nullptr);
+}
+
+template <int BM, int BN, int KC, int STRIDE>
+__global__ __launch_bounds__(256) void k_conv1x1_images(const float* __restrict__ x, const float* __restrict__ wfrag,
+                                                       const float* __restrict__ bias, const float* __restrict__ res, int Cin,
+                                                       int Kpad, int Cout, int act, float* __restrict__ y, const C1Images tab) {
+    conv1x1_body<BM, BN, KC, STRIDE, true>(x, wfrag, bias, res, nullptr, Cin, Kpad, Cout, 0, 0, 0, 0, act, 0, 1, 0, 0, 1, 1, y, &tab);
+}
 
 __global__ __launch_bounds__(256) void k_conv1x1_splitk_reduce(const float4* __restrict__ part, const float* __restrict__ bias,
                                                               const float4* __restrict__ res, int ksplit, int Cout, int HW4,
@@ -238,6 +305,13 @@
     HEAL_LAUNCH_CHECK();
     return 0;
 }
+}
+
+struct C1Cfg { bool set; int bm, bn, kc; };
+static C1Cfg c1_cfg_from_env() {
+    C1Cfg c{false, 64, 64, 32};
+    if (const char* e = getenv("HEAL_C1_CFG")) c.set = sscanf(e, "%d,%d,%d", &c.bm, &c.bn, &c.kc) == 3;
+    return c;
 }
 
 static int conv1x1_launch(const float* x, const float* weight_frag, const float* bias, const float* residual,
@@ -258,10 +332,8 @@
     }
     hipStream_t s = (hipStream_t)stream;
     int bm = 64, bn = 64, kc = 32;
-    if (const char* e = getenv("HEAL_C1_CFG")) {
-        int a_ = 0, b_ = 0, c_ = 0;
-        if (stride == 1 && sscanf(e, "%d,%d,%d", &a_, &b_, &c_) == 3) { bm = a_; bn = b_; kc = c_; }
-    }
+    static const C1Cfg cfg = c1_cfg_from_env();
+    if (stride == 1 && cfg.set) { bm = cfg.bm; bn = cfg.bn; kc = cfg.kc; }
     HEAL_REQUIRE(mpad % bm == 0, "conv1x1: padded Cout %d not a multiple of the tile height %d", mpad, bm);
 #define HEAL_C1(BM_, BN_, KC_, ST_)                                                                              \
     if (bm == BM_ && bn == BN_ && kc == KC_ && stride == ST_) {                                                  \
@@ -299,6 +371,90 @@
     HEAL_REQUIRE(out_pixel_major == 0 || out_pixel_major == 1, "conv1x1: out_pixel_major must be 0 or 1");
     return conv1x1_launch(x, weight_frag, bias, residual, in_scale, n, cin, cout, H, W, stride, act, out_pixel_major, 1, 0, 0,
                           y, stream);
+}
+
+namespace heal { int gconv_small_image_tiles(int group_channels, int stride, int H, int W); }
+
+static const int C1_IMAGES_BN = 64;
+
+extern "C" int heal_images_plan(const heal_image_desc* images, int n_images, int kind, int stride, int group_channels, int* tile0) {
+    HEAL_REQUIRE(images && tile0 && n_images >= 1 && n_images <= HEAL_MAX_IMAGES, "images_plan: 1..%d images (got %d)", HEAL_MAX_IMAGES,
+                 n_images);
+    HEAL_REQUIRE((kind == 0 || kind == 1) && (stride == 1 || stride == 2), "images_plan: kind 0 | 1, stride 1 | 2");
+    HEAL_REQUIRE(kind == 0 || group_channels == 4 || group_channels == 8 || group_channels == 16, "images_plan: 4, 8 or 16 channels per group");
+    long long t = 0;
+    for (int i = 0; i < n_images; ++i) {
+        HEAL_REQUIRE(images[i].H >= 1 && images[i].W >= 1, "images_plan: image %d is empty", i);
+        tile0[i] = (int)t;
+        const int Ho = (images[i].H - 1) / stride + 1, Wo = (images[i].W - 1) / stride + 1;
+        t += kind == 0 ? ceil_div(Ho * Wo, C1_IMAGES_BN) : gconv_small_image_tiles(group_channels, stride, images[i].H, images[i].W);
+        HEAL_REQUIRE(t < (1ll << 30), "images_plan: grid limit");
+    }
+    tile0[n_images] = (int)t;
+    return 0;
+}
+
+extern "C" int heal_images_locate(const int* tile0, int n_images, int tile) {
+    if (!tile0 || n_images < 1 || n_images > HEAL_MAX_IMAGES || tile < 0 || tile >= tile0[n_images]) return -1;
+    struct T { int tile0; } d[HEAL_MAX_IMAGES];
+    for (int i = 0; i < n_images; ++i) d[i].tile0 = tile0[i];
+    return images_locate(d, n_images, tile);
+}
+
+extern "C" int heal_conv1x1_images(const float* x, const float* weight_frag, const float* bias, const float* residual,
+                                   const heal_image_desc* images, int n_images, int cin, int cout, int stride, int act, float* y,
+                                   void* stream) {
+    HEAL_REQUIRE(images && n_images >= 1 && n_images <= HEAL_MAX_IMAGES, "conv1x1_images: 1..%d images (got %d)", HEAL_MAX_IMAGES, n_images);
+    HEAL_REQUIRE(cin >= 1 && cout >= 1, "conv1x1_images: bad shape");
+    HEAL_REQUIRE(stride == 1 || stride == 2, "conv1x1_images: stride must be 1 or 2 (got %d)", stride);
+    HEAL_REQUIRE(act >= 0 && act <= 3, "conv1x1_images: act must be 0 (none), 1 (ReLU), 2 (SiLU) or 3 (GELU)");
+    HEAL_REQUIRE(x && weight_frag && y, "conv1x1_images: null pointer");
+    HEAL_REQUIRE(((uintptr_t)x & 15) == 0 && ((uintptr_t)y & 15) == 0 && ((uintptr_t)residual & 15) == 0,
+                 "conv1x1_images: x, y and residual must be 16-B aligned");
+    const int kpad = (cin + 31) / 32 * 32, mpad = (cout + 63) / 64 * 64;
+    C1Images tab;
+    long long tiles = 0;
+    for (int i = 0; i < n_images; ++i) {
+        const heal_image_desc& s = images[i];
+        C1Image& d = tab.d[i];
+        HEAL_REQUIRE(s.H >= 1 && s.W >= 1, "conv1x1_images: image %d is empty", i);
+        const int Ho = (s.H - 1) / stride + 1, Wo = (s.W - 1) / stride + 1;
+        HEAL_REQUIRE(Wo % 4 == 0 && (stride == 2 || s.W % 4 == 0), "conv1x1_images: image %d: output width %d must be a multiple of 4", i, Wo);
+        HEAL_REQUIRE(s.x_off >= 0 && s.y_off >= 0 && s.y_off % 4 == 0 && s.y_row % 4 == 0 && s.y_chan % 4 == 0 &&
+                     (stride == 2 || (s.x_off % 4 == 0 && s.x_row % 4 == 0 && s.x_chan % 4 == 0)),
+                     "conv1x1_images: image %d: offsets / pitches must be multiples of 4 elements", i);
+        HEAL_REQUIRE(s.x_row >= s.W && s.y_row >= Wo && (long long)s.x_chan >= (long long)(s.H - 1) * s.x_row + s.W &&
+                     (long long)s.y_chan >= (long long)(Ho - 1) * s.y_row + Wo,
+                     "conv1x1_images: image %d: region %dx%d does not fit its pitches", i, s.H, s.W);
+        if (residual)
+            HEAL_REQUIRE(s.r_off >= 0 && s.r_off % 4 == 0 && s.r_row % 4 == 0 && s.r_chan % 4 == 0 && s.r_row >= Wo &&
+                         (long long)s.r_chan >= (long long)(Ho - 1) * s.r_row + Wo,
+                         "conv1x1_images: image %d: residual offsets / pitches must be multiples of 4 and hold the region", i);
+        const bool whole = (s.wy0 | s.wy1 | s.wx0 | s.wx1) == 0;
+        HEAL_REQUIRE(whole || (0 <= s.wy0 && s.wy0 < s.wy1 && s.wy1 <= Ho && 0 <= s.wx0 && s.wx0 < s.wx1 && s.wx1 <= Wo),
+                     "conv1x1_images: image %d: store window [%d,%d)x[%d,%d) outside the %dx%d output", i, s.wy0, s.wy1, s.wx0, s.wx1, Ho, Wo);
+        d.x_off = s.x_off; d.y_off = s.y_off; d.r_off = residual ? s.r_off : 0;
+        d.x_row = s.x_row; d.x_chan = s.x_chan; d.y_row = s.y_row; d.y_chan = s.y_chan;
+        d.r_row = residual ? s.r_row : 0; d.r_chan = residual ? s.r_chan : 0;
+        d.Ho = Ho; d.Wo = Wo;
+        d.wy0 = whole ? 0 : s.wy0; d.wy1 = whole ? Ho : s.wy1; d.wx0 = whole ? 0 : s.wx0; d.wx1 = whole ? Wo : s.wx1;
+        d.tile0 = (int)tiles;
+        tiles += ceil_div(Ho * Wo, C1_IMAGES_BN);
+        HEAL_REQUIRE(tiles <= 65535, "conv1x1_images: %lld pixel tiles exceed the grid limit", tiles);
+    }
+    for (int i = n_images; i < HEAL_MAX_IMAGES; ++i) tab.d[i] = tab.d[0];
+    tab.n = n_images;
+    hipStream_t s = (hipStream_t)stream;
+    const LaunchEvents ev = take_launch_events();
+    const dim3 grid(mpad / 64, (unsigned)tiles, 1);
+    if (stride == 1)
+        HEAL_LAUNCH_EV2((k_conv1x1_images<64, 64, 32, 1>), grid, dim3(256), 0, s, ev.start, ev.stop, x, weight_frag, bias, residual, cin,
+                        kpad, cout, act, y, tab);
+    else
+        HEAL_LAUNCH_EV2((k_conv1x1_images<64, 64, 32, 2>), grid, dim3(256), 0, s, ev.start, ev.stop, x, weight_frag, bias, residual, cin,
+                        kpad, cout, act, y, tab);
+    HEAL_LAUNCH_CHECK();
+    return 0;
 }
 
 extern "C" int heal_conv1x1_d2s(const float* x, const float* weight_frag, const float* bias, int n, int cin, int cout, int H,
diff --git a/heal_amd/csrc/gconv_small.hip b/heal_amd/csrc/gconv_small.hip
--- a/heal_amd/csrc/gconv_small.hip
+++ b/heal_amd/csrc/gconv_small.hip
@@ -6,10 +6,18 @@
 
 using f32x4 = __attribute__((ext_vector_type(4))) float;
 
-template <int CG, int TH, int STRIDE>
-__global__ __launch_bounds__(256) __attribute__((amdgpu_waves_per_eu(3, 4))) void k_gconv_small(
+struct GsImage {
+    long long x_off, y_off;
+    int x_row, x_chan, y_row, y_chan;
+    int H, W, Ho, Wo;
+    int tile0;
+};
+struct GsImages { GsImage d[HEAL_MAX_IMAGES]; int n; };
+
+template <int CG, int TH, int STRIDE, bool IMG>
+__device__ __forceinline__ void gconv_small_body(
     const float* __restrict__ x, const float* __restrict__ wq, const float* __restrict__ bias, int C, int H, int W, int Ho,
-    int Wo, int tiles_x, int relu, float* __restrict__ y) {
+    int Wo, int tiles_x, int relu, float* __restrict__ y, const GsImages* __restrict__ tab) {
     static_assert(CG == 4 || CG == 8 || CG == 16, "4, 8 or 16 channels per group");
     static_assert(TH == 8 || TH == 16, "tile height");
     static_assert(STRIDE == 1 || STRIDE == 2, "stride");
@@ -24,11 +32,23 @@
     __shared__ float4 sW[NSTEP * 16 / 4];
     const Block3 bk = xcd_block();
     const int sg = bk.y, n = bk.z;
-    const int ty = bk.x / tiles_x, tx = bk.x - ty * tiles_x;
+    unsigned tile = bk.x;
+    int xrow = W, yrow = Wo;
+    size_t HW = (size_t)H * W, HWo = (size_t)Ho * Wo;
+    if constexpr (IMG) {
+        const int img = images_locate(tab->d, tab->n, (int)bk.x);
+        const GsImage& D = tab->d[img];
+        tile -= (unsigned)D.tile0;
+        H = D.H; W = D.W; Ho = D.Ho; Wo = D.Wo;
+        constexpr int TWI = STRIDE == 1 ? 32 : 16;
+        tiles_x = (Wo + TWI - 1) / TWI;
+        xrow = D.x_row; yrow = D.y_row; HW = (size_t)D.x_chan; HWo = (size_t)D.y_chan;
+        x += D.x_off; y += D.y_off;
+    }
+    const int ty = tile / tiles_x, tx = tile - ty * tiles_x;
     const int oy0 = ty * TH, ox0 = tx * TW;
     const int gy0 = oy0 * STRIDE - 1, gx0 = ox0 * STRIDE;
     const int t = threadIdx.x, wave = t >> 6, l = t & 63;
-    const size_t HW = (size_t)H * W, HWo = (size_t)Ho * Wo;
     const float* __restrict__ xin = x + ((size_t)n * C + (size_t)sg * 16) * HW;
 
     constexpr int N_IN = PR * 8 * 4, IT_IN = (N_IN + 255) / 256;
@@ -43,7 +63,7 @@
         const int gy = gy0 + row, gx = gx0 + quad * 4;
         const bool ok = gy >= 0 && gy < H && gx < W;
         ok_bits |= ok ? (1u << it) : 0u;
-        const float* src = xin + (size_t)(gq * 4) * HW + (ok ? (size_t)gy * W + gx : 0);
+        const float* src = xin + (size_t)(gq * 4) * HW + (ok ? (size_t)gy * xrow + gx : 0);
         vin[it][0] = *reinterpret_cast<const float4*>(src);
         vin[it][1] = *reinterpret_cast<const float4*>(src + HW);
         vin[it][2] = *reinterpret_cast<const float4*>(src + 2 * HW);
@@ -56,7 +76,7 @@
         const int gy = gy0 + row, gx = side ? gx0 + 32 : gx0 - 1;
         const bool ok = gy >= 0 && gy < H && gx >= 0 && gx < W;
         ok_bits |= ok ? 256u : 0u;
-        const float* src = xin + (size_t)(gq * 4) * HW + (ok ? (size_t)gy * W + gx : 0);
+        const float* src = xin + (size_t)(gq * 4) * HW + (ok ? (size_t)gy * xrow + gx : 0);
         vha = make_float4(src[0], src[HW], src[2 * HW], src[3 * HW]);
     }
     constexpr int N_W4 = NSTEP * 16 / 4, IT_W = (N_W4 + 255) / 256;
@@ -139,14 +159,89 @@
             if (oy >= Ho || ox >= Wo) continue;
             float4 v = make_float4(acc[o][s][0] + bv0, acc[o][s][1] + bv0, acc[o][s][2] + bv0, acc[o][s][3] + bv0);
             if (relu) { v.x = fmaxf(v.x, 0.f); v.y = fmaxf(v.y, 0.f); v.z = fmaxf(v.z, 0.f); v.w = fmaxf(v.w, 0.f); }
-            *reinterpret_cast<float4*>(yout + (size_t)oy * Wo + ox) = v;
+            *reinterpret_cast<float4*>(yout + (size_t)oy * yrow + ox) = v;
         }
     }
 }
 
+template <int CG, int TH, int STRIDE>
+__global__ __launch_bounds__(256) __attribute__((amdgpu_waves_per_eu(3, 4))) void k_gconv_small(
+    const float* __restrict__ x, const float* __restrict__ wq, const float* __restrict__ bias, int C, int H, int W, int Ho,
+    int Wo, int tiles_x, int relu, float* __restrict__ y) {
+    gconv_small_body<CG, TH, STRIDE, false>(x, wq, bias, C, H, W, Ho, Wo, tiles_x, relu, y, nullptr);
+}
+
+template <int CG, int TH, int STRIDE>
+__global__ __launch_bounds__(256) __attribute__((amdgpu_waves_per_eu(3, 4))) void k_gconv_small_images(
+    const float* __restrict__ x, const float* __restrict__ wq, const float* __restrict__ bias, int C, int relu,
+    float* __restrict__ y, const GsImages tab) {
+    gconv_small_body<CG, TH, STRIDE, true>(x, wq, bias, C, 0, 0, 0, 0, 1, relu, y, &tab);
+}
+
 }
 
 using namespace heal;
+
+static int gs_tile_height(int group_channels, int stride) {
+    int th = (group_channels == 4 && stride == 1) ? 16 : 8;
+    if (const char* e = getenv("HEAL_GS_TH")) th = atoi(e) == 8 ? 8 : atoi(e) == 16 ? 16 : th;
+    if (stride == 2 || group_channels == 16) th = 8;
+    return th;
+}
+
+namespace heal {
+int gconv_small_image_tiles(int group_channels, int stride, int H, int W) {
+    const int Ho = (H - 1) / stride + 1, Wo = (W - 1) / stride + 1;
+    return ceil_div(Wo, stride == 1 ? 32 : 16) * ceil_div(Ho, gs_tile_height(group_channels, stride));
+}
+}
+
+extern "C" int heal_grouped_small_conv3x3_images(const float* x, const float* weight_q, const float* bias,
+                                                 const heal_image_desc* images, int n_images, int channels, int group_channels,
+                                                 int stride, int relu, float* y, void* stream) {
+    HEAL_REQUIRE(group_channels == 4 || group_channels == 8 || group_channels == 16,
+                 "grouped_small_conv3x3_images: 4, 8 or 16 channels per group (got %d)", group_channels);
+    HEAL_REQUIRE(stride == 1 || stride == 2, "grouped_small_conv3x3_images: stride must be 1 or 2 (got %d)", stride);
+    HEAL_REQUIRE(images && n_images >= 1 && n_images <= HEAL_MAX_IMAGES, "grouped_small_conv3x3_images: 1..%d images (got %d)",
+                 HEAL_MAX_IMAGES, n_images);
+    HEAL_REQUIRE(channels >= 16 && channels % 16 == 0 && channels / 16 <= 65535,
+                 "grouped_small_conv3x3_images: channels %% 16 == 0 (got %d)", channels);
+    HEAL_REQUIRE(x && weight_q && y && ((uintptr_t)x & 15) == 0 && ((uintptr_t)y & 15) == 0,
+                 "grouped_small_conv3x3_images: bad pointer (x, y must be 16-B aligned)");
+    GsImages tab;
+    long long tiles = 0;
+    for (int i = 0; i < n_images; ++i) {
+        const heal_image_desc& s = images[i];
+        GsImage& d = tab.d[i];
+        const int Ho = (s.H - 1) / stride + 1, Wo = (s.W - 1) / stride + 1;
+        HEAL_REQUIRE(s.H >= 1 && s.W >= 4 && s.W % 4 == 0 && Wo % 4 == 0,
+                     "grouped_small_conv3x3_images: image %d: W %% 4 == 0 and an output width %% 4 == 0 (got %dx%d)", i, s.H, s.W);
+        HEAL_REQUIRE(s.x_off >= 0 && s.y_off >= 0 && s.x_off % 4 == 0 && s.y_off % 4 == 0 && s.x_row % 4 == 0 && s.y_row % 4 == 0 &&
+                     s.x_chan % 4 == 0 && s.y_chan % 4 == 0, "grouped_small_conv3x3_images: image %d: offsets / pitches must be multiples of 4", i);
+        HEAL_REQUIRE(s.x_row >= s.W && s.y_row >= Wo && (long long)s.x_chan >= (long long)(s.H - 1) * s.x_row + s.W &&
+                     (long long)s.y_chan >= (long long)(Ho - 1) * s.y_row + Wo,
+                     "grouped_small_conv3x3_images: image %d: region %dx%d does not fit its pitches", i, s.H, s.W);
+        HEAL_REQUIRE((s.wy0 | s.wy1 | s.wx0 | s.wx1) == 0 || (s.wy0 == 0 && s.wx0 == 0 && s.wy1 == Ho && s.wx1 == Wo),
+                     "grouped_small_conv3x3_images: image %d: a store window is for heal_conv1x1_images only", i);
+        d.x_off = s.x_off; d.y_off = s.y_off; d.x_row = s.x_row; d.x_chan = s.x_chan; d.y_row = s.y_row; d.y_chan = s.y_chan;
+        d.H = s.H; d.W = s.W; d.Ho = Ho; d.Wo = Wo; d.tile0 = (int)tiles;
+        tiles += gconv_small_image_tiles(group_channels, stride, s.H, s.W);
+        HEAL_REQUIRE(tiles < (1ll << 30), "grouped_small_conv3x3_images: grid limit");
+    }
+    for (int i = n_images; i < HEAL_MAX_IMAGES; ++i) tab.d[i] = tab.d[0];
+    tab.n = n_images;
+    const int th = gs_tile_height(group_channels, stride);
+    const dim3 grid((unsigned)tiles, channels / 16, 1);
+    hipStream_t s_ = (hipStream_t)stream;
+#define HEAL_GSI(CG_, TH_, ST_)                                                                                       \
+    if (group_channels == CG_ && th == TH_ && stride == ST_)                                                          \
+        HEAL_LAUNCH_EV((k_gconv_small_images<CG_, TH_, ST_>), grid, dim3(256), 0, s_, x, weight_q, bias, channels, relu, y, tab);
+    HEAL_GSI(4, 16, 1) HEAL_GSI(4, 8, 1) HEAL_GSI(8, 16, 1) HEAL_GSI(8, 8, 1)
+    HEAL_GSI(4, 8, 2) HEAL_GSI(8, 8, 2) HEAL_GSI(16, 8, 1) HEAL_GSI(16, 8, 2)
+#undef HEAL_GSI
+    HEAL_LAUNCH_CHECK();
+    return 0;
+}
 
 extern "C" int heal_grouped_small_conv3x3(const float* x, const float* weight_q, const float* bias, int n, int channels,
                                           int group_channels, int H, int W, int stride, int relu, float* y, void* stream) {
@@ -159,9 +254,7 @@
                  channels, W);
     HEAL_REQUIRE(x && weight_q && y && ((uintptr_t)x & 15) == 0 && ((uintptr_t)y & 15) == 0,
                  "grouped_small_conv3x3: bad pointer (x, y must be 16-B aligned)");
-    int th = (group_channels == 4 && stride == 1) ? 16 : 8;
-    if (const char* e = getenv("HEAL_GS_TH")) th = atoi(e) == 8 ? 8 : atoi(e) == 16 ? 16 : th;
-    if (stride == 2 || group_channels == 16) th = 8;
+    const int th = gs_tile_height(group_channels, stride);
     const int tw = stride == 1 ? 32 : 16;
     const int tiles_x = ceil_div(Wo, tw), tiles_y = ceil_div(Ho, th);
     HEAL_REQUIRE(channels / 16 <= 65535 && n <= 65535, "grouped_small_conv3x3: grid limit");
diff --git a/heal_amd/opencood/models/fuse_modules/pyramid_fuse.py b/heal_amd/opencood/models/fuse_modules/pyramid_fuse.py
--- a/heal_amd/opencood/models/fuse_modules/pyramid_fuse.py
+++ b/heal_amd/opencood/models/fuse_modules/pyramid_fuse.py
@@ -153,11 +153,19 @@
         other = (0, c0) if c0 > 0 else (c1, n)
         bg = self._zero_response(x)
         plan = self._camcrop_plan(x, cam_slice, box)
+        merged = self._merged_ok(n, plan)
+        if merged and derived.capturing() and not derived.ready(*self._stage_out_slot(x, cam_slice, box)):
+            merged = False
+        stage_out = self._stage_outputs(x.contiguous(), cam_slice, box, plan, bg) if merged else None
         feats = []
         for i in range(self.layernum_):
             layer = getattr(self.resnet, f"layer{i}")
             if plan[i] is None:
                 x = self.resnet.run_stage(layer, x)
+                feats.append(x)
+                continue
+            if merged:
+                x = self._merged_stage(layer, x.contiguous(), other, cam_slice, plan[i], stage_out[i])
                 feats.append(x)
                 continue
             (cy0, cy1, cx0, cx1), (gy0, gy1, gx0, gx1), (py0, py1, px0, px1) = plan[i]
@@ -172,6 +180,47 @@
             x = full
             feats.append(x)
         return feats
+
+    def _merged_ok(self, n, plan):
+        import os
+        if os.environ.get("HEAL_PYRAMID_MERGED", "1") != "1" or n > 8:
+            return False
+        return all(blk.images_ok() for i, p in enumerate(plan) if p is not None for blk in getattr(self.resnet, f"layer{i}"))
+
+    def _stage_out_slot(self, x, cam_slice, box):
+        tag, sources, extra = self._zero_response_slot(x)
+        stream = torch.cuda.current_stream(x.device).cuda_stream
+        return "pyramid_stage_out", sources, extra + (int(x.shape[0]), tuple(cam_slice), tuple(box), stream)
+
+    def _stage_outputs(self, x, cam_slice, box, plan, bg):
+        n, (c0, c1) = int(x.shape[0]), cam_slice
+
+        def build():
+            outs = []
+            for i, p in enumerate(plan):
+                full = None
+                if p is not None:
+                    full = torch.empty((n,) + tuple(bg[i].shape[1:]), dtype=x.dtype, device=x.device)
+                    full[c0:c1] = bg[i]
+                outs.append(full)
+            return outs
+        return derived.derived(*self._stage_out_slot(x, cam_slice, box)[:2], build, self._stage_out_slot(x, cam_slice, box)[2])
+
+    def _merged_stage(self, layer, x, other, cam_slice, plan_i, full):
+        (cy0, cy1, cx0, cx1), _, (py0, py1, px0, px1) = plan_i
+        s_tot = 1
+        for blk in layer:
+            s_tot *= blk.stride
+        lidar = list(range(other[0], other[1]))
+        cams = list(range(*cam_slice))
+        regs = [ops.Region(x, j) for j in lidar] + [ops.Region(x, c, cy0, cx0, cy1 - cy0, cx1 - cx0) for c in cams]
+        ho, wo = (cy1 - cy0) // s_tot, (cx1 - cx0) // s_tot
+        outs = [ops.Region(full, j) for j in lidar] + [ops.Region(full, c, cy0 // s_tot, cx0 // s_tot, ho, wo) for c in cams]
+        windows = [None] * len(lidar) + [(py0, py1, px0, px1)] * len(cams)
+        for j, blk in enumerate(layer):
+            last = j == len(layer) - 1
+            regs = blk.forward_images(regs, outs if last else None, windows if last else None)
+        return full
 
     @property
     def layernum_(self):
diff --git a/heal_amd/opencood/models/sub_modules/bev_blocks.py b/heal_amd/opencood/models/sub_modules/bev_blocks.py
--- a/heal_amd/opencood/models/sub_modules/bev_blocks.py
+++ b/heal_amd/opencood/models/sub_modules/bev_blocks.py
@@ -220,6 +220,43 @@
         y = ConvBN.run(x, self.conv1, self.bn1, relu=True)
         y = ConvBN.run(y, self.conv2, self.bn2, relu=True)
         return ConvBN.run(y, self.conv3, self.bn3, relu=True, residual=identity, out=out)
+
+    def images_ok(self):
+        c2, d = self.conv2, self.downsample
+        cg = c2.in_channels // c2.groups
+        return (_CONV1X1 and c2.kernel_size == (3, 3) and c2.padding == (1, 1) and c2.dilation == (1, 1) and c2.stride in ((1, 1), (2, 2))
+                and c2.groups > 1 and cg in (4, 8, 16) and c2.in_channels % 16 == 0 and c2.out_channels == c2.in_channels
+                and self.conv1.stride == (1, 1) and self.conv3.stride == (1, 1)
+                and (d is None or (isinstance(d[0], nn.Conv2d) and d[0].kernel_size == (1, 1) and d[0].stride == c2.stride
+                                   and d[0].padding == (0, 0) and d[0].groups == 1)))
+
+    def forward_images(self, ins, outs=None, windows=None):
+        from heal_amd import ops
+        s = self.conv2.stride[0]
+
+        def compact(channels, stride):
+            sizes, regs = {}, []
+            for r in ins:
+                sizes.setdefault(((r.h - 1) // stride + 1, (r.w - 1) // stride + 1), []).append(r)
+            bufs = {hw: torch.empty((len(v), channels) + hw, dtype=torch.float32, device=ins[0].base.device) for hw, v in sizes.items()}
+            taken = dict.fromkeys(sizes, 0)
+            for r in ins:
+                hw = ((r.h - 1) // stride + 1, (r.w - 1) // stride + 1)
+                regs.append(ops.Region(bufs[hw], taken[hw]))
+                taken[hw] += 1
+            return regs
+        w1, b1 = fold_bn(self.conv1, self.bn1)
+        w2, b2 = fold_bn(self.conv2, self.bn2)
+        w3, b3 = fold_bn(self.conv3, self.bn3)
+        identity = ins
+        if self.downsample is not None:
+            wd, bd = fold_bn(self.downsample[0], self.downsample[1])
+            identity = ops.conv1x1_images(ins, wd, bd, compact(int(wd.shape[0]), s), act=0, stride=s)
+        y = ops.conv1x1_images(ins, w1, b1, compact(int(w1.shape[0]), 1), act=1)
+        y = ops.grouped_conv3x3_images(y, w2, b2, self.conv2.groups, compact(int(w2.shape[0]), s), stride=s, relu=True)
+        if outs is None:
+            outs = compact(int(w3.shape[0]), s)
+        return ops.conv1x1_images(y, w3, b3, outs, residuals=identity, act=1, windows=windows)
 
 
 class ResNetModified(nn.Module):
diff --git a/heal_amd/ops.py b/heal_amd/ops.py
--- a/heal_amd/ops.py
+++ b/heal_amd/ops.py
@@ -1548,6 +1548,114 @@
         _capi.call("heal_grouped_conv3x3", _ptr(x), _ptr(weight), _ptr(bias), n, C, int(groups), H, W, int(stride),
                    int(bool(relu)), _ptr(y), _stream())
     return y
+
+class Region:
+
+    def __init__(self, base, n=0, y0=0, x0=0, h=None, w=None):
+        if base.dim() == 3:
+            base = base.unsqueeze(0)
+        self.base, self.n, self.y0, self.x0 = base, int(n), int(y0), int(x0)
+        self.h = int(base.shape[2]) - self.y0 if h is None else int(h)
+        self.w = int(base.shape[3]) - self.x0 if w is None else int(w)
+
+    def check(self, who, channels, device_check=True):
+        b = self.base
+        if not isinstance(b, torch.Tensor) or (device_check and not b.is_cuda) or b.dtype != torch.float32 or not b.is_contiguous():
+            raise _capi.HealAmdError(f"{who}: a region's base must be a contiguous f32 CUDA/HIP tensor")
+        if int(b.shape[1]) != channels:
+            raise _capi.HealAmdError(f"{who}: a region's base has {int(b.shape[1])} channels, want {channels}")
+        if not (0 <= self.n < b.shape[0] and 0 <= self.y0 and 0 <= self.x0 and self.h >= 1 and self.w >= 1
+                and self.y0 + self.h <= b.shape[2] and self.x0 + self.w <= b.shape[3]):
+            raise _capi.HealAmdError(f"{who}: region ({self.n}, {self.y0}:{self.y0 + self.h}, {self.x0}:{self.x0 + self.w}) outside "
+                                     f"its base {tuple(b.shape)}")
+
+    def pitches(self):
+        _, C, H, W = (int(v) for v in self.base.shape)
+        return (self.n * C * H + self.y0) * W + self.x0, W, H * W
+
+    def view(self):
+        return self.base[self.n, :, self.y0:self.y0 + self.h, self.x0:self.x0 + self.w]
+
+
+def image_descs(who, xs, ys, rs, cin, cout, stride, windows=None, device_check=True):
+    n = len(xs)
+    if not 1 <= n <= _capi.IMAGES_MAX or len(ys) != n or (rs is not None and len(rs) != n) or (windows is not None and len(windows) != n):
+        raise _capi.HealAmdError(f"{who}: 1..{_capi.IMAGES_MAX} images, as many outputs (residuals, windows) as inputs")
+    for r in xs:
+        r.check(who, cin, device_check)
+    for r in list(ys) + list(rs or []):
+        r.check(who, cout, device_check)
+    for i in range(n):
+        ho, wo = (xs[i].h - 1) // stride + 1, (xs[i].w - 1) // stride + 1
+        for r, name in ((ys[i], "output"),) + (((rs[i], "residual"),) if rs is not None else ()):
+            if (r.h, r.w) != (ho, wo):
+                raise _capi.HealAmdError(f"{who}: image {i}: {name} region is {r.h}x{r.w}, the convolution gives {ho}x{wo}")
+
+    def base_of(regs):
+        p0 = min(r.base.data_ptr() for r in regs)
+        return p0, [((r.base.data_ptr() - p0) // 4,) + r.pitches() for r in regs]
+    xp, xo = base_of(xs)
+    yp, yo = base_of(ys)
+    rp, ro = base_of(rs) if rs is not None else (None, None)
+    arr = (_capi.ImageDesc * n)()
+    for i in range(n):
+        d = arr[i]
+        d.x_off, d.x_row, d.x_chan = xo[i][0] + xo[i][1], xo[i][2], xo[i][3]
+        d.y_off, d.y_row, d.y_chan = yo[i][0] + yo[i][1], yo[i][2], yo[i][3]
+        if ro is not None:
+            d.r_off, d.r_row, d.r_chan = ro[i][0] + ro[i][1], ro[i][2], ro[i][3]
+        d.H, d.W = xs[i].h, xs[i].w
+        if windows is not None and windows[i] is not None:
+            d.wy0, d.wy1, d.wx0, d.wx1 = (int(v) for v in windows[i])
+            if (d.wy0, d.wy1, d.wx0, d.wx1) == (0, 0, 0, 0):
+                raise _capi.HealAmdError(f"{who}: image {i}: an empty store window")
+    return arr, ctypes.c_void_p(xp), ctypes.c_void_p(yp), (ctypes.c_void_p(rp) if rp is not None else None)
+
+
+def images_plan(descs, kind, stride, group_channels=0):
+    n = len(descs)
+    out = (ctypes.c_int * (n + 1))()
+    _capi.call("heal_images_plan", ctypes.cast(descs, ctypes.c_void_p), n, int(kind), int(stride), int(group_channels),
+               ctypes.cast(out, ctypes.c_void_p))
+    return list(out)
+
+
+def images_locate(tile0, tile):
+    arr = (ctypes.c_int * len(tile0))(*tile0)
+    return int(_capi.lib().heal_images_locate(ctypes.cast(arr, ctypes.c_void_p), len(tile0) - 1, int(tile)))
+
+
+def conv1x1_images(xs, w, bias, ys, residuals=None, act=0, stride=1, windows=None):
+    cout, cin = int(w.shape[0]), int(w.shape[1])
+    w = _need(w, torch.float32, "w")
+    bias = _need_bias(bias, cout, "conv1x1_images")
+    if stride not in (1, 2):
+        raise _capi.HealAmdError(f"conv1x1_images: stride must be 1 or 2 (got {stride})")
+    descs, xp, yp, rp = image_descs("conv1x1_images", xs, ys, residuals, cin, cout, stride, windows)
+    frag = conv1x1_fragments(w)
+    pix = sum(r.h * r.w for r in ys)
+    with _Timed(f"conv1x1_images_{cin}_{cout}" + ("_s2" if stride == 2 else ""), 2.0 * cin * cout * pix,
+                4.0 * pix * (cin + cout * (2 if residuals is not None else 1)), kernel_events=True):
+        _capi.call("heal_conv1x1_images", xp, _ptr(frag), _ptr(bias) if bias is not None else None, rp,
+                   ctypes.cast(descs, ctypes.c_void_p), len(descs), cin, cout, int(stride), int(act), yp, _stream())
+    return ys
+
+
+def grouped_conv3x3_images(xs, weight, bias, groups, ys, stride=1, relu=True):
+    weight = _need(weight, torch.float32, "weight")
+    C = int(weight.shape[0])
+    cg = C // groups
+    if cg not in (4, 8, 16) or C % 16 or int(weight.shape[1]) != cg:
+        raise _capi.HealAmdError(f"grouped_conv3x3_images: 4, 8 or 16 channels per group and C % 16 == 0 (got C={C}, groups={groups})")
+    bias = _need_bias(bias, C, "grouped_conv3x3_images")
+    descs, xp, yp, _ = image_descs("grouped_conv3x3_images", xs, ys, None, C, C, stride)
+    frag = grouped_small_fragments(weight, cg)
+    pin, pout = sum(r.h * r.w for r in xs), sum(r.h * r.w for r in ys)
+    with _Timed(f"grouped_conv3x3_images_c{C}" + ("_s2" if stride == 2 else ""), 2.0 * 9 * C * cg * pout, 4.0 * C * (pin + pout),
+                kernel_events=True):
+        _capi.call("heal_grouped_small_conv3x3_images", xp, _ptr(frag), _ptr(bias), ctypes.cast(descs, ctypes.c_void_p), len(descs),
+                   C, cg, int(stride), int(bool(relu)), yp, _stream())
+    return ys
 
 
 def gconv_conv3_supported(width, cg, cout, H, W):
diff --git a/include/heal_amd.h b/include/heal_amd.h
--- a/include/heal_amd.h
+++ b/include/heal_amd.h
@@ -8,7 +8,7 @@
 extern "C" {
 #endif
 
-#define HEAL_AMD_ABI_VERSION 9
+#define HEAL_AMD_ABI_VERSION 10
 
 int heal_abi_version(void);
 const char* heal_last_error(void);
@@ -250,6 +250,20 @@
 int heal_grouped_small_conv3x3(const float* x, const float* weight_q, const float* bias, int n, int channels,
                                int group_channels, int H, int W, int stride, int relu, float* y, void* stream);
 
+#define HEAL_IMAGES_MAX 8
+typedef struct heal_image_desc {
+    long long x_off, y_off, r_off;
+    int x_row, x_chan, y_row, y_chan, r_row, r_chan;
+    int H, W;
+    int wy0, wy1, wx0, wx1;
+} heal_image_desc;
+int heal_conv1x1_images(const float* x, const float* weight_frag, const float* bias, const float* residual,
+                        const heal_image_desc* images, int n_images, int cin, int cout, int stride, int act, float* y, void* stream);
+int heal_grouped_small_conv3x3_images(const float* x, const float* weight_q, const float* bias, const heal_image_desc* images,
+                                      int n_images, int channels, int group_channels, int stride, int relu, float* y, void* stream);
+int heal_images_plan(const heal_image_desc* images, int n_images, int kind, int stride, int group_channels, int* tile0);
+int heal_images_locate(const int* tile0, int n_images, int tile);
+
 int heal_conv3x3_winograd(const float* x, const float* u_frag, const float* bias, const float* residual, int n, int cin,
                           int cout, int H, int W, int relu, int waves, float* y, void* stream);
 int heal_conv3x3_winograd_kc(const float* x, const float* u_frag, const float* bias, const float* residual, int n, int cin,
```

Result: no change. 162.6 (median of 5 runs) (-0.0%).
